# robot-learning-freiburg/CL-SLAM

Measured on AMD Instinct MI355X. Metric: online-adapt frames/sec @192x640 (1 triplet + K replay), higher is better.
Workload: dtype f32; 1 GPU; DepthPosePrediction.adapt(steps=1), 192x640, 1 online + K=4 replay triplets (global batch 5); ResNet-18 depth+pose nets, closed-form random-init weights; a frame = 5 triplets (value = steps/s * B/5); global_batch=5, replay_k=4, height=192, width=640, adapt_steps_per_frame=1, parallelism=single, lcd_encoder_in_frame=False

## Files before the change

cl-slam_amd/clslam_hip/_lib.py:

```python
import ctypes as C
from pathlib import Path

import torch
from typing import Optional

LIB_PATH = Path(__file__).resolve().parents[1] / 'lib' / 'libclslam_hip.so'

OK = 0
ACT_NONE, ACT_RELU, ACT_ELU, ACT_HSWISH, ACT_HSIGMOID = 0, 1, 2, 3, 4
PAD_ZERO, PAD_REFLECT = 0, 1
DEPTH_EVAL_MEDIAN_SCALING, DEPTH_EVAL_FROM_DISP, DEPTH_EVAL_NO_MAX = 1, 2, 4

fptr = C.c_void_p
i32 = C.c_int32


class ConvDesc(C.Structure):
    _fields_ = [('src_a', fptr), ('src_b', fptr), ('weight', fptr), ('scale', fptr), ('shift', fptr),
                ('residual', fptr), ('out', fptr),
                ('batch', i32), ('in_h', i32), ('in_w', i32), ('ch_a', i32), ('ch_b', i32),
                ('out_h', i32), ('out_w', i32), ('ch_out', i32),
                ('ksize', i32), ('stride', i32), ('pad', i32), ('pad_mode', i32), ('upsample_a', i32),
                ('act', i32), ('config', i32), ('actgrad_src', fptr), ('actgrad_kind', i32),
                ('workspace', C.c_void_p), ('workspace_bytes', C.c_size_t), ('weight_wino', fptr), ('cu_limit', i32)]


class TransposeItem(C.Structure):
    _fields_ = [('w', fptr), ('wt', fptr), ('ch_out', i32), ('taps', i32), ('ch_in', i32), ('ch_in_sel', i32)]


class CopyItem(C.Structure):
    _fields_ = [('src', C.c_void_p), ('dst', C.c_void_p), ('bytes', C.c_size_t)]


class LossDesc(C.Structure):
    _fields_ = [('partial', fptr * 4), ('disp', fptr * 4), ('rgb0', fptr * 4), ('means', fptr * 4),
                ('pose', fptr), ('dist0', fptr), ('dist1', fptr), ('sample_w', fptr), ('smooth_w', fptr),
                ('losses', fptr), ('smooth_aux', fptr),
                ('batch', i32), ('nblk', i32), ('H', i32), ('W', i32), ('n_smooth', i32),
                ('smooth_scale', C.c_float), ('vel_scale', C.c_float)]


_SIGNATURES = {
    'clslam_version': [],
    'clslam_is_device_build': [],
    'clslam_conv2d': [C.POINTER(ConvDesc), C.c_void_p],
    'clslam_conv2d_pick_config': [C.POINTER(ConvDesc)],
    'clslam_wino_weight_transform': [fptr, fptr, i32, i32, C.c_void_p],
    'clslam_weight_transpose': [fptr, fptr, i32, i32, i32, i32, C.c_void_p],
    'clslam_weight_transpose_multi': [C.POINTER(TransposeItem), i32, C.c_void_p],
    'clslam_fold_blocks': [i32, i32, i32, i32, i32],
    'clslam_fold_act_grad': [fptr, fptr, fptr, fptr, i32, i32, i32, i32, i32, i32, i32, i32, fptr, fptr, C.c_void_p],
    'clslam_wgrad_splits': [C.POINTER(ConvDesc), i32],
    'clslam_conv_wgrad': [C.POINTER(ConvDesc), fptr, fptr, i32, C.c_void_p],
    'clslam_wgrad_patch_supported': [C.POINTER(ConvDesc)],
    'clslam_wgrad_patch_splits': [C.POINTER(ConvDesc), i32],
    'clslam_conv_wgrad_patch': [C.POINTER(ConvDesc), fptr, fptr, i32, C.c_void_p],
    'clslam_reduce_partials': [fptr, fptr, C.c_size_t, i32, C.c_float, C.c_void_p],
    'clslam_reduce_multi': [fptr, i32, i32, C.c_void_p],
    'clslam_reduce_multi_adam': [fptr, i32, i32, fptr, fptr, fptr, fptr, C.c_double, C.c_double, C.c_double, C.c_double, i32, fptr, C.c_void_p],
    'clslam_colsum_blocks': [i32],
    'clslam_colsum': [fptr, fptr, i32, i32, C.c_void_p],
    'clslam_stem_packed_size': [i32],
    'clslam_stem_pack_weight': [fptr, fptr, i32, C.c_void_p],
    'clslam_stem_conv': [fptr, fptr, fptr, fptr, fptr, fptr, i32, i32, i32, i32, C.c_void_p],
    'clslam_maxpool3x3s2': [fptr, fptr, i32, i32, i32, i32, C.c_void_p],
    'clslam_dispconv_fwd': [fptr, fptr, fptr, fptr, i32, i32, i32, i32, C.c_void_p],
    'clslam_dispconv_bwd_data': [fptr, fptr, fptr, i32, i32, i32, i32, i32, C.c_void_p],
    'clslam_dispconv_wgrad_blocks': [i32],
    'clslam_dispconv_wgrad': [fptr, fptr, fptr, i32, i32, i32, i32, C.c_void_p],
    'clslam_pose_head_fwd': [fptr, fptr, fptr, fptr, fptr, i32, i32, C.c_void_p],
    'clslam_pose_head_bwd': [fptr, fptr, fptr, fptr, fptr, fptr, fptr, i32, i32, C.c_float, C.c_void_p],
    'clslam_pose_to_proj': [fptr, fptr, fptr, fptr, i32, C.c_void_p],
    'clslam_warp_fwd': [fptr, i32, i32, fptr, fptr, fptr, fptr, fptr, fptr, i32, i32, i32, C.c_float, C.c_float, C.c_void_p],
    'clslam_warp_fwd_pyramid': [C.POINTER(fptr), fptr, fptr, fptr, fptr, fptr, fptr, i32, i32, i32, C.c_float, C.c_float, C.c_void_p],
    'clslam_warp_coords_pyramid': [C.POINTER(fptr), fptr, fptr, fptr, i32, i32, i32, C.c_float, C.c_float, C.c_void_p],
    'clslam_warp_cells_pyramid': [C.POINTER(fptr), fptr, fptr, C.c_void_p, i32, i32, i32, C.c_float, C.c_float, C.c_void_p],
    'clslam_warp_bwd_blocks': [i32, i32],
    'clslam_automask_pyramid': [fptr, fptr, fptr, fptr, fptr, i32, i32, i32, i32, C.c_void_p],
    'clslam_disp_mean_pyramid': [C.POINTER(fptr), fptr, i32, i32, i32, C.c_void_p],
    'clslam_photo_automask_pyramid': [fptr, fptr, fptr, fptr, fptr, fptr, fptr, i32, i32, i32, C.c_void_p],
    'clslam_warp_fwd_pyramid_range': [C.POINTER(fptr), fptr, fptr, fptr, fptr, fptr, fptr, i32, i32, i32, C.c_float, C.c_float, i32, i32,
                                      C.c_void_p],
    'clslam_photo_automask_pyramid_range': [fptr, fptr, fptr, fptr, C.c_uint64, C.c_uint64, fptr, fptr, fptr, i32, i32, i32, i32, i32,
                                            C.c_void_p],
    'clslam_loss_bwd2_pyramid_range': [C.POINTER(fptr), fptr, fptr, fptr, fptr, fptr, fptr, fptr, fptr, fptr, fptr, fptr, i32, i32, i32,
                                       C.c_float, C.c_float, i32, i32, C.c_void_p],
    'clslam_disp_grad_pyramid_range': [fptr, C.POINTER(fptr), fptr, i32, C.POINTER(fptr), i32, i32, i32, i32, i32, C.c_void_p],
    'clslam_photo_automask_pyramid_rng': [fptr, fptr, fptr, C.c_uint64, C.c_uint64, fptr, fptr, fptr, i32, i32, i32, C.c_void_p],
    'clslam_tie_break_noise': [fptr, C.c_size_t, C.c_uint64, C.c_uint64, C.c_void_p],
    'clslam_smooth_intended_chunks': [],
    'clslam_smooth_intended_fwd': [C.POINTER(fptr), C.POINTER(fptr), fptr, i32, i32, i32, C.c_void_p],
    'clslam_smooth_intended_finalize': [fptr, fptr, fptr, fptr, fptr, i32, i32, i32, C.c_float, C.c_void_p],
    'clslam_smooth_intended_bwd': [C.POINTER(fptr), C.POINTER(fptr), fptr, fptr, C.POINTER(fptr), i32, i32, i32, C.c_float, C.c_void_p],
    'clslam_loss_bwd2_blocks': [i32, i32],
    'clslam_loss_bwd2_pyramid': [C.POINTER(fptr), fptr, fptr, fptr, fptr, fptr, fptr, fptr, fptr, fptr, fptr, fptr, i32, i32, i32,
                                 C.c_float, C.c_float, C.c_void_p],
    'clslam_loss_bwd_blocks': [i32, i32],
    'clslam_loss_bwd_pyramid': [C.POINTER(fptr), fptr, fptr, fptr, fptr, fptr, fptr, fptr, fptr, fptr, fptr, fptr, i32, i32, i32,
                                C.c_float, C.c_float, C.c_void_p],
    'clslam_disp_grad_pyramid': [fptr, C.POINTER(fptr), fptr, i32, C.POINTER(fptr), i32, i32, i32, C.c_void_p],
    'clslam_warp_bwd': [fptr, fptr, i32, i32, fptr, fptr, fptr, fptr, fptr, fptr, i32, i32, i32, C.c_float, C.c_float,
                        C.c_void_p],
    'clslam_pose_bwd': [fptr, i32, i32, fptr, fptr, fptr, fptr, fptr, C.c_float, fptr, i32, C.c_void_p],
    'clslam_photo_map': [fptr, fptr, fptr, fptr, i32, i32, i32, i32, C.c_void_p],
    'clslam_automask_blocks': [i32, i32],
    'clslam_automask': [fptr, fptr, fptr, fptr, fptr, i32, i32, i32, C.c_void_p],
    'clslam_disp_mean_chunks': [],
    'clslam_disp_mean': [fptr, fptr, i32, i32, C.c_void_p],
    'clslam_loss_finalize': [C.POINTER(LossDesc), C.c_void_p],
    'clslam_photo_grad': [fptr, fptr, fptr, fptr, fptr, fptr, i32, i32, i32, C.c_void_p],
    'clslam_mbv3_stem': [fptr, fptr, fptr, fptr, fptr, i32, i32, i32, C.c_void_p],
    'clslam_dwconv': [fptr, fptr, fptr, fptr, fptr, i32, i32, i32, i32, i32, i32, i32, C.c_void_p],
    'clslam_lanczos_ksize': [i32, i32],
    'clslam_lanczos_plan': [i32, i32, C.c_void_p, C.c_void_p],
    'clslam_resize_pass_u8': [C.c_void_p, C.c_void_p, fptr, C.c_void_p, C.c_void_p, i32, i32, i32, i32, i32, i32, i32, C.c_void_p],
    'clslam_u8_to_planar_f32': [C.c_void_p, fptr, i32, i32, i32, i32, C.c_void_p],
    'clslam_color_jitter_u8': [C.c_void_p, C.c_void_p, C.c_void_p, C.c_void_p, i32, i32, i32, C.POINTER(C.c_int), i32,
                               C.POINTER(C.c_double), C.c_void_p],
    'clslam_color_jitter_f32_blocks': [i32, i32],
    'clslam_color_jitter_f32': [fptr, fptr, C.c_void_p, fptr, i32, i32, i32, C.c_void_p],
    'clslam_avgpool_chunks': [i32],
    'clslam_global_avgpool': [fptr, fptr, fptr, i32, i32, i32, C.c_void_p],
    'clslam_se_gate': [fptr, fptr, fptr, fptr, fptr, fptr, i32, i32, i32, C.c_void_p],
    'clslam_channel_scale': [fptr, fptr, i32, i32, i32, C.c_void_p],
    'clslam_adam_step': [fptr, fptr, fptr, fptr, C.c_size_t, C.c_double, C.c_double, C.c_double, C.c_double, i32, C.c_float,
                         fptr, C.c_void_p],
    'clslam_disp_grad': [fptr, fptr, fptr, i32, fptr, i32, i32, i32, i32, i32, C.c_void_p],
    'clslam_copy_multi': [C.c_void_p, i32, C.c_void_p],
    'clslam_handoff_arm': [C.c_void_p],
    'clslam_handoff_wait': [C.c_void_p, C.c_void_p, C.c_void_p],
    'clslam_conv_profile_begin': [i32],
    'clslam_conv_profile_end': [C.c_void_p, i32, C.c_void_p],
    'clslam_ip_scores': [fptr, fptr, fptr, i32, i32, i32, C.c_void_p],
    'clslam_topk_chunks': [i32],
    'clslam_topk_desc': [fptr, i32, i32, i32, fptr, C.c_void_p, fptr, C.c_void_p, C.c_void_p],
    'clslam_l2_normalize_rows': [fptr, i32, i32, C.c_void_p],
    'clslam_diversity_commit': [fptr, fptr, i32, C.c_void_p, i32, i32, i32, i32, C.c_float, fptr, fptr, C.c_void_p,
                                fptr, C.c_void_p],    'clslam_pgo_edge_eval': [fptr, fptr, fptr, i32, fptr, fptr, fptr, C.c_void_p],
    'clslam_pgo_lin_stride': [],
    'clslam_pgo_build_system': [fptr, fptr, fptr, fptr, fptr, i32, fptr, fptr, fptr, i32, i32, fptr, fptr, fptr, fptr, C.c_void_p],
    'clslam_pgo_solve_workspace': [i32],
    'clslam_pgo_solve': [fptr, fptr, fptr, fptr, fptr, C.c_double, i32, C.c_double, i32, fptr, fptr, fptr, C.c_void_p],
    'clslam_pgo_update_score': [fptr, fptr, fptr, i32, fptr, fptr, fptr, fptr, fptr, i32, i32, fptr, i32, C.c_void_p],
    'clslam_depth_metrics_scratch': [i32, i32, i32],
    'clslam_depth_metrics': [fptr, fptr, fptr, C.c_void_p, fptr, fptr, i32, i32, i32, i32, i32, C.c_float, C.c_float, i32, C.c_void_p],
    'clslam_pcl_backproject_scratch': [i32, i32, i32],
    'clslam_pcl_backproject': [fptr, fptr, fptr, fptr, fptr, C.c_void_p, i32, i32, i32, C.c_float, C.c_void_p],
    'clslam_pcl_transform': [fptr, fptr, fptr, fptr, C.c_longlong, i32, C.c_void_p],
    'clslam_pcl_splat_scratch': [i32, i32],
    'clslam_pcl_splat': [fptr, fptr, fptr, i32, fptr, fptr, i32, i32, C.c_longlong, C.c_longlong, i32, C.c_double, i32, C.c_void_p],
    'clslam_pcl_resolve': [fptr, fptr, C.c_longlong, fptr, fptr, fptr, i32, i32, i32, C.c_void_p],
}
_RESTYPES = {'clslam_last_error': C.c_char_p, 'clslam_last_error_string': C.c_char_p, 'clslam_build_id': C.c_char_p}
ABI_VERSION = 106
_SIZE_FNS = {'clslam_wino_weight_size': [i32, i32]}
_PTR_FNS = {'clslam_handoff_event_create': []}
_VOID_FNS = {'clslam_handoff_event_destroy': [C.c_void_p]}


class ClslamError(RuntimeError):
    pass


class Library:
    def __init__(self, path: Path, require_device: bool = True) -> None:
        if not Path(path).exists():
            raise ClslamError(
                f'{path} not found: build it with `python cl-slam_amd/csrc/build.py` '
                '(hipcc --offload-arch=gfx950). There is no CPU fallback for this path.')
        self.path = Path(path)
        self.cdll = C.CDLL(str(path))
        try:
            got = int(self.cdll.clslam_version())
        except AttributeError:
            raise ClslamError(f'{path} does not export clslam_version: not a clslam kernel library') from None
        if got != ABI_VERSION:
            raise ClslamError(f'{path} implements ABI version {got}, this binding needs {ABI_VERSION}: rebuild it with '
                              '`python cl-slam_amd/csrc/build.py`')
        for name, rt in _RESTYPES.items():
            fn = getattr(self.cdll, name)
            fn.restype, fn.argtypes = rt, []
        for name, argtypes in _SIZE_FNS.items():
            fn = getattr(self.cdll, name)
            fn.restype, fn.argtypes = C.c_size_t, argtypes
        for name, argtypes in _PTR_FNS.items():
            fn = getattr(self.cdll, name)
            fn.restype, fn.argtypes = C.c_void_p, argtypes
        for name, argtypes in _VOID_FNS.items():
            fn = getattr(self.cdll, name)
            fn.restype, fn.argtypes = None, argtypes
        for name, argtypes in _SIGNATURES.items():
            fn = getattr(self.cdll, name)
            fn.argtypes = argtypes
            fn.restype = C.c_int
        self.is_device = bool(self.cdll.clslam_is_device_build())
        if require_device and not self.is_device:
            raise ClslamError(f'{path} is not a gfx950 device build')

    def call(self, name: str, *args) -> None:
        rc = getattr(self.cdll, name)(*args)
        if rc != OK:
            raise ClslamError(f'{name} failed ({rc}): {self.cdll.clslam_last_error().decode()}')

    @property
    def device_type(self) -> str:
        return 'cuda' if self.is_device else 'cpu'


_LIB: Optional[Library] = None


def get_lib() -> Library:
    global _LIB
    if _LIB is None:
        _LIB = Library(LIB_PATH, require_device=True)
    return _LIB


def install_library_for_tests(path) -> Library:
    global _LIB
    _LIB = Library(Path(path), require_device=False)
    return _LIB


def exported_symbols():
    return list(_RESTYPES) + list(_SIZE_FNS) + list(_PTR_FNS) + list(_VOID_FNS) + list(_SIGNATURES)


def build_id() -> str:
    built = get_lib().cdll.clslam_build_id().decode()
    built = built.split(':', 1)[1] if built.startswith('clslam-build-id:') else built
    csrc = Path(__file__).resolve().parents[1] / 'csrc'
    if not (csrc / 'build.py').exists():
        return built
    import importlib.util
    spec = importlib.util.spec_from_file_location('_clslam_build', csrc / 'build.py')
    mod = importlib.util.module_from_spec(spec)
    spec.loader.exec_module(mod)
    src = mod.source_id()
    return built if built == src else f'stale:{built}/{src}'
```

cl-slam_amd/clslam_hip/engine.py:

```python
import contextlib
import math
import os
from types import SimpleNamespace
from typing import Any, Dict, List, Optional, Tuple

import torch

from . import ops
from ._lib import ACT_ELU, ACT_NONE, ACT_RELU, PAD_REFLECT, PAD_ZERO, ClslamError, get_lib

NUM_CH_ENC = (64, 64, 128, 256, 512)
NUM_CH_DEC = (16, 32, 64, 128, 256)
BN_EPS = 1e-5

LOSS_NAMES = ('reprojection_loss', 'smooth_loss', 'reg_loss', 'depth_loss')

WGRAD_TARGET_BLOCKS = 512


def _align4(n: int) -> int:
    return (n + 3) // 4 * 4


class TrainableLayout:
# ... 111 lines not shown
        for st in (self.main_stream, self.side_stream, self.wg_stream, self.capture_stream):
            if st is not None:
                self._conv_workspace(st.cuda_stream)
        self.async_tail = False
        self.data_parallel = False
        self.tail_stream = pool.get('tail')
        self._tail_event = None
        self._tail_open = False
        self.fuse_adam = os.environ.get('CLSLAM_FUSE_ADAM', '0') == '1'
        self._pending_reduce = None
        self.descriptor_memo = os.environ.get('CLSLAM_DESCRIPTOR_MEMO', '1') != '0'
        self._memo = None
        self.memo_hits = 0
        self.grad_buckets = int(os.environ.get('CLSLAM_GRAD_BUCKETS', '3'))
        self.grads_synced = False
        self.time_exchange = False
        self.exchange_events: List[Any] = []
        self.exchange_main_done = None
        self._capturing = False
        self._noise_torch_seed = None
        self.noise_seed = 1
        self.noise_draws = 0
        self.noise_stream = 0
        self._handoff = ops.Handoff() if device.type == 'cuda' else None
        self._cu_enc = self._cu_dec = self._cu_pose = self._cu_depth = 0
        self.device_cus = (torch.cuda.get_device_properties(device).multi_processor_count if device.type == 'cuda' else 256)
        self.reuse_frozen_features = os.environ.get('CLSLAM_REUSE_FROZEN', '1') != '0'
        self.winograd = not os.environ.get('CLSLAM_NO_WINOGRAD')

    def bind(self, models: Dict[str, torch.nn.Module]) -> None:
        self.models = models
        for name, m in models.items():
            m._bind(self, name)

    def _module_version(self) -> int:
        if self._tracked is None:
            self._tracked = [t for m in self.models.values() for t in torch.nn.Module.state_dict(m, keep_vars=True).values()]
        return sum(t._version for t in self._tracked)

    def pack_if_needed(self) -> None:
        ver = self._module_version()
        if ver != self._packed_version:
            if self._modules_stale:
                raise ClslamError('module parameters were modified while newer adapted weights live in the engine; '
                                  'call sync_modules() first')
            self.pack()

    def _on(self, st):
        if st is None:
            return contextlib.nullcontext()
        return torch.cuda.stream(st) if self._capturing else ops.launch_on(st)

    def _use_tail(self) -> bool:
        return (self.async_tail and self.tail_stream is not None and self.device.type == 'cuda' and not self._capturing
                and ops.PROFILE is None)

    def _side_streams(self):
        return (self.side_stream, self.wg_stream) if self.use_side_stream else (None, None)

    def cu_limit(self, B: int, phase: str = 'encoders') -> int:
        if not phase.startswith('enc'):
            return 0
        if not (self.use_side_stream and 2 <= B <= 16):
            return 0
        if phase == 'enc_pose':
            return self.device_cus * 5 // 8
        if phase == 'enc_depth':
            return self.device_cus * 3 // 8
        return self.device_cus // 2

    def wait_training(self, stream=None) -> None:
        if self._tail_event is not None:
            (stream or torch.cuda.current_stream(self.device)).wait_event(self._tail_event)
        if self._train_done is not None:
            (stream or torch.cuda.current_stream(self.device)).wait_event(self._train_done)

    @property
    def w(self) -> torch.Tensor:
        self.wait_training()
        return self._w

    @property
    def g(self) -> torch.Tensor:
        self.wait_training()
        return self._g

    @property
    def m(self) -> torch.Tensor:
        self.wait_training()
        return self._m

    @property
    def v(self) -> torch.Tensor:
        self.wait_training()
        return self._v

    def prealloc_outputs(self, B: int) -> None:
        H, W = self.H, self.W
        E = lambda *s: torch.empty(*s, device=self.device)
        self._prealloc = (B, ([E(B, H >> s, W >> s) for s in range(4)], E(2 * B, 12), E(2, B, 4, 4), E(4, B, H, W),
                              E(4, 2, B, 3, H, W), E(18)))

    def detached_ok(self) -> bool:
        return (self.detached_training and self.main_stream is not None and self.device.type == 'cuda'
                and not self._capturing and ops.PROFILE is None)

    def begin_detached(self):
        cur = torch.cuda.current_stream(self.device)
        em = self.main_stream
        if cur.cuda_stream == em.cuda_stream:
            return cur, None
        em.wait_stream(cur)
        self._caller = cur
        return cur, em

    def end_detached(self, cur, released, failed: bool = False) -> None:
        self._caller = None
        self._prealloc, self._prealloc_armed = None, False
        ev = torch.cuda.Event()
        ev.record(self.main_stream)
        self._train_done = ev
        cur.wait_event(ev if (failed or released is None) else released)

    def training_stream(self):
        return torch.cuda.stream(self.tail_stream) if self._tail_open else contextlib.nullcontext()

    @torch.no_grad()
    def pack(self) -> None:
        dev = self.device
        self.wait_training()
        for which in ('depth_encoder', 'pose_encoder'):
            sd = {k: v.detach().to(dev, torch.float32) for k, v in torch.nn.Module.state_dict(self.models[which]).items()}
            e = SimpleNamespace()

            def bn(prefix):
                scale = sd[prefix + '.weight'] / torch.sqrt(sd[prefix + '.running_var'] + BN_EPS)
                shift = sd[prefix + '.bias'] - sd[prefix + '.running_mean'] * scale
                return scale.contiguous(), shift.contiguous()

            def conv(key):
                wt = sd[key]
                return wt.permute(0, 2, 3, 1).reshape(wt.shape[0], wt.shape[2] * wt.shape[3], wt.shape[1]).contiguous()

            e.stem_w = ops.stem_pack_weight(sd['resnet.conv1.weight'].contiguous())
            e.stem_scale, e.stem_shift = bn('resnet.bn1')
            e.blocks = []
            for li, (cin, cout, stride) in enumerate(((64, 64, 1), (64, 128, 2), (128, 256, 2), (256, 512, 2)), start=1):
                for bi in range(2):
                    p = f'resnet.layer{li}.{bi}'
                    blk = SimpleNamespace(stride=stride if bi == 0 else 1, cin=cin if bi == 0 else cout, cout=cout)
                    blk.w1 = conv(p + '.conv1.weight'); blk.s1, blk.b1 = bn(p + '.bn1')
                    blk.w2 = conv(p + '.conv2.weight'); blk.s2, blk.b2 = bn(p + '.bn2')
                    blk.u1 = ops.wino_weight_transform(blk.w1) if (blk.stride == 1 and self.winograd) else None
                    blk.u2 = ops.wino_weight_transform(blk.w2) if self.winograd else None
                    blk.wd = None
                    if (p + '.downsample.0.weight') in sd:
                        blk.wd = conv(p + '.downsample.0.weight'); blk.sd, blk.bd = bn(p + '.downsample.1')
                    e.blocks.append(blk)
            self.enc[which] = e
        for name, off, shape in self.layout.entries:
            model, key = name.split('/', 1)
            t = torch.nn.Module.state_dict(self.models[model])[key].detach().to(dev, torch.float32)
            flat = TrainableLayout.to_compute(t)
            self._w[off:off + flat.numel()].copy_(flat)
        self._packed_version = self._module_version()
        self._modules_stale = False
        self._desc_cache.clear()
        for ws in self._ws.values():
            if hasattr(ws, 'frozen_valid'):
                ws.frozen_valid = False
        self._memo = None

    @torch.no_grad()
    def sync_modules(self) -> None:
        if not self._modules_stale or self.models is None:
            return
        self.wait_training()
        for name, off, shape in self.layout.entries:
            model, key = name.split('/', 1)
            p = torch.nn.Module.state_dict(self.models[model], keep_vars=True)[key]
            p.data.copy_(TrainableLayout.to_reference(self._w[off:off + math.prod(shape)], shape))
        self._modules_stale = False
        self._packed_version = self._module_version()

    @torch.no_grad()
    def install_weights(self, flat: torch.Tensor, adam_step_count: Optional[int] = None) -> None:
        self.pack_if_needed()
        self.wait_training()
        self._w.copy_(flat.reshape(-1)[:self.layout.size])
        if adam_step_count is not None:
            self.adam_step_count = int(adam_step_count)
        self._modules_stale = True

    def wview(self, name: str) -> torch.Tensor:
        self.wait_training()
        for n, off, shape in self.layout.entries:
            if n == name:
                return self._w[off:off + math.prod(shape)]
        raise KeyError(name)

    def _slot(self, buf: torch.Tensor, name: str, numel: int) -> torch.Tensor:
        off = self.layout.offset[name]
        return buf[off:off + numel]

    def workspace(self, B: int) -> SimpleNamespace:
        ws = self._ws.get(B)
        if ws is not None:
            return ws
        dev, H, W = self.device, self.H, self.W
        E = lambda *s: torch.empty(*s, device=dev)
        ws = SimpleNamespace(B=B)
        ws.denc = self._enc_bufs(B)
        ws.penc = self._enc_bufs(2 * B)
        self._depth_dec_bufs(B, ws)
        self._pose_dec_bufs(2 * B, ws)
        ws.T = E(2, B, 4, 4)
        ws.P = E(2, B, 3, 4)
        ws.depth = E(4, B, H, W)
        ws.warped = E(4, 2, B, 3, H, W)
        ws.idmap = E(2, B, H, W)
        ws.coef = None
        ws.sel = torch.empty(4, B, H, W, dtype=torch.uint8, device=dev)
        ws.nblk = ops.automask_blocks(H, W)
        ws.partial = E(4, B, ws.nblk)
        ws.means = E(4, B, ops.disp_mean_chunks())
        ws.losses = E(18)
        ws.noise = E(4, B, 2, H, W)
        ws.train = None
        self._ws[B] = ws
        return ws

    def _enc_bufs(self, n: int) -> SimpleNamespace:
        dev, H, W = self.device, self.H, self.W
        E = lambda *s: torch.empty(*s, device=dev)
        hs = [H >> k for k in range(6)]
        wsz = [W >> k for k in range(6)]
        e = SimpleNamespace()
        e.f0 = E(n, hs[1], wsz[1], 64)
        e.pool = E(n, hs[2], wsz[2], 64)
        e.t = [E(n, hs[2 + li], wsz[2 + li], c) for li, c in enumerate((64, 128, 256, 512))]
        e.ds = [None] + [E(n, hs[2 + li], wsz[2 + li], c) for li, c in ((1, 128), (2, 256), (3, 512))]
        e.y = [[E(n, hs[2 + li], wsz[2 + li], c) for _ in range(2)] for li, c in enumerate((64, 128, 256, 512))]
        return e

    def _depth_dec_bufs(self, n: int, st: Optional[SimpleNamespace] = None) -> SimpleNamespace:
        st = SimpleNamespace() if st is None else st
        H, W = self.H, self.W
        E = lambda *s: torch.empty(*s, device=self.device)
        st.x = {}
        for i in range(4, -1, -1):
            st.x[i, 0] = E(n, H >> (i + 1), W >> (i + 1), NUM_CH_DEC[i])
            st.x[i, 1] = E(n, H >> i, W >> i, NUM_CH_DEC[i])
        st.disp = [E(n, H >> s, W >> s) for s in range(4)]
        return st

    def _pose_dec_bufs(self, n: int, st: Optional[SimpleNamespace] = None) -> SimpleNamespace:
        st = SimpleNamespace() if st is None else st
        h5, w5 = self.H >> 5, self.W >> 5
        E = lambda *s: torch.empty(*s, device=self.device)
        st.sq, st.p0, st.p1 = E(n, h5, w5, 256), E(n, h5, w5, 256), E(n, h5, w5, 256)
        st.pmean, st.pose = E(n, 256), E(n, 12)
        return st

    def _train_bufs(self, ws: SimpleNamespace) -> SimpleNamespace:
        if ws.train is not None:
            return ws.train
        dev, H, W, B = self.device, self.H, self.W, ws.B
        E = lambda *s: torch.empty(*s, device=dev)
        t = SimpleNamespace()
        ws.coef = E(4, B, 9, H, W)
        t.ddisp_up = E(4, B, H, W)
        t.nb2 = ops.loss_bwd2_blocks(H, W)
        t.dp_partial = torch.empty(4, B, t.nb2, 24, dtype=torch.float64, device=dev)
        t.dz_disp = [torch.empty(B, H >> s, W >> s, device=dev) for s in range(4)]
        t.dpose = E(2 * B, 12)
        t.dz = {k: torch.empty_like(v) for k, v in ws.x.items()}
        pad_elems = max(B * ((H >> i) + 2) * ((W >> i) + 2) * NUM_CH_DEC[i] for i in range(5))
        t.dxp = [E(pad_elems), E(pad_elems)]
        t.wt_ready = None
        t.wt_dec = {}
        t.wt_pose = {}
        t.wt_table = None
        t.dz_p1 = torch.empty_like(ws.p1)
        t.dz_p0 = torch.empty_like(ws.p0)
        t.dz_sq = torch.empty_like(ws.sq)
        t.plan, t.items, t.table, t.disp_part = {}, [], None, {}
        t.side = SimpleNamespace()
        t.bias_part = {k: E(ops.fold_blocks(v.shape[0], v.shape[1], v.shape[2], v.shape[3], False) * v.shape[-1])
                       for k, v in ws.x.items()}
        ws.train = t
        return t

    CONV_WS_BYTES = 32 << 20

    def _conv_workspace(self, handle: Optional[int] = None) -> None:
        if self.device.type != 'cuda' and handle is None:
            handle = 0
        if handle is None:
            handle = torch.cuda.current_stream(self.device).cuda_stream
        if handle not in self._conv_ws:
            self._conv_ws[handle] = torch.zeros(self.CONV_WS_BYTES, dtype=torch.uint8, device=self.device)
            ops.set_conv_workspace(handle, self._conv_ws[handle])

    def _encoder(self, e, bufs, n: int, stem_inputs, waits=None, stream=None, aux=None, cu_limit=None) -> List[torch.Tensor]:
        ops.PERSISTENT_CU_LIMIT = self._cu_enc if cu_limit is None else cu_limit
        ek = (id(self), 'enc', id(e), id(bufs), n)
        for i, (img_a, img_b, off, cnt) in enumerate(stem_inputs):
            if waits is not None:
                (stream or torch.cuda.current_stream(self.device)).wait_event(waits[i])
            ops.stem_conv(img_a, img_b, e.stem_w, e.stem_scale, e.stem_shift, bufs.f0[off:off + cnt])
        ops.maxpool3x3s2(bufs.f0, bufs.pool)
        x = bufs.pool
        feats = [bufs.f0]
        for li in range(4):
            for bi in range(2):
                blk = e.blocks[li * 2 + bi]
                t, y = bufs.t[li], bufs.y[li][bi]
                res, joined = x, None
                if blk.wd is not None:
                    res = bufs.ds[li]
                    if aux is not None and stream is not None:
                        evs = bufs.__dict__.setdefault('ds_events', {})
                        fork, joined = evs.get(li) or evs.setdefault(li, (torch.cuda.Event(), torch.cuda.Event()))
                        fork.record(stream)
                        aux.wait_event(fork)
                        with self._on(aux):
                            ops.conv2d(x, blk.wd, res, scale=blk.sd, shift=blk.bd, ksize=1, stride=blk.stride, pad=0, act=ACT_NONE,
                                       cache=self._desc_cache, key=(ek, li, bi, 'd'))
                        joined.record(aux)
                ops.conv2d(x, blk.w1, t, scale=blk.s1, shift=blk.b1, ksize=3, stride=blk.stride, act=ACT_RELU, weight_wino=blk.u1,
                           cache=self._desc_cache, key=(ek, li, bi, 1))
                if blk.wd is not None and joined is None:
                    ops.conv2d(x, blk.wd, res, scale=blk.sd, shift=blk.bd, ksize=1, stride=blk.stride, pad=0, act=ACT_NONE,
                               cache=self._desc_cache, key=(ek, li, bi, 'd'))
                if joined is not None:
                    stream.wait_event(joined)
                ops.conv2d(t, blk.w2, y, scale=blk.s2, shift=blk.b2, residual=res, ksize=3, act=ACT_RELU, weight_wino=blk.u2,
                           cache=self._desc_cache, key=(ek, li, bi, 2))
                x = y
            feats.append(x)
        return feats

    def _wb(self, prefix: str, cout: int, cin: int, taps: int):
        hit = self._wb_cache.get(prefix)
        if hit is None:
            w = self._slot(self._w, prefix + '.weight', cout * taps * cin).view(cout, taps, cin)
            b = self._slot(self._w, prefix + '.bias', cout)
            hit = self._wb_cache[prefix] = (w, b)
        return hit

    def _depth_decoder(self, ws, feats: List[torch.Tensor]) -> None:
        x = feats[4]
        ops.PERSISTENT_CU_LIMIT = self._cu_dec
        main = self._main
        leaf = self._side_streams()[1] if main is not None else None
        forked = False
        for i in range(4, -1, -1):
            cin0 = NUM_CH_ENC[-1] if i == 4 else NUM_CH_DEC[i + 1]
            w, b = self._wb(f'depth_decoder/upconv_{i}_0.conv.conv', NUM_CH_DEC[i], cin0, 9)
            ops.conv2d(x, w, ws.x[i, 0], shift=b, ksize=3, pad_mode=PAD_REFLECT, act=ACT_ELU, cache=self._desc_cache, key=(id(self), 'dec', id(ws), i, 0))
            skip = feats[i - 1] if i > 0 else None
            cin1 = NUM_CH_DEC[i] + (NUM_CH_ENC[i - 1] if i > 0 else 0)
            w, b = self._wb(f'depth_decoder/upconv_{i}_1.conv.conv', NUM_CH_DEC[i], cin1, 9)
            fork = leaf is not None and 0 < i <= 3
            ho = self._handoff if (fork and not self._capturing and ops.PROFILE is None) else None
            if ho is not None:
                ho.arm()
            ops.conv2d(ws.x[i, 0], w, ws.x[i, 1], src_b=skip, shift=b, ksize=3, pad_mode=PAD_REFLECT, upsample_a=True,
                       act=ACT_ELU, cache=self._desc_cache, key=None if skip is None else (id(self), 'dec', id(ws), i, 1, skip.data_ptr()))
            x = ws.x[i, 1]
            if i <= 3:
                w, b = self._wb(f'depth_decoder/dispconv_{i}.conv', 1, NUM_CH_DEC[i], 9)
                if fork:
                    if ho is not None:
                        ho.release(main, leaf)
                    else:
                        ev = torch.cuda.Event()
                        ev.record(main)
                        leaf.wait_event(ev)
                    with self._on(leaf):
                        ops.dispconv_fwd(x, w.view(9, NUM_CH_DEC[i]), b, ws.disp[i])
                    forked = True
                else:
                    ops.dispconv_fwd(x, w.view(9, NUM_CH_DEC[i]), b, ws.disp[i])
        if forked:
            main.wait_stream(leaf)

    def _pose_decoder(self, ws, f4: torch.Tensor) -> None:
        ops.PERSISTENT_CU_LIMIT = self._cu_dec
        w, b = self._wb('pose_decoder/squeeze', 256, 512, 1)
        ops.conv2d(f4, w, ws.sq, shift=b, ksize=1, pad=0, act=ACT_RELU, cache=self._desc_cache, key=(id(self), 'pdec', id(ws), 0))
        w, b = self._wb('pose_decoder/pose_0', 256, 256, 9)
        ops.conv2d(ws.sq, w, ws.p0, shift=b, ksize=3, act=ACT_RELU, cache=self._desc_cache, key=(id(self), 'pdec', id(ws), 1))
        w, b = self._wb('pose_decoder/pose_1', 256, 256, 9)
        ops.conv2d(ws.p0, w, ws.p1, shift=b, ksize=3, act=ACT_RELU, cache=self._desc_cache, key=(id(self), 'pdec', id(ws), 2))
        w, b = self._wb('pose_decoder/pose_2', 12, 256, 1)
        ops.pose_head_fwd(ws.p1, w.view(12, 256), b, ws.pmean, ws.pose)

    def forward(self, inputs: Dict[Any, torch.Tensor], *, train: bool, sample_w: torch.Tensor,
                smooth_w: Optional[torch.Tensor], noise: Optional[Dict[int, torch.Tensor]] = None,
                draw_noise: bool = True, keep_noise: bool = False,
                reuse_frozen: bool = False, inputs_ready=None) -> Tuple[Dict[Any, torch.Tensor], torch.Tensor]:
        self._main = torch.cuda.current_stream(self.device) if self.device.type == 'cuda' else None
        self._conv_workspace(None if self._main is None else self._main.cuda_stream)
        if self._train_done is not None and self._main.cuda_stream != self.main_stream.cuda_stream:
            self._main.wait_event(self._train_done)
        c = SimpleNamespace(inputs=inputs, inputs_ready=inputs_ready, train=train, noise=noise, draw_noise=draw_noise,
                            keep_noise=keep_noise, have_noise=False, id_ready=None)
        self._convert_inputs(c)
        B = c.B
        self._cu_enc, self._cu_dec = self.cu_limit(B, 'encoders'), self.cu_limit(B, 'decoders')
        self._cu_pose, self._cu_depth = self.cu_limit(B, 'enc_pose'), self.cu_limit(B, 'enc_depth')
        ops.PERSISTENT_CU_LIMIT = self._cu_dec
        ws = self.workspace(B)
        c.reuse = bool(reuse_frozen and self.reuse_frozen_features and getattr(ws, 'frozen_valid', False))
        ws.frozen_valid = False
        c.memo_feats = self._memo_lookup(c.aug[0]) if (B == 1 and not c.reuse) else None
        if train:
            self._train_bufs(ws)
        if self.fresh_outputs:
            self._fresh_output_planes(ws, B)
        self._networks(ws, c)
        self._loss_stage(ws, c, sample_w, smooth_w)
        ws.frozen_valid = True
        return self._outputs(ws, B), ws.losses

    def _convert_inputs(self, c) -> None:
        inputs, H, W = c.inputs, self.H, self.W
        if c.inputs_ready is not None:
            needs_conversion = any(inputs[k, f, 0].dtype != torch.float32 or not inputs[k, f, 0].is_contiguous()
                                   for k in ('rgb_aug', 'rgb') for f in (-1, 0, 1))
            self._main.wait_event(c.inputs_ready[3 if needs_conversion else 0])
        c.aug = {f: self._img(inputs['rgb_aug', f, 0]) for f in (-1, 0, 1)}
        c.rgb = {f: self._img(inputs['rgb', f, 0]) for f in (-1, 0, 1)}
        B = c.B = c.aug[0].shape[0]
        for name, group in (('rgb_aug', c.aug), ('rgb', c.rgb)):
            for f, t in group.items():
                if tuple(t.shape) != (B, 3, H, W):
                    raise ClslamError(f"('{name}', {f}, 0) must be ({B}, 3, {H}, {W}), got {tuple(t.shape)}")
        for s in range(1, 4):
            t = inputs['rgb', 0, s]
            if tuple(t.shape) != (B, 3, H >> s, W >> s):
                raise ClslamError(f"('rgb', 0, {s}) must be ({B}, 3, {H >> s}, {W >> s}), got {tuple(t.shape)}")
        for k in (('camera_matrix', 0), ('inv_camera_matrix', 0)):
            if tuple(inputs[k].shape) != (B, 4, 4):
                raise ClslamError(f'{k} must be ({B}, 4, 4), got {tuple(inputs[k].shape)}')

    def _fresh_output_planes(self, ws, B: int) -> None:
        H, W = self.H, self.W
        pre = self._prealloc if self._prealloc_armed else None
        if pre is not None and pre[0] == B:
            self._prealloc = None
            ws.disp, ws.pose, ws.T, ws.depth, ws.warped, ws.losses = pre[1]
        else:
            E = lambda *s: torch.empty(*s, device=self.device)
            ws.disp = [E(B, H >> s, W >> s) for s in range(4)]
            ws.pose, ws.T = E(2 * B, 12), E(2, B, 4, 4)
            ws.depth, ws.warped, ws.losses = E(4, B, H, W), E(4, 2, B, 3, H, W), E(18)

    def _identity_and_noise(self, ws, c) -> bool:
        if not c.reuse:
            ops.photo_map(c.rgb[-1], c.rgb[0], ws.idmap[0], None, c.B, c.B, self.H, self.W)
            ops.photo_map(c.rgb[1], c.rgb[0], ws.idmap[1], None, c.B, c.B, self.H, self.W)
        if c.noise is not None:
            for s in range(4):
                ws.noise[s].copy_(c.noise[s])
            return True
        if c.keep_noise:
            return True
        if c.draw_noise and self._capturing:
            ws.noise.normal_().mul_(1e-5)
            return True
        return False

    def _enqueue_identity(self, ws, c, wg) -> None:
        if c.inputs_ready is not None:
            wg.wait_event(c.inputs_ready[3])
        with (torch.cuda.stream(wg) if (c.noise is not None or self._capturing) else ops.launch_on(wg)):
            c.have_noise = self._identity_and_noise(ws, c)
        c.id_ready = torch.cuda.Event()
        c.id_ready.record(wg)

    def _pose_encoder(self, ws, c, **kw) -> torch.Tensor:
        aug, B = c.aug, c.B
        return self._encoder(self.enc['pose_encoder'], ws.penc, 2 * B, [(aug[-1], aug[0], 0, B), (aug[0], aug[1], B, B)],
                             waits=None if c.inputs_ready is None else c.inputs_ready[1:3], cu_limit=self._cu_pose, **kw)[4]

    def _pose_branch(self, ws, c, side, ds_aux) -> torch.Tensor:
        with self._on(side):
            pf4 = ws.pf4 if c.reuse else self._pose_encoder(ws, c, stream=side, aux=ds_aux)
            self.wait_training(side)
            self._pose_decoder(ws, pf4)
        return pf4

    def _networks(self, ws, c) -> None:
        B, reuse, main = c.B, c.reuse, self._main
        side, wg = self._side_streams()
        ds_aux = wg if (B == 1 and not self._capturing) else None
        defer_identity = wg is not None and ds_aux is not None and c.inputs_ready is not None and not reuse
        if wg is not None:
            wg.wait_stream(main)
            if not defer_identity:
                self._enqueue_identity(ws, c, wg)
        if side is not None:
            side.wait_stream(main)
            if reuse:
                dfeats = ws.dfeats
                self.wait_training(main)
                self._depth_decoder(ws, dfeats)
                pf4 = self._pose_branch(ws, c, side, ds_aux)
            else:
                dfeats = c.memo_feats if c.memo_feats is not None else self._encoder(
                    self.enc['depth_encoder'], ws.denc, B, [(c.aug[0], None, 0, B)], stream=main, aux=ds_aux, cu_limit=self._cu_depth)
                pf4 = self._pose_branch(ws, c, side, ds_aux)
                self.wait_training(main)
                self._depth_decoder(ws, dfeats)
            main.wait_stream(side)
        else:
            self.wait_training()
            dfeats = (ws.dfeats if reuse else c.memo_feats if c.memo_feats is not None else
                      self._encoder(self.enc['depth_encoder'], ws.denc, B, [(c.aug[0], None, 0, B)], cu_limit=self._cu_depth))
            self._depth_decoder(ws, dfeats)
            pf4 = ws.pf4 if reuse else self._pose_encoder(ws, c)
            self._pose_decoder(ws, pf4)
        ws.dfeats, ws.pf4 = dfeats, pf4
        if defer_identity:
            self._enqueue_identity(ws, c, wg)

    def _loss_stage(self, ws, c, sample_w: torch.Tensor, smooth_w: Optional[torch.Tensor]) -> None:
        inputs, rgb, B, H, W = c.inputs, c.rgb, c.B, self.H, self.W
        if c.inputs_ready is not None:
            self._main.wait_event(c.inputs_ready[3])
        K = self._mat(inputs['camera_matrix', 0])
        Kinv = self._mat(inputs['inv_camera_matrix', 0])
        ops.pose_to_proj(ws.pose, K, ws.T, ws.P)
        ops.warp_fwd_pyramid(ws.disp, rgb[-1], rgb[1], Kinv, ws.P, ws.depth, ws.warped, self.min_depth, self.max_depth)
        if c.id_ready is not None:
            self._main.wait_event(c.id_ready)
        else:
            c.have_noise = self._identity_and_noise(ws, c)
        if c.have_noise or not c.draw_noise:
            ops.photo_automask_pyramid(ws.warped, rgb[0], ws.idmap, ws.noise if c.have_noise else None, ws.sel,
                                       ws.coef if c.train else None, ws.partial, B, H, W)
        else:
            seed, offset = self._next_noise_draw()
            ops.photo_automask_pyramid_rng(ws.warped, rgb[0], ws.idmap, seed, offset, ws.sel,
                                           ws.coef if c.train else None, ws.partial, B, H, W)
        ops.disp_mean_pyramid(ws.disp, ws.means, H, W)
        n_smooth = 0 if (smooth_w is None or self.smooth_intended) else int(smooth_w.numel())
        if n_smooth and not (n_smooth < (W >> 3) - 1):
            raise ClslamError('reference smoothness layout needs batch < width/8 - 1')
        aux = getattr(ws, 'smooth_aux', None)
        if n_smooth and (aux is None or aux.shape[1] != 2 + 2 * n_smooth):
            aux = torch.zeros(4, 2 + 2 * n_smooth, device=self.device)
            ws.smooth_aux = aux
        d0 = inputs['relative_distance', 0].to(torch.float64).reshape(-1).contiguous() if self.vel_scale > 0 else None
        d1 = inputs['relative_distance', 1].to(torch.float64).reshape(-1).contiguous() if self.vel_scale > 0 else None
        rgb0 = [self._img(inputs['rgb', 0, s]) for s in range(4)]
        ops.loss_finalize([ws.partial[s] for s in range(4)], ws.disp, rgb0, [ws.means[s] for s in range(4)], ws.pose, d0, d1,
                          sample_w, smooth_w if n_smooth else None, ws.losses, aux if n_smooth else None, B, ws.nblk, H, W,
                          n_smooth, self.smooth_scale, self.vel_scale)
        if self.smooth_intended:
            if getattr(ws, 'si_partial', None) is None:
                ws.si_partial = torch.empty(4, B, ops.smooth_intended_chunks(), device=self.device)
                ws.si_aux = torch.empty(4, B, 2, device=self.device)
            ops.smooth_intended_fwd(ws.disp, rgb0, ws.si_partial, H, W)
            ops.smooth_intended_finalize(ws.si_partial, ws.means, sample_w, ws.losses, ws.si_aux, B, H, W, self.smooth_scale)
        ws.ctx = SimpleNamespace(rgb=rgb, K=K, Kinv=Kinv, d0=d0, d1=d1, sample_w=sample_w, n_smooth=n_smooth,
                                 aux=aux if n_smooth else None, B=B, rgb0=rgb0)

    def _memo_lookup(self, x: torch.Tensor) -> Optional[List[torch.Tensor]]:
        m = self._memo
        if (m is None or not self.descriptor_memo or self._capturing or m.version != self._packed_version
                or m.x.shape != x.shape or m.x.device != x.device):
            return None
        self._memo = None
        if not bool(torch.equal(m.x, x)):
            return None
        self.memo_hits += 1
        return m.feats

    def _next_noise_draw(self) -> Tuple[int, int]:
        if self.device.type == 'cuda':
            gen = torch.cuda.default_generators[self.device.index if self.device.index is not None else torch.cuda.current_device()]
            ts = int(gen.initial_seed())
            off = int(gen.get_offset())
            gen.set_offset(off + 4)
            self.noise_draws = off // 4 + 1
        else:
            ts = int(torch.default_generator.initial_seed())
            if ts != self._noise_torch_seed:
                self.noise_draws = 0
            self.noise_draws += 1
        if ts != self._noise_torch_seed:
            self._noise_torch_seed = ts
            self.noise_seed = (ts * 0x9E3779B97F4A7C15 + 0x7F4A7C15) & 0xFFFFFFFFFFFFFFFF or 1
        return self.noise_seed, (int(self.noise_stream) << 40) | self.noise_draws

    def _img(self, t: torch.Tensor) -> torch.Tensor:
        if t.dtype != torch.float32 or not t.is_contiguous():
            t = t.to(torch.float32).contiguous()
        return t

    def _mat(self, t: torch.Tensor) -> torch.Tensor:
        return t.to(torch.float32).contiguous()

    def _outputs(self, ws, B: int) -> Dict[Any, torch.Tensor]:
        out: Dict[Any, torch.Tensor] = {}
        for s in (3, 2, 1, 0):
            out['disp', s] = ws.disp[s].unsqueeze(1)
        for fi, f in enumerate((-1, 1)):
            out['axis_angle', 0, f] = ws.pose[fi * B:(fi + 1) * B, 0:3].unsqueeze(1)
            out['translation', 0, f] = ws.pose[fi * B:(fi + 1) * B, 3:6].unsqueeze(1)
            out['cam_T_cam', 0, f] = ws.T[fi]
        for s in range(4):
            out['depth', s] = ws.depth[s].unsqueeze(1)
            for fi, f in enumerate((-1, 1)):
                out['rgb', f, s] = ws.warped[s, fi]
        return out

    def losses_dict(self, losses: torch.Tensor) -> Dict[str, torch.Tensor]:
        d: Dict[str, torch.Tensor] = {}
        for s in range(4):
            for j, name in enumerate(LOSS_NAMES):
                d[f'{name}/scale_{s}'] = losses[s * 4 + j]
        total = losses[17:18]
        d['depth_loss'] = total
        if self.vel_scale > 0:
            d['velocity_loss'] = losses[16]
        d['loss'] = total
        return d

    def _wgrad(self, t, desc_src, out_shape, dz, name_prefix: str, cout: int, cin: int, taps: int, bias_blocks: int = 0,
               bias_partial=None, **geom) -> None:
        desc = ops.conv_desc(desc_src[0], out_shape, src_b=desc_src[1], ksize=3 if taps == 9 else 1, **geom)
        n = cout * taps * cin
        plan = t.plan.get(name_prefix)
        if plan is None:
            use_patch = ops.wgrad_patch_supported(desc)
            splits = (ops.wgrad_patch_splits(desc, WGRAD_TARGET_BLOCKS) if use_patch else
                      ops.wgrad_splits(desc, WGRAD_TARGET_BLOCKS))
            plan = SimpleNamespace(use_patch=use_patch, splits=splits, partial=torch.empty(splits * n, device=self.device),
                                   colsum=None, nb=0)
            t.items.append((plan.partial, self._slot(self._g, name_prefix + '.weight', n), n, splits))
            if bias_blocks:
                t.items.append((bias_partial, self._slot(self._g, name_prefix + '.bias', cout), cout, bias_blocks))
            else:
                rows = out_shape[0] * out_shape[1] * out_shape[2]
                plan.nb = ops.colsum_blocks(rows)
                plan.colsum = torch.empty(plan.nb * cout, device=self.device)
                t.items.append((plan.colsum, self._slot(self._g, name_prefix + '.bias', cout), cout, plan.nb))
            t.plan[name_prefix] = plan
        if plan.use_patch:
            ops.conv_wgrad_patch(desc, dz, plan.partial, plan.splits)
        else:
            ops.conv_wgrad(desc, dz, plan.partial, plan.splits)
        if plan.colsum is not None:
            ops.colsum(dz, plan.colsum, out_shape[0] * out_shape[1] * out_shape[2], cout)

    def bucket_ranges(self):
        off = self.layout.offset
        a_end, c_start = off['depth_decoder/upconv_3_0.conv.conv.weight'], off['pose_decoder/squeeze.weight']
        if self.grad_buckets >= 3:
            return [('pose', c_start, self.layout.size), ('mid', a_end, c_start), ('deep', 0, a_end)]
        if self.grad_buckets == 2:
            return [('early', a_end, self.layout.size), ('deep', 0, a_end)]
        return [('all', 0, self.layout.size)]

    def exchange_report(self) -> Optional[Dict[str, Any]]:
        if not self.exchange_events or self.exchange_main_done is None:
            return None
        buckets = [{'bucket': n, 'mbytes': round(nb / 1e6, 2), 'ms': round(e0.elapsed_time(e1), 4)} for n, e0, e1, nb in self.exchange_events]
        total = sum(b['ms'] for b in buckets)
        exposed = max(0.0, self.exchange_main_done.elapsed_time(self.exchange_events[-1][2]))
        rep = {'buckets': buckets, 'allreduce_ms': round(total, 4), 'exposed_ms': round(exposed, 4),
               'overlap_fraction': round(1.0 - min(exposed, total) / total, 4) if total > 0 else None}
        self.exchange_events, self.exchange_main_done = [], None
        return rep

    def _bucket_sync(self, t, name: str, events, allreduce) -> None:
        tail = self.tail_stream
        for ev in events:
            tail.wait_event(ev)
        table, n, lo, hi = t.bucket_tables[name]
        with torch.cuda.stream(tail):
            ops.reduce_multi(table, n, self._g)
            if self.time_exchange:
                e0, e1 = torch.cuda.Event(enable_timing=True), torch.cuda.Event(enable_timing=True)
                e0.record(tail)
                allreduce(self._g[lo:hi])
                e1.record(tail)
                self.exchange_events.append((name, e0, e1, (hi - lo) * 4))
            else:
                allreduce(self._g[lo:hi])

    def backward(self, B: int, defer_reduce: bool = False, allreduce=None) -> None:
        ops.PERSISTENT_CU_LIMIT = self.cu_limit(B, 'backward')
        ws = self._ws[B]
        t = ws.train
        c = ws.ctx
        H, W = self.H, self.W
        feats = ws.dfeats
        self._main = torch.cuda.current_stream(self.device) if self.device.type == 'cuda' else None
        side, wg = self._side_streams()
        t.wt_ready = None
        if wg is None:
            self._transpose_decoder_weights(t)
        else:
            wg.wait_stream(self._main)
            with self._on(wg):
                self._transpose_decoder_weights(t)
            t.wt_ready = torch.cuda.Event()
            t.wt_ready.record(wg)
        ops.loss_bwd2_pyramid(ws.disp, ws.sel, ws.coef, ws.warped, c.rgb[0], c.rgb[-1], c.rgb[1], c.Kinv, ws.P, c.sample_w,
                              t.ddisp_up, t.dp_partial, self.min_depth, self.max_depth)
        ops.disp_grad_pyramid(t.ddisp_up, ws.disp, c.aux if c.n_smooth else None, c.n_smooth, t.dz_disp, H, W)
        if self.smooth_intended:
            ops.smooth_intended_bwd(ws.disp, c.rgb0, ws.si_aux, c.sample_w, t.dz_disp, H, W, self.smooth_scale)
        ops.pose_bwd(t.dp_partial, 4, t.nb2, ws.pose, c.K, c.d0, c.d1, c.sample_w, self.vel_scale, t.dpose)
        self.inputs_released = None
        if self._caller is not None:
            self.inputs_released = torch.cuda.Event()
            self.inputs_released.record(self._main)
        bucketed = allreduce is not None and self.grad_buckets > 1
        overlap = (bucketed and self._use_tail() and side is not None and wg is not None
                   and getattr(t, 'bucket_tables', None) is not None)
        self.grads_synced = False
        if side is not None:
            main = self._main
            side.wait_stream(main)
            if t.wt_ready is not None:
                side.wait_event(t.wt_ready)
            with self._on(side):
                self._backward_pose_decoder(ws, t, B, t.side)
            if overlap and self.grad_buckets >= 3:
                ev = torch.cuda.Event()
                ev.record(side)
                self._bucket_sync(t, 'pose', [ev], allreduce)
            self._backward_depth_decoder(ws, t, B, mid_done=(lambda evs: self._bucket_sync(
                t, 'mid' if self.grad_buckets >= 3 else 'early', evs, allreduce)) if overlap else None)
            main.wait_stream(side)
        else:
            self._backward_depth_decoder(ws, t, B)
            self._backward_pose_decoder(ws, t, B, t)
        if t.table is None:
            for key, n in (('pose_decoder/pose_2.weight', 12 * 256), ('pose_decoder/pose_2.bias', 12)):
                sl = self._slot(self._g, key, n)
                t.items.append((sl, sl, n, 1))
            t.table = ops.make_reduce_table(t.items, self.device)
            base = self._g.data_ptr()
            t.bucket_tables = {}
            for name, lo, hi in self.bucket_ranges():
                its = [it for it in t.items if lo <= (it[1].data_ptr() - base) // 4 < hi]
                t.bucket_tables[name] = (ops.make_reduce_table(its, self.device), len(its), lo, hi)
            assert sum(v[1] for v in t.bucket_tables.values()) == len(t.items)
        self._pending_reduce = None
        if bucketed:
            ranges = self.bucket_ranges()
            if overlap:
                name, lo, hi = ranges[-1]
                if self.time_exchange:
                    self.exchange_main_done = torch.cuda.Event(enable_timing=True)
                    self.exchange_main_done.record(self._main)
                self.tail_stream.wait_stream(self._main)
                self._bucket_sync(t, name, [], allreduce)
                self._tail_open = True
            else:
                if self._use_tail():
                    self.tail_stream.wait_stream(self._main)
                    with torch.cuda.stream(self.tail_stream):
                        ops.reduce_multi(t.table, len(t.items), self._g)
                        for name, lo, hi in ranges:
                            allreduce(self._g[lo:hi])
                    self._tail_open = True
                else:
                    ops.reduce_multi(t.table, len(t.items), self._g)
                    for name, lo, hi in ranges:
                        allreduce(self._g[lo:hi])
            self.grads_synced = True
        elif defer_reduce and self.fuse_adam and not self.data_parallel and not self._capturing and not self._use_tail():
            self._pending_reduce = (t.table, len(t.items))
        elif self._use_tail():
            self.tail_stream.wait_stream(self._main)
            with torch.cuda.stream(self.tail_stream):
                ops.reduce_multi(t.table, len(t.items), self._g)
            self._tail_open = True
        else:
            ops.reduce_multi(t.table, len(t.items), self._g)

    def _transpose_decoder_weights(self, t) -> None:
        if t.wt_table is None:
            items = []
            for i in range(5):
                ci = NUM_CH_DEC[i]
                cin1 = ci + (NUM_CH_ENC[i - 1] if i > 0 else 0)
                t.wt_dec[i, 1] = torch.empty(ci, 9, ci, device=self.device)
                w1, _ = self._wb(f'depth_decoder/upconv_{i}_1.conv.conv', ci, cin1, 9)
                items.append((w1, t.wt_dec[i, 1], ci))
                if i < 4:
                    cin0 = NUM_CH_DEC[i + 1]
                    t.wt_dec[i, 0] = torch.empty(cin0, 9, ci, device=self.device)
                    w0, _ = self._wb(f'depth_decoder/upconv_{i}_0.conv.conv', ci, cin0, 9)
                    items.append((w0, t.wt_dec[i, 0], None))
            for k in (0, 1):
                t.wt_pose[k] = torch.empty(256, 9, 256, device=self.device)
                wp, _ = self._wb(f'pose_decoder/pose_{k}', 256, 256, 9)
                items.append((wp, t.wt_pose[k], None))
            t.wt_table = ops.transpose_table(items)
        ops.weight_transpose_multi(t.wt_table, self._w)

    def _backward_depth_decoder(self, ws, t, B: int, mid_done=None) -> None:
        H, W = self.H, self.W
        feats = ws.dfeats
        main = self._main
        side, wg = self._side_streams()
        if wg is not None:
            wg.wait_stream(main)

        wg_streams = [wg] if (wg is None or side is None) else [wg, side]
        counter = [0]

        ho = self._handoff if (wg is not None and not self._capturing and ops.PROFILE is None) else None

        def on_wg(fn, dep='record'):
            if wg is None:
                fn()
                return
            st = wg_streams[counter[0] % len(wg_streams)]
            counter[0] += 1
            if dep == 'armed':
# ... 288 lines not shown
```

cl-slam_amd/clslam_hip/ops.py:

```python
import ctypes as C
from typing import Optional

import torch

from . import _lib
from ._lib import ACT_ELU, ACT_HSIGMOID, ACT_HSWISH, ACT_NONE, ACT_RELU, PAD_REFLECT, PAD_ZERO


PROFILE = None


def profile_begin(max_launches: int = 8192) -> None:
    global PROFILE
    _lib.get_lib().call('clslam_conv_profile_begin', max_launches)
    PROFILE = []


def profile_end():
    global PROFILE
    meta, PROFILE = PROFILE, None
    cap = max(1, len(meta))
    ms = (C.c_float * cap)()
    count = C.c_int(0)
    _lib.get_lib().call('clslam_conv_profile_end', C.cast(ms, C.c_void_p), cap, C.cast(C.pointer(count), C.c_void_p))
    if not _lib.get_lib().is_device:
        return [(k, cfg, fl, 0.0, desc, nb) for k, cfg, fl, desc, nb in meta]
    if count.value != len(meta):
        raise _lib.ClslamError(f'profile_end: {count.value} timed launches for {len(meta)} conv2d calls')
    return [(k, cfg, fl, ms[i] * 1e-3, desc, nb) for i, (k, cfg, fl, desc, nb) in enumerate(meta)]


_raw_stream = torch._C._cuda_getCurrentRawStream if hasattr(torch._C, '_cuda_getCurrentRawStream') else None


_FORCED_STREAM: Optional[int] = None


class launch_on:
    __slots__ = ('handle', 'prev')

    def __init__(self, stream):
        self.handle = None if stream is None else stream.cuda_stream

    def __enter__(self):
        global _FORCED_STREAM
        self.prev = _FORCED_STREAM
        if self.handle is not None:
            _FORCED_STREAM = self.handle
        return self

    def __exit__(self, *exc):
        global _FORCED_STREAM
        _FORCED_STREAM = self.prev
        return False


def _stream(t: torch.Tensor) -> int:
    if _FORCED_STREAM is not None:
        return _FORCED_STREAM
    if t.is_cuda:
        if _raw_stream is not None:
            return _raw_stream(t.device.index)
        return torch.cuda.current_stream(t.device).cuda_stream
    return 0


_QUERY_CACHE: dict = {}


def _query(name: str, *args) -> int:
    lib = _lib._LIB or _lib.get_lib()
    key = (id(lib), name, args)
    v = _QUERY_CACHE.get(key)
    if v is None:
        v = _QUERY_CACHE[key] = getattr(lib.cdll, name)(*args)
    return v


def _p(t: Optional[torch.Tensor]):
    if t is None:
        return None
    lib = _lib._LIB or _lib.get_lib()
    if t.is_cuda != lib.is_device or t.dtype is not torch.float32 or not t.is_contiguous():
        if t.device.type != lib.device_type:
            raise _lib.ClslamError(f'tensor on {t.device}, library {lib.path.name} runs on {lib.device_type}')
        raise _lib.ClslamError(f'expected contiguous fp32, got {t.dtype} contiguous={t.is_contiguous()}')
    return t.data_ptr()


def _pa(t: Optional[torch.Tensor], dtype):
    if t is None:
        return None
    lib = _lib.get_lib()
    if t.device.type != lib.device_type or t.dtype != dtype or not t.is_contiguous():
        raise _lib.ClslamError(f'expected contiguous {dtype} on {lib.device_type}, got {t.dtype} on {t.device}')
    return t.data_ptr()


class Handoff:
    POOL = 64

    def __init__(self) -> None:
        self.lib = _lib.get_lib()
        self.events = []
        self.next = 0
        self.armed = None

    def arm(self) -> None:
        if not self.lib.is_device:
            return
        if len(self.events) < self.POOL:
            ev = self.lib.cdll.clslam_handoff_event_create()
            if not ev:
                raise _lib.ClslamError('clslam_handoff_event_create failed: ' + self.lib.cdll.clslam_last_error().decode())
            self.events.append(ev)
            self.armed = ev
        else:
            self.armed = self.events[self.next % self.POOL]
        self.next += 1
        self.lib.call('clslam_handoff_arm', self.armed)

    def release(self, producer, consumer) -> None:
        ev, self.armed = self.armed, None
        if ev is None:
            return
        self.lib.call('clslam_handoff_wait', ev, producer.cuda_stream, consumer.cuda_stream)

    def __del__(self):
        try:
            for ev in self.events:
                self.lib.cdll.clslam_handoff_event_destroy(ev)
        except Exception:
            pass


_CONV_WORKSPACES = {}


def set_conv_workspace(stream_handle: int, workspace: Optional[torch.Tensor]) -> None:
    if workspace is None:
        _CONV_WORKSPACES.pop(stream_handle, None)
    else:
        assert workspace.dtype == torch.uint8 and workspace.is_contiguous()
        _CONV_WORKSPACES[stream_handle] = workspace


PERSISTENT_CU_LIMIT = 0


_CONV_DESC_CACHE: dict = {}


def conv2d(src_a, weight, out, *, src_b=None, scale=None, shift=None, residual=None, ksize=3, stride=1,
           pad=None, pad_mode=PAD_ZERO, upsample_a=False, act=ACT_NONE, config=-1, actgrad_src=None,
           actgrad_kind=ACT_NONE, workspace=None, weight_wino=None, cu_limit=None, key=None, cache=None):
    if cache is None:
        cache = _CONV_DESC_CACHE
    if key is not None and PROFILE is None:
        ent = cache.get(key)
        if ent is not None:
            d, ref, lib = ent
            if d.src_a == src_a.data_ptr() and d.out == out.data_ptr() and d.weight == weight.data_ptr():
                stream = _stream(out)
                ws = workspace if workspace is not None else (_CONV_WORKSPACES.get(stream) if _CONV_WORKSPACES else None)
                if ws is None:
                    d.workspace, d.workspace_bytes = None, 0
                else:
                    d.workspace, d.workspace_bytes = ws.data_ptr(), ws.numel()
                d.cu_limit = PERSISTENT_CU_LIMIT if cu_limit is None else cu_limit
                rc = lib.cdll.clslam_conv2d(ref, stream)
                if rc != _lib.OK:
                    raise _lib.ClslamError(f'clslam_conv2d failed ({rc}): {lib.cdll.clslam_last_error().decode()}')
                return out
    B, Ho, Wo, Cout = out.shape
    Ha, Wa, Ca = src_a.shape[1:]
    Hi, Wi = (Ha * 2, Wa * 2) if upsample_a else (Ha, Wa)
    Cb = 0 if src_b is None else src_b.shape[3]
    if pad is None:
        pad = ksize // 2
    assert weight.shape[0] == Cout and weight.numel() == Cout * ksize * ksize * (Ca + Cb), weight.shape
    stream = _stream(out)
    if workspace is None and _CONV_WORKSPACES:
        workspace = _CONV_WORKSPACES.get(stream)
    d = _lib.ConvDesc(_p(src_a), _p(src_b), _p(weight), _p(scale), _p(shift), _p(residual), _p(out),
                      B, Hi, Wi, Ca, Cb, Ho, Wo, Cout, ksize, stride, pad, pad_mode, int(upsample_a), act, config,
                      _p(actgrad_src), actgrad_kind, None if workspace is None else workspace.data_ptr(),
                      0 if workspace is None else workspace.numel(), _p(weight_wino),
                      PERSISTENT_CU_LIMIT if cu_limit is None else cu_limit)
    if PROFILE is not None:
        cfg = config if config >= 0 else _lib.get_lib().cdll.clslam_conv2d_pick_config(C.byref(d))
        nbytes = 4.0 * (src_a.numel() + (0 if src_b is None else src_b.numel()) + weight.numel() + out.numel() +
                        (0 if residual is None else residual.numel()) + (0 if actgrad_src is None else actgrad_src.numel()))
        PROFILE.append(('conv', cfg, 2.0 * B * Ho * Wo * Cout * ksize * ksize * (Ca + Cb),
                        f'B{B} {Hi}x{Wi} {Ca}+{Cb}->{Cout} k{ksize} s{stride} pad{pad}', nbytes))
    lib = _lib.get_lib()
    lib.call('clslam_conv2d', C.byref(d), stream)
    if key is not None and PROFILE is None:
        cache[key] = (d, C.byref(d), lib)
    return out


def conv_desc(src_a, out_shape, *, src_b=None, ksize=3, stride=1, pad=None, pad_mode=PAD_ZERO, upsample_a=False):
    B, Ho, Wo, Cout = out_shape
    Ha, Wa, Ca = src_a.shape[1:]
    Hi, Wi = (Ha * 2, Wa * 2) if upsample_a else (Ha, Wa)
    Cb = 0 if src_b is None else src_b.shape[3]
    if pad is None:
        pad = ksize // 2
    return _lib.ConvDesc(_p(src_a), _p(src_b), None, None, None, None, None, B, Hi, Wi, Ca, Cb, Ho, Wo, Cout,
                         ksize, stride, pad, pad_mode, int(upsample_a), ACT_NONE, -1, None, ACT_NONE, None, 0, None, 0)


def wino_weight_transform(w, out=None):
    Cout, taps, Cin = w.shape
    assert taps == 9
    n = _lib.get_lib().cdll.clslam_wino_weight_size(Cout, Cin)
    if out is None:
        out = torch.empty(n, device=w.device, dtype=torch.float32)
    assert out.numel() >= n
    _lib.get_lib().call('clslam_wino_weight_transform', _p(w), _p(out), Cout, Cin, _stream(w))
    return out


def weight_transpose(w, wt, ch_in_sel=None):
    Cout, taps, Cin = w.shape
    sel = Cin if ch_in_sel is None else ch_in_sel
    assert wt.numel() >= sel * taps * Cout
    _lib.get_lib().call('clslam_weight_transpose', _p(w), _p(wt), Cout, taps, Cin, sel, _stream(w))
    return wt


def transpose_table(items):
    tab = (_lib.TransposeItem * len(items))()
    for rec, (w, wt, sel) in zip(tab, items):
        Cout, taps, Cin = w.shape
        sel = Cin if sel is None else sel
        assert wt.numel() >= sel * taps * Cout
        rec.w, rec.wt, rec.ch_out, rec.taps, rec.ch_in, rec.ch_in_sel = _p(w), _p(wt), Cout, taps, Cin, sel
    return tab


def weight_transpose_multi(table, stream_ref):
    _lib.get_lib().call('clslam_weight_transpose_multi', table, len(table), _stream(stream_ref))


def fold_blocks(batch, h, w, ch, pool) -> int:
    return _query('clslam_fold_blocks', batch, h, w, ch, int(pool))


def fold_act_grad(dxp, yout, dz, *, h, w, ch, border, pool, act, bias_partial=None, disp_dz=None, disp_w=None):
    B = dz.shape[0]
    _lib.get_lib().call('clslam_fold_act_grad', _p(dxp), _p(yout), _p(dz), _p(bias_partial), B, h, w, ch,
                        ch if dxp is None else dxp.shape[3], border, int(pool), act, _p(disp_dz), _p(disp_w), _stream(dz))
    return dz


def wgrad_splits(desc, target_blocks=1024) -> int:
    return _lib.get_lib().cdll.clslam_wgrad_splits(C.byref(desc), target_blocks)


def conv_wgrad(desc, dz, partial, splits):
    _lib.get_lib().call('clslam_conv_wgrad', C.byref(desc), _p(dz), _p(partial), splits, _stream(dz))
    return partial


def wgrad_patch_supported(desc) -> bool:
    return bool(_lib.get_lib().cdll.clslam_wgrad_patch_supported(C.byref(desc)))


def wgrad_patch_splits(desc, target_blocks=1024) -> int:
    return _lib.get_lib().cdll.clslam_wgrad_patch_splits(C.byref(desc), target_blocks)


def conv_wgrad_patch(desc, dz, partial, splits):
    _lib.get_lib().call('clslam_conv_wgrad_patch', C.byref(desc), _p(dz), _p(partial), splits, _stream(dz))
    return partial


def reduce_partials(partial, out, n, splits, scale=1.0):
    _lib.get_lib().call('clslam_reduce_partials', _p(partial), _p(out), n, splits, scale, _stream(out))
    return out


def make_reduce_table(items, device):
    import numpy as np
    rec = np.zeros(len(items), dtype=np.dtype([('partial', '<u8'), ('out', '<u8'), ('n', '<u8'), ('splits', '<i4'), ('scale', '<f4')]))
    for i, (part, out, n, splits) in enumerate(items):
        rec[i] = (_p(part), _p(out), n, splits, 1.0)
    return torch.from_numpy(rec.view(np.uint8).copy()).to(device)


def reduce_multi(table, nitems, stream_ref, blocks_per_item=384):
    _lib.get_lib().call('clslam_reduce_multi', table.data_ptr(), nitems, blocks_per_item, _stream(stream_ref))


def reduce_multi_adam(table, nitems, grad, param, exp_avg, exp_avg_sq, lr, step, beta1=0.9, beta2=0.999, eps=1e-8, guard=None,
                      blocks_per_item=384):
    _lib.get_lib().call('clslam_reduce_multi_adam', table.data_ptr(), nitems, blocks_per_item, _p(grad), _p(param), _p(exp_avg),
                        _p(exp_avg_sq), lr, beta1, beta2, eps, step, _p(guard), _stream(grad))


def copy_multi(pairs, stream_ref=None):
    pairs = [(s, d) for s, d in pairs if d.numel()]
    if not pairs:
        return
    items = (_lib.CopyItem * len(pairs))()
    for it, (src, dst) in zip(items, pairs):
        if (src.dtype != dst.dtype or src.numel() != dst.numel() or src.device != dst.device
                or not src.is_contiguous() or not dst.is_contiguous()):
            raise _lib.ClslamError(f'copy_multi: {tuple(src.shape)} {src.dtype} {src.device} -> '
                                   f'{tuple(dst.shape)} {dst.dtype} {dst.device} is not a plain copy')
        it.src, it.dst, it.bytes = src.data_ptr(), dst.data_ptr(), src.numel() * src.element_size()
    _lib.get_lib().call('clslam_copy_multi', C.cast(items, C.c_void_p), len(pairs), _stream(stream_ref if stream_ref is not None else pairs[0][1]))


def colsum_blocks(rows: int) -> int:
    return _query('clslam_colsum_blocks', rows)


def colsum(x, partial, rows, ch):
    _lib.get_lib().call('clslam_colsum', _p(x), _p(partial), rows, ch, _stream(x))
    return partial


def stem_pack_weight(weight):
    n_img = weight.shape[1] // 3
    packed = torch.empty(_lib.get_lib().cdll.clslam_stem_packed_size(n_img), device=weight.device)
    _lib.get_lib().call('clslam_stem_pack_weight', _p(weight), _p(packed), n_img, _stream(weight))
    return packed


def stem_conv(img_a, img_b, weight, scale, shift, out):
    B, _, H, W = img_a.shape
    n_img = 1 if img_b is None else 2
    _lib.get_lib().call('clslam_stem_conv', _p(img_a), _p(img_b), _p(weight), _p(scale), _p(shift), _p(out),
                        B, H, W, n_img, _stream(out))
    return out


def maxpool3x3s2(x, out):
    B, H, W, Cc = x.shape
    _lib.get_lib().call('clslam_maxpool3x3s2', _p(x), _p(out), B, H, W, Cc, _stream(out))
    return out


def dispconv_fwd(x, w, bias, disp):
    B, H, W, Cc = x.shape
    _lib.get_lib().call('clslam_dispconv_fwd', _p(x), _p(w), _p(bias), _p(disp), B, H, W, Cc, _stream(disp))
    return disp


def dispconv_bwd_data(dz, w, dxp, ch, accumulate):
    B, H, W = dz.shape[0], dz.shape[-2], dz.shape[-1]
    _lib.get_lib().call('clslam_dispconv_bwd_data', _p(dz), _p(w), _p(dxp), B, H, W, ch, int(accumulate), _stream(dxp))
    return dxp


def dispconv_wgrad_blocks(pixels: int) -> int:
    return _query('clslam_dispconv_wgrad_blocks', pixels)


def dispconv_wgrad(dz, x, partial):
    B, H, W, Cc = x.shape
    _lib.get_lib().call('clslam_dispconv_wgrad', _p(dz), _p(x), _p(partial), B, H, W, Cc, _stream(x))
    return partial


def pose_head_fwd(x, w2, b2, mean, pose):
    N, H, W, _ = x.shape
    _lib.get_lib().call('clslam_pose_head_fwd', _p(x), _p(w2), _p(b2), _p(mean), _p(pose), N, H * W, _stream(x))
    return pose


def pose_head_bwd(dpose, x, w2, mean, dz1, dw2, db2, grad_scale=1.0):
    N, H, W, _ = x.shape
    _lib.get_lib().call('clslam_pose_head_bwd', _p(dpose), _p(x), _p(w2), _p(mean), _p(dz1), _p(dw2), _p(db2),
                        N, H * W, grad_scale, _stream(x))


def _nd(v):
    return -1.0 if v is None else float(v)


def pose_to_proj(pose, kmat, cam_t_cam, proj):
    B = kmat.shape[0]
    _lib.get_lib().call('clslam_pose_to_proj', _p(pose), _p(kmat), _p(cam_t_cam), _p(proj), B, _stream(pose))


def warp_fwd(disp_s, src_m1, src_p1, inv_k, proj, depth, warped, min_depth, max_depth):
    B, H, W = depth.shape[0], depth.shape[-2], depth.shape[-1]
    h, w = disp_s.shape[-2:]
    _lib.get_lib().call('clslam_warp_fwd', _p(disp_s), h, w, _p(src_m1), _p(src_p1), _p(inv_k), _p(proj), _p(depth),
                        _p(warped), B, H, W, _nd(min_depth), _nd(max_depth), _stream(depth))


def warp_bwd_blocks(H, W) -> int:
    return _query('clslam_warp_bwd_blocks', H, W)


def warp_bwd(dpred, disp_s, src_m1, src_p1, inv_k, proj, ddisp_up, dp_partial, min_depth, max_depth):
    B, H, W = ddisp_up.shape[0], ddisp_up.shape[-2], ddisp_up.shape[-1]
    h, w = disp_s.shape[-2:]
    _lib.get_lib().call('clslam_warp_bwd', _p(dpred), _p(disp_s), h, w, _p(src_m1), _p(src_p1), _p(inv_k), _p(proj),
                        _p(ddisp_up), _pa(dp_partial, torch.float64), B, H, W, _nd(min_depth), _nd(max_depth), _stream(dpred))


def pose_bwd(dp_partial, nscale, nblk, pose, kmat, dist0, dist1, sample_w, vel_scale, dpose):
    B = kmat.shape[0]
    _lib.get_lib().call('clslam_pose_bwd', _pa(dp_partial, torch.float64), nscale, nblk, _p(pose), _p(kmat), _pa(dist0, torch.float64),
                        _pa(dist1, torch.float64), _p(sample_w), float(vel_scale or 0.0), _p(dpose), B, _stream(pose))


def photo_map(pred, target, out_map, coef, npred, batch, H, W):
    _lib.get_lib().call('clslam_photo_map', _p(pred), _p(target), _p(out_map), _p(coef), npred, batch, H, W,
                        _stream(out_map))


def automask_blocks(H, W) -> int:
    return _query('clslam_automask_blocks', H, W)


def automask(idmap, noise, rpmap, sel, partial, batch, H, W):
    _lib.get_lib().call('clslam_automask', _p(idmap), _p(noise), _p(rpmap), _pa(sel, torch.uint8), _p(partial), batch,
                        H, W, _stream(idmap))


def disp_mean_chunks() -> int:
    return _query('clslam_disp_mean_chunks')


def disp_mean(disp, means):
    B = disp.shape[0]
    _lib.get_lib().call('clslam_disp_mean', _p(disp), _p(means), B, disp.numel() // B, _stream(disp))


def loss_finalize(partials, disps, rgb0s, means, pose, dist0, dist1, sample_w, smooth_w, losses, smooth_aux, batch,
                  nblk, H, W, n_smooth, smooth_scale, vel_scale):
    d = _lib.LossDesc()
    for s in range(4):
        d.partial[s] = _p(partials[s]); d.disp[s] = _p(disps[s]); d.rgb0[s] = _p(rgb0s[s]); d.means[s] = _p(means[s])
    d.pose = _p(pose)
    d.dist0 = _pa(dist0, torch.float64); d.dist1 = _pa(dist1, torch.float64)
    d.sample_w = _p(sample_w); d.smooth_w = _p(smooth_w); d.losses = _p(losses); d.smooth_aux = _p(smooth_aux)
    d.batch, d.nblk, d.H, d.W, d.n_smooth = batch, nblk, H, W, n_smooth
    d.smooth_scale, d.vel_scale = float(smooth_scale), float(vel_scale or 0.0)
    _lib.get_lib().call('clslam_loss_finalize', C.byref(d), _stream(losses))


def photo_grad(sel, coef, pred, target, sample_w, dpred, batch, H, W):
    _lib.get_lib().call('clslam_photo_grad', _pa(sel, torch.uint8), _p(coef), _p(pred), _p(target), _p(sample_w),
                        _p(dpred), batch, H, W, _stream(dpred))


def disp_grad(ddisp_up, disp, smooth_aux, n_smooth, dz, H, W):
    B, h, w = disp.shape[0], disp.shape[-2], disp.shape[-1]
    _lib.get_lib().call('clslam_disp_grad', _p(ddisp_up), _p(disp), _p(smooth_aux), n_smooth, _p(dz), B, h, w, H, W,
                        _stream(dz))


def adam_step(param, grad, exp_avg, exp_avg_sq, lr, step, beta1=0.9, beta2=0.999, eps=1e-8, grad_scale=1.0, guard=None):
    _lib.get_lib().call('clslam_adam_step', _p(param), _p(grad), _p(exp_avg), _p(exp_avg_sq), param.numel(), lr, beta1,
                        beta2, eps, step, grad_scale, _p(guard), _stream(param))


def mbv3_stem(img, weight, scale, shift, out):
    B, _, H, W = img.shape
    _lib.get_lib().call('clslam_mbv3_stem', _p(img), _p(weight), _p(scale), _p(shift), _p(out), B, H, W, _stream(out))
    return out


def dwconv(x, weight, scale, shift, out, ksize, stride, act):
    B, H, W, Cc = x.shape
    _lib.get_lib().call('clslam_dwconv', _p(x), _p(weight), _p(scale), _p(shift), _p(out), B, H, W, Cc, ksize, stride, act,
                        _stream(out))
    return out


def avgpool_chunks(hw: int) -> int:
    return _query('clslam_avgpool_chunks', hw)


def global_avgpool(x, out, partial=None):
    B, Cc = x.shape[0], x.shape[-1]
    hw = 1
    for n in x.shape[1:-1]:
        hw *= n
    _lib.get_lib().call('clslam_global_avgpool', _p(x), _p(out), _p(partial), B, hw, Cc, _stream(out))
    return out


def se_gate(pool, w1, b1, w2, b2, gate):
    B, Cc = pool.shape
    _lib.get_lib().call('clslam_se_gate', _p(pool), _p(w1), _p(b1), _p(w2), _p(b2), _p(gate), B, Cc, w1.shape[0],
                        _stream(gate))
    return gate


def channel_scale(x, gate):
    B, Cc = x.shape[0], x.shape[-1]
    _lib.get_lib().call('clslam_channel_scale', _p(x), _p(gate), B, x.numel() // (B * Cc), Cc, _stream(x))
    return x


def _ptr4(tensors):
# ... 301 lines not shown
```

cl-slam_amd/csrc/capi.hip:

```cpp
#include "common.h"

#include <cstdarg>
#include <cstdio>
#include <utility>
#include <vector>

namespace clslam {

static thread_local char g_err[512] = "";

void set_error(const char* fmt, ...) {
    va_list ap;
    va_start(ap, fmt);
    vsnprintf(g_err, sizeof(g_err), fmt, ap);
    va_end(ap);
}

int check_launch(const char* what) {
    hipError_t e = hipGetLastError();
    if (e != hipSuccess) {
        set_error("%s: launch failed: %s", what, hipGetErrorString(e));
        return CLSLAM_ERR_LAUNCH;
    }
    return CLSLAM_OK;
}

static thread_local std::vector<std::pair<hipEvent_t, hipEvent_t>> g_prof;
static thread_local int g_prof_cap = 0;

static thread_local hipEvent_t g_handoff = nullptr;

hipEvent_t take_handoff_event() {
    hipEvent_t e = g_handoff;
    g_handoff = nullptr;
    return e;
}

bool profile_next_events(hipEvent_t* start, hipEvent_t* stop) {
#if CLSLAM_DEVICE_BUILD
    if (g_prof_cap <= 0 || (int)g_prof.size() >= g_prof_cap) {
        hipEvent_t h = take_handoff_event();
        if (h == nullptr) return false;
        *start = nullptr; *stop = h;
        return true;
    }
    hipEvent_t a = nullptr, b = nullptr;
    if (hipEventCreate(&a) != hipSuccess || hipEventCreate(&b) != hipSuccess) return false;
    g_prof.emplace_back(a, b);
    *start = a; *stop = b;
    return true;
#else
    (void)start; (void)stop;
    return false;
#endif
}

}

extern "C" int clslam_conv_profile_begin(int max_launches) {
    CLSLAM_REQUIRE(max_launches > 0, "conv_profile_begin: max_launches must be positive");
    CLSLAM_REQUIRE(clslam::g_prof_cap == 0, "conv_profile_begin: already armed on this thread");
    clslam::g_prof.clear();
    clslam::g_prof_cap = max_launches;
    return CLSLAM_OK;
}

extern "C" int clslam_conv_profile_end(float* ms, int capacity, int* count) {
    CLSLAM_REQUIRE(count && (ms || capacity == 0), "conv_profile_end: null");
    clslam::g_prof_cap = 0;
    int n = 0, rc = CLSLAM_OK;
#if CLSLAM_DEVICE_BUILD
    for (auto& ev : clslam::g_prof) {
        float t = 0.f;
        if (hipEventSynchronize(ev.second) != hipSuccess || hipEventElapsedTime(&t, ev.first, ev.second) != hipSuccess) {
            clslam::set_error("conv_profile_end: %s", hipGetErrorString(hipGetLastError()));
            rc = CLSLAM_ERR_LAUNCH;
        }
        if (n < capacity) ms[n] = t;
        ++n;
        hipEventDestroy(ev.first); hipEventDestroy(ev.second);
    }
#endif
    clslam::g_prof.clear();
    *count = n;
    return rc;
}

extern "C" void* clslam_handoff_event_create(void) {
#if CLSLAM_DEVICE_BUILD
    hipEvent_t e = nullptr;
    if (hipEventCreateWithFlags(&e, hipEventDisableTiming) != hipSuccess) {
        clslam::set_error("handoff_event_create: %s", hipGetErrorString(hipGetLastError()));
        return nullptr;
    }
    return (void*)e;
#else
    return nullptr;
#endif
}

extern "C" void clslam_handoff_event_destroy(void* event) {
#if CLSLAM_DEVICE_BUILD
    if (event) (void)hipEventDestroy((hipEvent_t)event);
#else
    (void)event;
#endif
}

extern "C" int clslam_handoff_arm(void* event) {
    CLSLAM_REQUIRE(event, "handoff_arm: null event");
    clslam::g_handoff = (hipEvent_t)event;
    return CLSLAM_OK;
}

extern "C" int clslam_handoff_wait(void* event, void* producer_stream, void* consumer_stream) {
    CLSLAM_REQUIRE(event, "handoff_wait: null event");
#if CLSLAM_DEVICE_BUILD
    hipEvent_t e = (hipEvent_t)event;
    if (clslam::g_handoff == e) {
        clslam::g_handoff = nullptr;
        if (hipEventRecord(e, (hipStream_t)producer_stream) != hipSuccess) {
            clslam::set_error("handoff_wait: hipEventRecord: %s", hipGetErrorString(hipGetLastError()));
            return CLSLAM_ERR_LAUNCH;
        }
    }
    if (hipStreamWaitEvent((hipStream_t)consumer_stream, e, 0) != hipSuccess) {
        clslam::set_error("handoff_wait: hipStreamWaitEvent: %s", hipGetErrorString(hipGetLastError()));
        return CLSLAM_ERR_LAUNCH;
    }
#else
    (void)producer_stream; (void)consumer_stream;
    if (clslam::g_handoff == (hipEvent_t)event) clslam::g_handoff = nullptr;
#endif
    return CLSLAM_OK;
}

extern "C" int clslam_version(void) { return 106; }
#ifndef CLSLAM_BUILD_ID
#define CLSLAM_BUILD_ID "unstamped"
#endif
extern "C" const char* clslam_build_id(void) { return CLSLAM_BUILD_ID; }
extern "C" const char* clslam_last_error(void) { return clslam::g_err; }
extern "C" const char* clslam_last_error_string(void) { return clslam::g_err; }
extern "C" int clslam_is_device_build(void) { return CLSLAM_DEVICE_BUILD; }
```

cl-slam_amd/csrc/common.h:

```cpp
#pragma once
#include <hip/hip_runtime.h>
#if CLSLAM_DEVICE_BUILD
#include <hip/hip_ext.h>
#endif
#include <clslam/intrin.h>

#include <algorithm>

#include "../../include/clslam_hip.h"

namespace clslam {

void set_error(const char* fmt, ...);
int check_launch(const char* what);

#define CLSLAM_REQUIRE(cond, ...)                     \
    do {                                              \
        if (!(cond)) {                                \
            ::clslam::set_error(__VA_ARGS__);         \
            return CLSLAM_ERR_INVALID;                \
        }                                             \
    } while (0)

__device__ __forceinline__ int reflect_idx(int i, int n) {
    i = i < 0 ? -i : i;
    return i >= n ? 2 * n - 2 - i : i;
}

__device__ __forceinline__ float apply_act(float v, int act) {
    if (act == CLSLAM_ACT_RELU) return v > 0.f ? v : 0.f;
    if (act == CLSLAM_ACT_ELU) return v > 0.f ? v : expm1f(v);
    if (act == CLSLAM_ACT_HSWISH) return v * fminf(fmaxf(v + 3.f, 0.f), 6.f) / 6.f;
    if (act == CLSLAM_ACT_HSIGMOID) return fminf(fmaxf(v + 3.f, 0.f), 6.f) / 6.f;
    return v;
}

__device__ __forceinline__ float act_grad_from_output(float y, int act) {
    if (act == CLSLAM_ACT_RELU) return y > 0.f ? 1.f : 0.f;
    if (act == CLSLAM_ACT_ELU) return y > 0.f ? 1.f : y + 1.f;
    return 1.f;
}

__device__ __forceinline__ int xcd_remap(int bid, int nblk) {
    const int q = nblk >> 3, r = nblk & 7;
    const int xcd = bid & 7, idx = bid >> 3;
    return (xcd < r ? xcd * (q + 1) : r * (q + 1) + (xcd - r) * q) + idx;
}

inline int cdiv(int a, int b) { return (a + b - 1) / b; }

bool profile_next_events(hipEvent_t* start, hipEvent_t* stop);
hipEvent_t take_handoff_event();

template <typename F, typename Arg>
inline void conv_launch(F kernel, int nblk, hipStream_t stream, const Arg& k) {
#if CLSLAM_DEVICE_BUILD
    hipEvent_t e0, e1;
    if (profile_next_events(&e0, &e1)) {
        hipExtLaunchKernelGGL(kernel, dim3(nblk), dim3(256), 0, stream, e0, e1, 0, k);
        return;
    }
#endif
    hipLaunchKernelGGL(kernel, dim3(nblk), dim3(256), 0, stream, k);
}

}
```

cl-slam_amd/csrc/conv_fwd.hip:

```cpp
#include "common.h"

#include <type_traits>

namespace clslam {

struct ConvK {
    const float* __restrict__ src_a;
    const float* __restrict__ src_b;
    const float* __restrict__ wgt;
    const float* __restrict__ scale;
    const float* __restrict__ shift;
    const float* __restrict__ residual;
    const float* __restrict__ actgrad_src;
    float* __restrict__ out;
    int actgrad_kind;
    int B, Hi, Wi, Ca, Cb, Ho, Wo, Cout;
    int ksize, stride, pad, pad_mode, ups, act;
    int M, tilesM, tilesN, nblk;
};

template <int BM, int BN, int BK, int MF, int WGM>
__global__ __launch_bounds__(256) void conv_igemm_kernel(ConvK p) {
    constexpr int LDA = BK + 4;
    constexpr int WGN = 4 / WGM;
    constexpr int WM = BM / WGM, WN = BN / WGN;
    constexpr int TM = WM / MF, TN = WN / MF;
    constexpr int KG = 64 / MF;
    constexpr int KSTEP = KG * 4;
    constexpr int F4_ROW = BK / 4;
    constexpr int A_IT = (BM * F4_ROW + 255) / 256;
    constexpr int B_IT = (BN * F4_ROW + 255) / 256;
    constexpr int NACC = MF == 32 ? 16 : 4;
    static_assert(WM % MF == 0 && WN % MF == 0 && BK % KSTEP == 0, "tile shape");

    __shared__ __attribute__((aligned(16))) float As[2][BM * LDA];
    __shared__ __attribute__((aligned(16))) float Bs[2][BN * LDA];

    const int tid = threadIdx.x;
    const int lane = tid & 63, wave = tid >> 6;
    const int wm0 = (wave / WGN) * WM, wn0 = (wave % WGN) * WN;

    const int logical = xcd_remap((int)blockIdx.x, p.nblk);
    const int tn = logical / p.tilesM, tm = logical - tn * p.tilesM;
    const int m0 = tm * BM, n0 = tn * BN;

    const int Cin = p.Ca + p.Cb;
    const int taps = p.ksize * p.ksize;
    const int HA = p.ups ? (p.Hi >> 1) : p.Hi, WA = p.ups ? (p.Wi >> 1) : p.Wi;

    int a_b[A_IT], a_iy0[A_IT], a_ix0[A_IT];
    bool a_ok[A_IT];
#pragma unroll
    for (int it = 0; it < A_IT; ++it) {
        const int f = tid + it * 256;
        const int row = f / F4_ROW;
        const int m = m0 + row;
        a_ok[it] = (f < BM * F4_ROW) && (m < p.M);
        const int mm = a_ok[it] ? m : 0;
        const int b = mm / (p.Ho * p.Wo);
        const int r = mm - b * (p.Ho * p.Wo);
        const int oy = r / p.Wo, ox = r - oy * p.Wo;
        a_b[it] = b;
        a_iy0[it] = oy * p.stride - p.pad;
        a_ix0[it] = ox * p.stride - p.pad;
    }

    float4 ra[A_IT], rb[B_IT];
    bool ra_ok[A_IT];
    const int chunks_per_tap = Cin / BK;
    const int niter = taps * chunks_per_tap;

    auto load_global = [&](int iter) {
        const int tap = iter / chunks_per_tap;
        const int c0 = (iter - tap * chunks_per_tap) * BK;
        const int ky = tap / p.ksize, kx = tap - ky * p.ksize;
#pragma unroll
        for (int it = 0; it < A_IT; ++it) {
            const int f = tid + it * 256;
            const int c = c0 + (f % F4_ROW) * 4;
            int iy = a_iy0[it] + ky, ix = a_ix0[it] + kx;
            bool ok = a_ok[it];
            if (p.pad_mode == CLSLAM_PAD_REFLECT) {
                iy = reflect_idx(iy, p.Hi);
                ix = reflect_idx(ix, p.Wi);
            } else {
                ok = ok && iy >= 0 && iy < p.Hi && ix >= 0 && ix < p.Wi;
            }
            const int sy = p.ups ? (iy >> 1) : iy, sx = p.ups ? (ix >> 1) : ix;
            const size_t oa = ok ? ((size_t)(a_b[it] * HA + sy) * WA + sx) * p.Ca : 0;
            const size_t ob = ok ? ((size_t)(a_b[it] * p.Hi + iy) * p.Wi + ix) * p.Cb : 0;
            const float* ptr = (c < p.Ca) ? p.src_a + oa + c : p.src_b + ob + (c - p.Ca);
            ra[it] = *reinterpret_cast<const float4*>(ptr);
            ra_ok[it] = ok;
        }
#pragma unroll
        for (int it = 0; it < B_IT; ++it) {
            const int f = tid + it * 256;
            const int row = f / F4_ROW;
            const int n = n0 + row;
            const bool okb = (f < BN * F4_ROW) && (n < p.Cout);
            rb[it] = *reinterpret_cast<const float4*>(p.wgt + ((size_t)(okb ? n : 0) * taps + tap) * Cin + c0 + (f % F4_ROW) * 4);
        }
    };
    auto store_lds = [&](int buf) {
#pragma unroll
        for (int it = 0; it < A_IT; ++it) {
            const int f = tid + it * 256;
            float4 v = ra[it];
            if (!ra_ok[it]) v = make_float4(0.f, 0.f, 0.f, 0.f);
            if (f < BM * F4_ROW)
                *reinterpret_cast<float4*>(&As[buf][(f / F4_ROW) * LDA + (f % F4_ROW) * 4]) = v;
        }
#pragma unroll
        for (int it = 0; it < B_IT; ++it) {
            const int f = tid + it * 256;
            float4 v = rb[it];
            if (n0 + f / F4_ROW >= p.Cout) v = make_float4(0.f, 0.f, 0.f, 0.f);
            if (f < BN * F4_ROW)
                *reinterpret_cast<float4*>(&Bs[buf][(f / F4_ROW) * LDA + (f % F4_ROW) * 4]) = v;
        }
    };

    typedef float accv __attribute__((ext_vector_type(NACC)));
    accv acc[TM][TN];
#pragma unroll
    for (int i = 0; i < TM; ++i)
#pragma unroll
        for (int j = 0; j < TN; ++j)
#pragma unroll
            for (int r = 0; r < NACC; ++r) acc[i][j][r] = 0.f;

    const int frow = lane % MF;
    const int kg = lane / MF;

    load_global(0);
    store_lds(0);
    __syncthreads();

    for (int iter = 0; iter < niter; ++iter) {
        const int buf = iter & 1;
        if (iter + 1 < niter) load_global(iter + 1);
#pragma unroll
        for (int kk = 0; kk < BK / KSTEP; ++kk) {
            float4 fa[TM], fb[TN];
#pragma unroll
            for (int i = 0; i < TM; ++i)
                fa[i] = *reinterpret_cast<const float4*>(&As[buf][(wm0 + i * MF + frow) * LDA + kk * KSTEP + kg * 4]);
#pragma unroll
            for (int j = 0; j < TN; ++j)
                fb[j] = *reinterpret_cast<const float4*>(&Bs[buf][(wn0 + j * MF + frow) * LDA + kk * KSTEP + kg * 4]);
#pragma unroll
            for (int t = 0; t < 4; ++t) {
#pragma unroll
                for (int i = 0; i < TM; ++i) {
                    const float av = t == 0 ? fa[i].x : t == 1 ? fa[i].y : t == 2 ? fa[i].z : fa[i].w;
#pragma unroll
                    for (int j = 0; j < TN; ++j) {
                        const float bv = t == 0 ? fb[j].x : t == 1 ? fb[j].y : t == 2 ? fb[j].z : fb[j].w;
                        if constexpr (MF == 32) acc[i][j] = mfma_32x32x2(av, bv, acc[i][j]);
                        else acc[i][j] = mfma_16x16x4(av, bv, acc[i][j]);
                    }
                }
            }
        }
        if (iter + 1 < niter) store_lds(buf ^ 1);
        __syncthreads();
    }

    auto element = [&](int i, int j, int r, bool& ok) -> size_t {
        int row;
        if constexpr (MF == 32) row = (r & 3) + 8 * (r >> 2) + 4 * (lane >> 5);
        else row = 4 * (lane >> 4) + r;
        const int m = m0 + wm0 + i * MF + row;
        const int n = n0 + wn0 + j * MF + (lane % MF);
        ok = m < p.M && n < p.Cout;
        return (size_t)min(m, p.M - 1) * p.Cout + min(n, p.Cout - 1);
    };
    float sc[TN], sh[TN];
#pragma unroll
    for (int j = 0; j < TN; ++j) {
        const int n = min(n0 + wn0 + j * MF + (lane % MF), p.Cout - 1);
        sc[j] = p.scale ? p.scale[n] : 1.f;
        sh[j] = p.shift ? p.shift[n] : 0.f;
    }
    float resq[TM][TN][NACC], agq[TM][TN][NACC];
    const bool has_res = p.residual != nullptr, has_ag = p.actgrad_src != nullptr;
#pragma unroll
    for (int i = 0; i < TM; ++i)
#pragma unroll
        for (int j = 0; j < TN; ++j)
#pragma unroll
            for (int r = 0; r < NACC; ++r) { resq[i][j][r] = 0.f; agq[i][j][r] = 1.f; }
    if (has_res) {
#pragma unroll
        for (int i = 0; i < TM; ++i)
#pragma unroll
            for (int j = 0; j < TN; ++j)
#pragma unroll
                for (int r = 0; r < NACC; ++r) { bool ok; resq[i][j][r] = p.residual[element(i, j, r, ok)]; }
    }
    if (has_ag) {
#pragma unroll
        for (int i = 0; i < TM; ++i)
#pragma unroll
            for (int j = 0; j < TN; ++j)
#pragma unroll
                for (int r = 0; r < NACC; ++r) { bool ok; agq[i][j][r] = p.actgrad_src[element(i, j, r, ok)]; }
    }
    auto values = [&](auto act_tag) {
        constexpr int ACT = decltype(act_tag)::value;
#pragma unroll
        for (int i = 0; i < TM; ++i)
#pragma unroll
            for (int j = 0; j < TN; ++j)
#pragma unroll
                for (int r = 0; r < NACC; ++r) {
                    const float v = acc[i][j][r] * sc[j] + sh[j] + resq[i][j][r];
                    acc[i][j][r] = ACT < 0 ? apply_act(v, p.act) : apply_act(v, ACT);
                }
    };
    if (p.act == CLSLAM_ACT_RELU) values(std::integral_constant<int, CLSLAM_ACT_RELU>{});
    else if (p.act == CLSLAM_ACT_NONE) values(std::integral_constant<int, CLSLAM_ACT_NONE>{});
    else if (p.act == CLSLAM_ACT_ELU) values(std::integral_constant<int, CLSLAM_ACT_ELU>{});
    else values(std::integral_constant<int, -1>{});
    if (has_ag) {
#pragma unroll
        for (int i = 0; i < TM; ++i)
#pragma unroll
            for (int j = 0; j < TN; ++j)
#pragma unroll
                for (int r = 0; r < NACC; ++r) acc[i][j][r] *= act_grad_from_output(agq[i][j][r], p.actgrad_kind);
    }
#pragma unroll
    for (int i = 0; i < TM; ++i)
#pragma unroll
        for (int j = 0; j < TN; ++j)
#pragma unroll
            for (int r = 0; r < NACC; ++r) {
                bool ok;
                const size_t o = element(i, j, r, ok);
                if (ok) p.out[o] = acc[i][j][r];
            }
}

template <int BM, int BN, int BK, int MF, int WGM>
static int launch_conv(ConvK k, hipStream_t stream) {
    k.tilesM = cdiv(k.M, BM);
    k.tilesN = cdiv(k.Cout, BN);
    k.nblk = k.tilesM * k.tilesN;
    conv_launch(conv_igemm_kernel<BM, BN, BK, MF, WGM>, k.nblk, stream, k);
    return check_launch("conv_igemm");
}

}

namespace clslam { int conv3x3_patch_dispatch(const clslam_conv_desc* d, int cfg, hipStream_t stream);
                   int conv3x3_sk_dispatch(const clslam_conv_desc* d, int cfg, hipStream_t stream);
                   int conv3x3_wino_dispatch(const clslam_conv_desc* d, hipStream_t stream);
                   int conv3x3_wino_supported(const clslam_conv_desc* d);
                   int conv3x3_wino_units_per_group(const clslam_conv_desc* d); }

using namespace clslam;

extern "C" int clslam_conv2d_pick_config(const clslam_conv_desc* d) {
    const int Cin = d->ch_a + d->ch_b;
    const int M = d->batch * d->out_h * d->out_w;
    const bool bk32 = (Cin % 32 == 0) && (d->ch_b == 0 || d->ch_a % 32 == 0);
    if (d->config != -2 && d->workspace != nullptr && conv3x3_wino_supported(d) && Cin >= 64 && d->ch_out >= 64 && !getenv("CLSLAM_NO_WINOGRAD")) {
        static const int min_units = getenv("CLSLAM_WINO_MIN_UNITS") ? atoi(getenv("CLSLAM_WINO_MIN_UNITS")) : 8;
        const int upg = conv3x3_wino_units_per_group(d);
        if (upg >= min_units || (d->out_w <= 24 && upg >= 5)) return 40;
    }
    const bool sk_ok = d->workspace != nullptr && d->ksize == 3 && d->ch_out >= 64 && !getenv("CLSLAM_NO_STREAMK") &&
                       d->config != -2;
    static const int sk_all = getenv("CLSLAM_SK_ALL") ? atoi(getenv("CLSLAM_SK_ALL")) : 0;
    if (sk_ok && sk_all && Cin >= sk_all) return d->stride == 2 ? (d->out_w <= 44 ? 31 : 30) : (d->out_w <= 44 ? 32 : 30);
    static const int sk_fill_min = getenv("CLSLAM_SK_FILL") ? atoi(getenv("CLSLAM_SK_FILL")) : 0;
    const bool sk_fill = (long long)d->batch * cdiv(d->out_h * d->out_w, 128) * cdiv(d->ch_out, 64) >= sk_fill_min;
    const int px = d->out_h * d->out_w;
    auto full_enough = [&](int cfg) {
        const int covered = cfg == 32 ? cdiv(px, 128) * 128 : cfg == 33 ? cdiv(px, 64) * 64
                                      : cdiv(d->out_h, cfg == 30 ? 8 : 4) * (cfg == 30 ? 8 : 4) * cdiv(d->out_w, 16) * 16;
        return px * 10 >= covered * 4;
    };
    int sk = 0;
    if (sk_ok && sk_fill && d->stride == 1 && d->out_h == d->in_h + 2 * d->pad - 2 && d->out_w == d->in_w + 2 * d->pad - 2) {
        const long long units128 = (long long)d->batch * cdiv(px, 128) * cdiv(d->ch_out, 64) * (Cin / 16);
        const bool tie_case = Cin < 512 && d->ch_out >= 256 && d->out_w > 24 && units128 >= 1280 && M < 4000;
        if (d->out_w <= 44 && Cin >= 256 && !tie_case) sk = units128 >= 1280 ? 32 : 33;
        else if (d->out_w <= 84 && d->out_w > 44 && Cin >= 256 && M >= 4000) sk = 30;
    }
    if (sk_ok && sk_fill && d->stride == 2 && d->out_w <= 24 && Cin >= 256) {
        const int spanned = std::min(d->out_h, (127 + d->out_w - 1) / d->out_w + 1);
        const bool band_fits = ((spanned - 1) * 2 + 3) * ((d->out_w - 1) * 2 + 3) <= 544;
        const long long units = (long long)d->batch * cdiv(px, 128) * cdiv(d->ch_out, 64) * (Cin / 16);
        if (units >= 512) sk = (band_fits && !getenv("CLSLAM_NO_SK_RUN_S2")) ? 32 : 30;
        else sk = 31;
    }
    if (sk_ok && sk_fill && d->stride == 2 && d->out_w > 24 && d->out_w <= 84 && M >= 16000) sk = 30;
    if (sk && full_enough(sk)) return sk;
    if (d->ksize == 3 && d->stride == 1 && d->out_h == d->in_h + 2 * d->pad - 2 && d->out_w == d->in_w + 2 * d->pad - 2) {
        if (d->out_w <= 24) return 22;
        static const bool pick_v2 = !getenv("CLSLAM_PICK_V1");
        if (pick_v2 && d->ch_out >= 32) {
            const double cov20 = (double)px / ((double)cdiv(d->out_h, 8) * 8 * cdiv(d->out_w, 16) * 16);
            const double cov21 = (double)px / ((double)cdiv(d->out_h, 4) * 4 * cdiv(d->out_w, 16) * 16);
            const long long nblk20 = (long long)d->batch * cdiv(d->out_h, 8) * cdiv(d->out_w, 16) * cdiv(d->ch_out, 16);
            if (cov21 > 1.04 * cov20) return 21;
            if (M >= 4000) return nblk20 < 1000 ? 21 : 20;
            return nblk20 >= 400 ? 20 : 21;
        }
        return M >= 16000 ? 20 : 21;
    }
    if (d->ksize == 3 && d->stride == 2 && d->out_h == (d->in_h + 2 * d->pad - 3) / 2 + 1 && d->out_w == (d->in_w + 2 * d->pad - 3) / 2 + 1)
        return 23;
    if (d->ch_out % 32 != 0) return bk32 ? 6 : 4;
    if (!bk32) return 5;
    if (d->ch_out == 32) return 3;
    if (d->ch_out == 64 && M >= 30000) return 3;
    return 2;
}

extern "C" int clslam_conv2d(const clslam_conv_desc* d, void* stream_) {
    hipStream_t stream = (hipStream_t)stream_;
    CLSLAM_REQUIRE(d, "conv2d: null descriptor");
    if (d->batch == 0 || d->out_h * d->out_w == 0) return CLSLAM_OK;
    CLSLAM_REQUIRE(d->src_a && d->weight && d->out, "conv2d: null pointer");
    const int Cin = d->ch_a + d->ch_b;
    CLSLAM_REQUIRE(d->ksize == 1 || d->ksize == 3, "conv2d: ksize %d unsupported", d->ksize);
    CLSLAM_REQUIRE(Cin % 16 == 0 && d->ch_a % 16 == 0 && d->ch_out % 16 == 0,
                   "conv2d: channels must be multiples of 16 (Ca=%d Cb=%d Cout=%d)", d->ch_a, d->ch_b, d->ch_out);
    CLSLAM_REQUIRE(!d->upsample_a || (d->in_h % 2 == 0 && d->in_w % 2 == 0), "conv2d: upsample needs even dims");
    CLSLAM_REQUIRE(d->pad_mode == CLSLAM_PAD_ZERO || (d->pad < d->in_h && d->pad < d->in_w), "conv2d: reflect pad too large");
    CLSLAM_REQUIRE(d->ch_b == 0 || d->src_b, "conv2d: src_b missing");
    CLSLAM_REQUIRE(d->stride >= 1 && d->out_h == (d->in_h + 2 * d->pad - d->ksize) / d->stride + 1 &&
                       d->out_w == (d->in_w + 2 * d->pad - d->ksize) / d->stride + 1,
                   "conv2d: output size %dx%d does not match input %dx%d, ksize %d, stride %d, pad %d", d->out_h, d->out_w, d->in_h,
                   d->in_w, d->ksize, d->stride, d->pad);
    ConvK k;
    k.src_a = d->src_a; k.src_b = d->src_b; k.wgt = d->weight; k.scale = d->scale; k.shift = d->shift;
    k.residual = d->residual; k.out = d->out; k.actgrad_src = d->actgrad_src; k.actgrad_kind = d->actgrad_kind;
    k.B = d->batch; k.Hi = d->in_h; k.Wi = d->in_w; k.Ca = d->ch_a; k.Cb = d->ch_b;
    k.Ho = d->out_h; k.Wo = d->out_w; k.Cout = d->ch_out;
    k.ksize = d->ksize; k.stride = d->stride; k.pad = d->pad; k.pad_mode = d->pad_mode;
    k.ups = d->upsample_a; k.act = d->act;
    k.M = d->batch * d->out_h * d->out_w;
    k.tilesM = k.tilesN = k.nblk = 0;
    if (k.M == 0) return CLSLAM_OK;
    int cfg = d->config;
    const bool bk32 = (Cin % 32 == 0) && (d->ch_b == 0 || d->ch_a % 32 == 0);
    if (cfg < 0) cfg = clslam_conv2d_pick_config(d);
    if (cfg == 40) {
        const int rc = conv3x3_wino_dispatch(d, stream);
        if (rc == CLSLAM_OK || d->config >= 0) return rc;
        clslam_conv_desc tiled = *d;
        tiled.config = -2;
        cfg = clslam_conv2d_pick_config(&tiled);
    }
    if (cfg >= 30) {
        const int rc = conv3x3_sk_dispatch(d, cfg, stream);
        if (rc == CLSLAM_OK || d->config >= 0) return rc;
        clslam_conv_desc tiled = *d;
        tiled.config = -2;
        cfg = clslam_conv2d_pick_config(&tiled);
    }
    if (cfg >= 10) return conv3x3_patch_dispatch(d, cfg, stream);
    const bool need32 = (cfg <= 3 || cfg == 6);
    if (need32 && !bk32) { set_error("conv2d: config %d needs channel multiples of 32", cfg); return CLSLAM_ERR_INVALID; }
    if ((cfg == 0 || cfg == 1) && d->ch_out % 32 != 0) { set_error("conv2d: config %d needs Cout %% 32 == 0", cfg); return CLSLAM_ERR_INVALID; }
    switch (cfg) {
        case 0: return launch_conv<128, 64, 32, 32, 2>(k, stream);
        case 1: return launch_conv<64, 64, 32, 32, 2>(k, stream);
        case 2: return launch_conv<32, 32, 32, 16, 2>(k, stream);
        case 3: return launch_conv<64, 32, 32, 16, 2>(k, stream);
        case 4: return launch_conv<128, 16, 16, 16, 4>(k, stream);
        case 5: return launch_conv<64, 32, 16, 16, 2>(k, stream);
        case 6: return launch_conv<128, 16, 32, 16, 4>(k, stream);
        default: set_error("conv2d: unknown config %d", cfg); return CLSLAM_ERR_INVALID;
    }
}
```

cl-slam_amd/csrc/conv_patch.hip:

```cpp
#include "common.h"

#include <type_traits>

namespace clslam {

constexpr int kSplitKMaxTiles = 16384;

struct PatchK {
    const float* __restrict__ src_a;
    const float* __restrict__ src_b;
    const float* __restrict__ wgt;
    const float* __restrict__ scale;
    const float* __restrict__ shift;
    const float* __restrict__ residual;
    const float* __restrict__ actgrad_src;
    float* __restrict__ out;
    int actgrad_kind;
    int B, Hi, Wi, Ca, Cb, Ho, Wo, Cout;
    int pad, pad_mode, ups, act;
    int tilesX, tilesY, tilesN, nblk;
    int n_fastest;
    int ksplit;
    float* ws;
    unsigned* counters;
    size_t ws_bytes;
};

constexpr int run_pp(int bm) { return bm <= 64 ? 224 : 320; }

template <int TH, int TW, int BN, int BK, int MF, int WGM, bool RUN, int LDPAD, int S, bool SK>
__global__ __launch_bounds__(256) void conv3x3_patch_kernel(PatchK p) {
    constexpr int BM = TH * TW;
    constexpr int PH = (TH - 1) * S + 3, PW = (TW - 1) * S + 3, PP = RUN ? run_pp(BM) : PH * PW;
    static_assert(!RUN || S == 1, "run tiles are stride-1 only");
    constexpr int LD = BK + LDPAD;
    constexpr int WGN = 4 / WGM;
    constexpr int WM = BM / WGM, WN = BN / WGN;
    constexpr int TM = WM / MF, TN = WN / MF;
    constexpr int KG = 64 / MF, KSTEP = KG * 4;
    constexpr int F4 = BK / 4;
    constexpr int P_SLOTS = PP * F4, W_SLOTS = 9 * BN * F4;
    constexpr int P_IT = (P_SLOTS + 255) / 256, W_IT = (W_SLOTS + 255) / 256;
    constexpr int NACC = MF == 32 ? 16 : 4;
    static_assert(WM % MF == 0 && WN % MF == 0 && BK % KSTEP == 0 && TW % 8 == 0, "tile shape");

    __shared__ __attribute__((aligned(16))) float Ps[PP * LD];
    __shared__ __attribute__((aligned(16))) float Wsm[9 * BN * LD];

    const int tid = threadIdx.x, lane = tid & 63, wave = tid >> 6;
    const int wm0 = (wave / WGN) * WM, wn0 = (wave % WGN) * WN;

    int logical = xcd_remap((int)blockIdx.x, p.nblk);
    const int tiles_total = SK ? p.nblk / p.ksplit : p.nblk;
    const int split = SK ? logical / tiles_total : 0;
    if (SK) logical -= split * tiles_total;
    const int tile_id = logical;
    int tn;
    if (p.n_fastest) { tn = logical % p.tilesN; logical /= p.tilesN; }
    const int tx = logical % p.tilesX; logical /= p.tilesX;
    const int ty = logical % p.tilesY; logical /= p.tilesY;
    const int b = logical % p.B;
    if (!p.n_fastest) tn = logical / p.B;
    const int n0 = tn * BN;
    const int m0 = tx * BM;
    const int oy0 = RUN ? m0 / p.Wo : ty * TH, ox0 = RUN ? 0 : tx * TW;
    const int pw = RUN ? p.Wo + 2 : PW;
    const int ph = RUN ? (min(p.Ho * p.Wo, m0 + BM) - 1) / p.Wo - oy0 + 3 : PH;
    const int npatch = ph * pw;
    const int Cin = p.Ca + p.Cb;
    const int HA = p.ups ? (p.Hi >> 1) : p.Hi, WA = p.ups ? (p.Wi >> 1) : p.Wi;

    int offA[P_IT], offB[P_IT];
#pragma unroll
    for (int it = 0; it < P_IT; ++it) {
        const int f = tid + it * 256;
        const int pp = f / F4;
        offA[it] = -1; offB[it] = -1;
        if (f < P_SLOTS && pp < npatch) {
            const int pr = pp / pw, pc = pp - pr * pw;
            int iy = oy0 * S - p.pad + pr, ix = ox0 * S - p.pad + pc;
            bool ok = true;
            if (p.pad_mode == CLSLAM_PAD_REFLECT) {
                iy = reflect_idx(iy, p.Hi); ix = reflect_idx(ix, p.Wi);
                iy = min(max(iy, 0), p.Hi - 1); ix = min(max(ix, 0), p.Wi - 1);
            } else {
                ok = iy >= 0 && iy < p.Hi && ix >= 0 && ix < p.Wi;
            }
            if (ok) {
                const int sy = p.ups ? (iy >> 1) : iy, sx = p.ups ? (ix >> 1) : ix;
                offA[it] = ((b * HA + sy) * WA + sx) * p.Ca;
                offB[it] = ((b * p.Hi + iy) * p.Wi + ix) * p.Cb;
            }
        }
    }

    bool okP[P_IT], okW[W_IT];
    const float* wptr[W_IT];
#pragma unroll
    for (int it = 0; it < P_IT; ++it) {
        okP[it] = offA[it] >= 0;
        if (!okP[it]) { offA[it] = 0; offB[it] = 0; }
    }
#pragma unroll
    for (int it = 0; it < W_IT; ++it) {
        const int f = tid + it * 256;
        const int c4 = f % F4;
        const int n = (f / F4) % BN;
        const int tap = f / (F4 * BN);
        okW[it] = (f < W_SLOTS) && (n0 + n < p.Cout);
        wptr[it] = p.wgt + ((size_t)(okW[it] ? n0 + n : 0) * 9 + (okW[it] ? tap : 0)) * Cin + c4 * 4;
    }
    float4 rp[P_IT], rw[W_IT];
    auto load_global = [&](int c0) {
#pragma unroll
        for (int it = 0; it < P_IT; ++it) {
            const int f = tid + it * 256;
            const int c = c0 + (f % F4) * 4;
            const float* ptr = c < p.Ca ? p.src_a + offA[it] + c : p.src_b + offB[it] + (c - p.Ca);
            rp[it] = *reinterpret_cast<const float4*>(ptr);
        }
#pragma unroll
        for (int it = 0; it < W_IT; ++it) rw[it] = *reinterpret_cast<const float4*>(wptr[it] + c0);
    };
    auto store_lds = [&]() {
#pragma unroll
        for (int it = 0; it < P_IT; ++it) {
            const int f = tid + it * 256;
            float4 v = rp[it];
            if (!okP[it]) v = make_float4(0.f, 0.f, 0.f, 0.f);
            if (f < P_SLOTS) *reinterpret_cast<float4*>(&Ps[(f / F4) * LD + (f % F4) * 4]) = v;
        }
#pragma unroll
        for (int it = 0; it < W_IT; ++it) {
            const int f = tid + it * 256;
            float4 v = rw[it];
            if (!okW[it]) v = make_float4(0.f, 0.f, 0.f, 0.f);
            if (f < W_SLOTS) *reinterpret_cast<float4*>(&Wsm[(f / F4) * LD + (f % F4) * 4]) = v;
        }
    };

    typedef float accv __attribute__((ext_vector_type(NACC)));
    constexpr int NCH = (TM * TN == 1) ? 2 : 1;
    accv acc[TM][TN][NCH];
#pragma unroll
    for (int i = 0; i < TM; ++i)
#pragma unroll
        for (int j = 0; j < TN; ++j)
#pragma unroll
            for (int h = 0; h < NCH; ++h)
#pragma unroll
                for (int r = 0; r < NACC; ++r) acc[i][j][h][r] = 0.f;

    const int frow = lane % MF, kg = lane / MF;
    int prow[TM];
#pragma unroll
    for (int i = 0; i < TM; ++i) {
        const int m = wm0 + i * MF + frow;
        if constexpr (RUN) {
            const int mm = min(m0 + m, p.Ho * p.Wo - 1);
            prow[i] = (mm / p.Wo - oy0) * pw + (mm % p.Wo);
        } else {
            prow[i] = (m / TW) * S * PW + (m % TW) * S;
        }
    }

    const int cps = SK ? (Cin / BK + p.ksplit - 1) / p.ksplit : Cin / BK;
    const int c_begin = SK ? split * cps * BK : 0, c_end = SK ? min(Cin, c_begin + cps * BK) : Cin;
    if (c_begin < c_end) load_global(c_begin);
    float scv[TN], shv[TN];
#pragma unroll
    for (int j = 0; j < TN; ++j) {
        const int n = min(n0 + wn0 + j * MF + (lane % MF), p.Cout - 1);
        scv[j] = p.scale ? p.scale[n] : 1.f;
        shv[j] = p.shift ? p.shift[n] : 0.f;
    }
    constexpr bool PRE_RES = (TM * TN * NACC <= 4) && !SK && RUN;
    float resv[PRE_RES ? TM * TN * NACC : 1];
    if constexpr (PRE_RES) {
#pragma unroll
        for (int r = 0; r < NACC; ++r) {
            const int m = wm0 + 4 * (lane >> 4) + r;
            int oy, ox;
            bool ok = true;
            if constexpr (RUN) {
                const int mm = min(m0 + m, p.Ho * p.Wo - 1);
                oy = mm / p.Wo; ox = mm % p.Wo;
            } else {
                oy = min(oy0 + m / TW, p.Ho - 1); ox = min(ox0 + m % TW, p.Wo - 1);
            }
            const int n = min(n0 + wn0 + (lane % MF), p.Cout - 1);
            resv[r] = p.residual ? p.residual[(((size_t)b * p.Ho + oy) * p.Wo + ox) * p.Cout + n] : 0.f;
        }
    }
    for (int c0 = c_begin; c0 < c_end; c0 += BK) {
        __syncthreads();
        store_lds();
        __syncthreads();
        if (c0 + BK < c_end) load_global(c0 + BK);
#pragma unroll
        for (int tap = 0; tap < 9; ++tap) {
            const int ky = tap / 3, kx = tap - ky * 3;
#pragma unroll
            for (int kk = 0; kk < BK / KSTEP; ++kk) {
                float4 fa[TM], fb[TN];
#pragma unroll
                for (int i = 0; i < TM; ++i)
                    fa[i] = *reinterpret_cast<const float4*>(&Ps[(prow[i] + ky * pw + kx) * LD + kk * KSTEP + kg * 4]);
#pragma unroll
                for (int j = 0; j < TN; ++j)
                    fb[j] = *reinterpret_cast<const float4*>(&Wsm[((tap * BN) + wn0 + j * MF + frow) * LD + kk * KSTEP + kg * 4]);
#pragma unroll
                for (int t = 0; t < 4; ++t) {
#pragma unroll
                    for (int i = 0; i < TM; ++i) {
                        const float av = t == 0 ? fa[i].x : t == 1 ? fa[i].y : t == 2 ? fa[i].z : fa[i].w;
#pragma unroll
                        for (int j = 0; j < TN; ++j) {
                            const float bv = t == 0 ? fb[j].x : t == 1 ? fb[j].y : t == 2 ? fb[j].z : fb[j].w;
                            accv& a = acc[i][j][t % NCH];
                            if constexpr (MF == 32) a = mfma_32x32x2(av, bv, a);
                            else a = mfma_16x16x4(av, bv, a);
                        }
                    }
                }
            }
        }
    }

    if constexpr (SK) {
        __shared__ int s_last;
        float* slab = p.ws + ((size_t)split * tiles_total + tile_id) * (BM * BN);
#pragma unroll
        for (int i = 0; i < TM; ++i)
#pragma unroll
            for (int j = 0; j < TN; ++j)
#pragma unroll
                for (int r = 0; r < NACC; ++r) {
                    int row;
                    if constexpr (MF == 32) row = (r & 3) + 8 * (r >> 2) + 4 * (lane >> 5);
                    else row = 4 * (lane >> 4) + r;
                    coherent_store(&slab[(wm0 + i * MF + row) * BN + wn0 + j * MF + (lane % MF)],
                                   NCH == 2 ? acc[i][j][0][r] + acc[i][j][NCH - 1][r] : acc[i][j][0][r]);
                }
        stores_complete();
        __syncthreads();
        if (tid == 0) s_last = (coherent_inc(&p.counters[tile_id]) == (unsigned)(p.ksplit - 1));
        __syncthreads();
        if (!s_last) return;
        if (tid == 0) coherent_store_u32(&p.counters[tile_id], 0u);
        const float* gather = p.ws + (size_t)tile_id * (BM * BN);
#pragma unroll
        for (int i = 0; i < TM; ++i)
#pragma unroll
            for (int j = 0; j < TN; ++j)
#pragma unroll
                for (int r = 0; r < NACC; ++r) {
                    int row;
                    if constexpr (MF == 32) row = (r & 3) + 8 * (r >> 2) + 4 * (lane >> 5);
                    else row = 4 * (lane >> 4) + r;
                    const int e = (wm0 + i * MF + row) * BN + wn0 + j * MF + (lane % MF);
                    float sum = 0.f;
                    for (int sp = 0; sp < p.ksplit; ++sp) sum += coherent_load(&gather[(size_t)sp * tiles_total * (BM * BN) + e]);
                    acc[i][j][0][r] = sum;
                    if (NCH == 2) acc[i][j][NCH - 1][r] = 0.f;
                }
    }

    constexpr int NE = TM * TN * NACC;
    auto element = [&](int i, int j, int r, bool& ok) -> size_t {
        int row;
        if constexpr (MF == 32) row = (r & 3) + 8 * (r >> 2) + 4 * (lane >> 5);
        else row = 4 * (lane >> 4) + r;
        const int m = wm0 + i * MF + row;
        const int n = n0 + wn0 + j * MF + (lane % MF);
        int oy, ox;
        if constexpr (RUN) {
            ok = (m0 + m < p.Ho * p.Wo) && n < p.Cout;
            const int mm = min(m0 + m, p.Ho * p.Wo - 1);
            oy = mm / p.Wo; ox = mm % p.Wo;
        } else {
            oy = oy0 + m / TW; ox = ox0 + m % TW;
            ok = oy < p.Ho && ox < p.Wo && n < p.Cout;
            oy = min(oy, p.Ho - 1); ox = min(ox, p.Wo - 1);
        }
        return (((size_t)b * p.Ho + oy) * p.Wo + ox) * p.Cout + min(n, p.Cout - 1);
    };
    float vals[TM][TN][NACC], resq[TM][TN][NACC], agq[TM][TN][NACC];
    const bool has_res = !PRE_RES && p.residual != nullptr, has_ag = p.actgrad_src != nullptr;
#pragma unroll
    for (int i = 0; i < TM; ++i)
#pragma unroll
        for (int j = 0; j < TN; ++j)
#pragma unroll
            for (int r = 0; r < NACC; ++r) {
                if constexpr (PRE_RES) resq[i][j][r] = resv[r];
                else resq[i][j][r] = 0.f;
                agq[i][j][r] = 1.f;
            }
    if (has_res) {
#pragma unroll
        for (int i = 0; i < TM; ++i)
#pragma unroll
            for (int j = 0; j < TN; ++j)
#pragma unroll
                for (int r = 0; r < NACC; ++r) { bool ok; resq[i][j][r] = p.residual[element(i, j, r, ok)]; }
    }
    if (has_ag) {
#pragma unroll
        for (int i = 0; i < TM; ++i)
#pragma unroll
            for (int j = 0; j < TN; ++j)
#pragma unroll
                for (int r = 0; r < NACC; ++r) { bool ok; agq[i][j][r] = p.actgrad_src[element(i, j, r, ok)]; }
    }
    auto values = [&](auto act_tag) {
        constexpr int ACT = decltype(act_tag)::value;
#pragma unroll
        for (int i = 0; i < TM; ++i)
#pragma unroll
            for (int j = 0; j < TN; ++j)
#pragma unroll
                for (int r = 0; r < NACC; ++r) {
                    float v = (NCH == 2 ? acc[i][j][0][r] + acc[i][j][NCH - 1][r] : acc[i][j][0][r]) * scv[j] + shv[j];
                    v += resq[i][j][r];
                    vals[i][j][r] = ACT < 0 ? apply_act(v, p.act) : apply_act(v, ACT);
                }
    };
    if (p.act == CLSLAM_ACT_ELU) values(std::integral_constant<int, CLSLAM_ACT_ELU>{});
    else if (p.act == CLSLAM_ACT_RELU) values(std::integral_constant<int, CLSLAM_ACT_RELU>{});
    else if (p.act == CLSLAM_ACT_NONE) values(std::integral_constant<int, CLSLAM_ACT_NONE>{});
    else values(std::integral_constant<int, -1>{});
    if (has_ag) {
#pragma unroll
        for (int i = 0; i < TM; ++i)
#pragma unroll
            for (int j = 0; j < TN; ++j)
#pragma unroll
                for (int r = 0; r < NACC; ++r) vals[i][j][r] *= act_grad_from_output(agq[i][j][r], p.actgrad_kind);
    }
#pragma unroll
    for (int i = 0; i < TM; ++i)
#pragma unroll
        for (int j = 0; j < TN; ++j)
#pragma unroll
            for (int r = 0; r < NACC; ++r) {
                bool ok;
                const size_t o = element(i, j, r, ok);
                if (ok) p.out[o] = vals[i][j][r];
            }
    (void)NE;
}

template <int TH, int TW, int BN, int BK, int MF, int WGM, bool RUN = false, int LDPAD = 4, int S = 1, bool SKOK = false>
static int launch_patch(PatchK k, hipStream_t stream) {
    if (RUN) {
        const int spanned = (TH * TW - 1 + k.Wo - 1) / k.Wo + 1;
        if ((spanned + 2) * (k.Wo + 2) > run_pp(TH * TW)) { set_error("conv2d: image too wide for run tiles (Wo=%d)", k.Wo); return CLSLAM_ERR_INVALID; }
    }
    k.tilesX = RUN ? cdiv(k.Ho * k.Wo, TH * TW) : cdiv(k.Wo, TW);
    k.tilesY = RUN ? 1 : cdiv(k.Ho, TH);
    k.tilesN = cdiv(k.Cout, BN);
    const int tiles = k.tilesX * k.tilesY * k.tilesN * k.B;
    const int chunks = (k.Ca + k.Cb) / BK;
    int ksplit = 1;
    if (const char* e = getenv("CLSLAM_SPLITK")) { if (k.ws) ksplit = std::max(1, std::min(atoi(e), chunks)); }
    if (!SKOK || (size_t)ksplit * tiles * (TH * TW * BN) * sizeof(float) > k.ws_bytes || tiles > kSplitKMaxTiles) ksplit = 1;
    k.ksplit = ksplit;
    k.nblk = tiles * ksplit;
    k.n_fastest = ((size_t)k.Cout * 9 * (k.Ca + k.Cb) * 4 <= (size_t)(2 << 20)) ? 1 : 0;
    if (const char* e = getenv("CLSLAM_N_FASTEST")) k.n_fastest = atoi(e);
    if constexpr (SKOK) {
        if (ksplit > 1) {
            conv_launch(conv3x3_patch_kernel<TH, TW, BN, BK, MF, WGM, RUN, LDPAD, S, true>, k.nblk, stream, k);
            return check_launch("conv3x3_patch(split-K)");
        }
    }
    conv_launch(conv3x3_patch_kernel<TH, TW, BN, BK, MF, WGM, RUN, LDPAD, S, false>, k.nblk, stream, k);
    return check_launch("conv3x3_patch");
}

int conv3x3_patch_dispatch(const clslam_conv_desc* d, int cfg, hipStream_t stream) {
    const int st = d->stride;
    if (d->ksize != 3 || (st != 1 && st != 2) || (st == 2) != (cfg == 23) || ((cfg == 24 || cfg == 25) && (d->ch_a + d->ch_b) % 32 != 0) ||
        (cfg == 26 && d->ch_out % 32 != 0)) {
        set_error("conv2d: patch configs need a 3x3 conv with stride 1 (configs 10-22) or 2 (config 23)");
        return CLSLAM_ERR_INVALID;
    }
    if (d->out_h != (d->in_h + 2 * d->pad - 3) / st + 1 || d->out_w != (d->in_w + 2 * d->pad - 3) / st + 1) {
        set_error("conv2d: inconsistent output size for the patch kernel");
        return CLSLAM_ERR_INVALID;
    }
    PatchK k;
    k.src_a = d->src_a; k.src_b = d->src_b; k.wgt = d->weight; k.scale = d->scale; k.shift = d->shift;
    k.residual = d->residual; k.actgrad_src = d->actgrad_src; k.out = d->out; k.actgrad_kind = d->actgrad_kind;
    k.B = d->batch; k.Hi = d->in_h; k.Wi = d->in_w; k.Ca = d->ch_a; k.Cb = d->ch_b; k.Ho = d->out_h; k.Wo = d->out_w;
    k.Cout = d->ch_out; k.pad = d->pad; k.pad_mode = d->pad_mode; k.ups = d->upsample_a; k.act = d->act;
    k.tilesX = k.tilesY = k.tilesN = k.nblk = 0; k.n_fastest = 0;
    k.ksplit = 1; k.ws = nullptr; k.counters = nullptr; k.ws_bytes = 0;
    if (d->workspace && d->workspace_bytes > (size_t)kSplitKMaxTiles * sizeof(unsigned)) {
        k.counters = (unsigned*)d->workspace;
        k.ws = (float*)((char*)d->workspace + (size_t)kSplitKMaxTiles * sizeof(unsigned));
        k.ws_bytes = d->workspace_bytes - (size_t)kSplitKMaxTiles * sizeof(unsigned);
    }
    switch (cfg) {
        case 10: return launch_patch<8, 16, 64, 16, 32, 2>(k, stream);
        case 11: return launch_patch<8, 16, 32, 16, 32, 4>(k, stream);
        case 12: return launch_patch<8, 16, 16, 16, 16, 4>(k, stream);
        case 13: return launch_patch<4, 16, 64, 16, 32, 2>(k, stream);
        case 14: return launch_patch<8, 16, 16, 32, 16, 4>(k, stream);
        case 15: return launch_patch<16, 16, 16, 16, 16, 4>(k, stream);
        case 16: return launch_patch<8, 16, 32, 16, 16, 4>(k, stream);
        case 17: return launch_patch<4, 16, 16, 16, 16, 4>(k, stream);
        case 18: return launch_patch<4, 16, 16, 16, 16, 4, true>(k, stream);
        case 19: return launch_patch<8, 16, 16, 16, 16, 4, true>(k, stream);
        case 20: return launch_patch<8, 16, 16, 16, 16, 4, false, 8, 1, true>(k, stream);
        case 21: return launch_patch<4, 16, 16, 16, 16, 4, false, 8, 1, true>(k, stream);
        case 22: return launch_patch<4, 16, 16, 16, 16, 4, true, 8, 1, true>(k, stream);
        case 23: return launch_patch<4, 16, 16, 16, 16, 4, false, 8, 2, true>(k, stream);
        case 24: return launch_patch<4, 16, 16, 32, 16, 4, true, 8>(k, stream);
        case 25: return launch_patch<4, 16, 16, 32, 16, 4, false, 8>(k, stream);
        case 26: return launch_patch<4, 8, 32, 16, 16, 2, false, 8>(k, stream);
        default: set_error("conv2d: unknown patch config %d", cfg); return CLSLAM_ERR_INVALID;
    }
}

}
```

cl-slam_amd/csrc/conv_sk.hip:

```cpp
#include "common.h"

#include <mutex>
#include <unordered_map>

namespace clslam {

__device__ float g_zero_page[64];

constexpr int kSkFlagOffset = 8192;
constexpr int kSkMaxGroups = 4096;
constexpr int kSkSlabOffsetBytes = 64 << 10;
constexpr unsigned kSkSpinLimit = 1u << 22;

struct SkK {
    const float* __restrict__ src_a;
    const float* __restrict__ src_b;
    const float* __restrict__ wgt;
    const float* __restrict__ scale;
    const float* __restrict__ shift;
    const float* __restrict__ residual;
    const float* __restrict__ actgrad_src;
    float* __restrict__ out;
    int actgrad_kind;
    int B, Hi, Wi, Ca, Cb, Ho, Wo, Cout;
    int pad, pad_mode, ups, act;
    int tilesX, tilesY, tilesN, tiles, NC, G;
    long long units;
    float* slabs;
    unsigned* flags;
    int b_fastest;
    unsigned epoch;
    int dbg;
};

constexpr int sk_run_pp(int bm, int s = 1) { return s == 2 ? 544 : (bm <= 64 ? 336 : 416); }

template <int TH, int TW, bool RUN, int S, int BN, int NWM, int NWN>
__global__ __launch_bounds__(NWM * NWN * 64) void conv3x3_sk_kernel(SkK p) {
    constexpr int NW = NWM * NWN, NT = NW * 64;
    constexpr int BM = TH * TW;
    constexpr int TM = BM / (16 * NWM), TN = BN / (16 * NWN);
    constexpr int PH = (TH - 1) * S + 3, PW = (TW - 1) * S + 3;
    constexpr int PP = RUN ? sk_run_pp(BM, S) : (PH * PW + 15) / 16 * 16;
    constexpr int NPP = PP / 16, NWP = 9 * BN / 16;
    constexpr int STAGE = (PP + 9 * BN) * 16;
    static_assert(BM % (16 * NWM) == 0 && BN % (16 * NWN) == 0 && TW % 16 == 0, "tile shape");

    __shared__ __attribute__((aligned(1024))) float lds[2 * STAGE];
    __shared__ int s_flag_ok;

    const int tid = threadIdx.x, lane = tid & 63, wave = tid >> 6;
    const int wm = wave / NWN, wn = wave % NWN;
    const int frow = lane & 15, kg = lane >> 4;
    const int Cin = p.Ca + p.Cb;
    const int HA = p.ups ? (p.Hi >> 1) : p.Hi, WA = p.ups ? (p.Wi >> 1) : p.Wi;

#if CLSLAM_DEVICE_BUILD
    const int grp = xcd_remap((int)blockIdx.x, p.G);
#else
    const int grp = (int)blockIdx.x;
#endif
    const long long u0 = (long long)grp * p.units / p.G, u1 = (long long)(grp + 1) * p.units / p.G;
    if (u0 >= u1) return;
    if (tid == 0) s_flag_ok = 1;

    const int drow = lane >> 2;
    const int dslot = (lane & 3) ^ (((drow >> 2) & 1) << 1);
    const int wlane_off = drow * 9 * Cin + dslot * 4;

    auto decode_tile = [&](int t, int& tn, int& tx, int& ty, int& b) {
        if (p.b_fastest) {
            b = t % p.B; t /= p.B;
            tn = t % p.tilesN; t /= p.tilesN;
            tx = t % p.tilesX; ty = t / p.tilesX;
        } else {
            tn = t % p.tilesN; t /= p.tilesN;
            tx = t % p.tilesX; t /= p.tilesX;
            ty = t % p.tilesY; b = t / p.tilesY;
        }
    };

    constexpr int MYP = (NPP + NW - 1) / NW, MYW = (NWP + NW - 1) / NW;
    int offA[MYP], offB[MYP];
    int dma_n0 = 0;
    auto dma_setup_tile = [&](int t) {
        int tn, tx, ty, b;
        decode_tile(t, tn, tx, ty, b);
        dma_n0 = tn * BN;
        const int m0 = tx * BM;
        const int oy0 = RUN ? m0 / p.Wo : ty * TH, ox0 = RUN ? 0 : tx * TW;
        const int pw = RUN ? (p.Wo - 1) * S + 3 : PW;
        const int ph = RUN ? ((min(p.Ho * p.Wo, m0 + BM) - 1) / p.Wo - oy0) * S + 3 : PH;
#pragma unroll
        for (int k = 0; k < MYP; ++k) {
            const int piece = wave + k * NW;
            const int row = piece * 16 + drow;
            offA[k] = -1; offB[k] = -1;
            if (piece < NPP && row < ph * pw) {
                const int pr = row / pw, pc = row - pr * pw;
                int iy = oy0 * S - p.pad + pr, ix = ox0 * S - p.pad + pc;
                bool ok = true;
                if (p.pad_mode == CLSLAM_PAD_REFLECT) {
                    iy = reflect_idx(iy, p.Hi); ix = reflect_idx(ix, p.Wi);
                    iy = min(max(iy, 0), p.Hi - 1); ix = min(max(ix, 0), p.Wi - 1);
                } else {
                    ok = iy >= 0 && iy < p.Hi && ix >= 0 && ix < p.Wi;
                }
                if (ok) {
                    const int sy = p.ups ? (iy >> 1) : iy, sx = p.ups ? (ix >> 1) : ix;
                    offA[k] = ((b * HA + sy) * WA + sx) * p.Ca;
                    offB[k] = ((b * p.Hi + iy) * p.Wi + ix) * p.Cb;
                }
            }
        }
    };
    auto dma_issue = [&](int c, float* stage) {
        if (p.dbg & 8) return;
        const int c0 = c * 16;
        const bool from_a = c0 < p.Ca;
#pragma unroll
        for (int k = 0; k < MYP; ++k) {
            const int piece = wave + k * NW;
            if (piece < NPP) {
                const int off = from_a ? offA[k] : offB[k];
                const float* src = off < 0 ? g_zero_page + dslot * 4
                                           : (from_a ? p.src_a + off + c0 : p.src_b + off + (c0 - p.Ca)) + dslot * 4;
                lds_dma16(src, stage + piece * 256);
            }
        }
#pragma unroll
        for (int k = 0; k < MYW; ++k) {
            const int piece = wave + k * NW;
            if (piece < NWP) {
                const int tap = piece / (BN / 16), nb = (piece % (BN / 16)) * 16;
                const bool ok = dma_n0 + nb + drow < p.Cout;
                const float* src = ok ? p.wgt + (size_t)((dma_n0 + nb) * 9 + tap) * Cin + c0 + wlane_off : g_zero_page + dslot * 4;
                lds_dma16(src, stage + PP * 16 + piece * 256);
            }
        }
    };

    const int bslot = (kg ^ (((frow >> 2) & 1) << 1)) * 4;
    int brow[TN];
#pragma unroll
    for (int j = 0; j < TN; ++j) brow[j] = ((wn * TN + j) * 16 + frow) * 16 + bslot;

    f32x4 acc[TM][TN];
    auto zero_acc = [&]() {
#pragma unroll
        for (int i = 0; i < TM; ++i)
#pragma unroll
            for (int j = 0; j < TN; ++j)
#pragma unroll
                for (int r = 0; r < 4; ++r) acc[i][j][r] = 0.f;
    };
    zero_acc();

    int prow[TM];
    int c_pw = PW;
    auto cmp_setup_tile = [&](int t) {
        if constexpr (RUN) {
            int tn, tx, ty, b;
            decode_tile(t, tn, tx, ty, b);
            const int m0 = tx * BM;
            const int oy0 = m0 / p.Wo;
            c_pw = (p.Wo - 1) * S + 3;
#pragma unroll
            for (int i = 0; i < TM; ++i) {
                const int mm = min(m0 + (wm * TM + i) * 16 + frow, p.Ho * p.Wo - 1);
                prow[i] = (mm / p.Wo - oy0) * S * c_pw + (mm % p.Wo) * S;
            }
        } else {
#pragma unroll
            for (int i = 0; i < TM; ++i) {
                const int m = (wm * TM + i) * 16 + frow;
                prow[i] = (m / TW) * S * PW + (m % TW) * S;
            }
        }
    };

    auto load_frags = [&](const float* Ps, const float* Ws, int tap, float4 (&fa)[TM], float4 (&fb)[TN]) {
        const int ky = tap / 3, kx = tap - ky * 3;
#pragma unroll
        for (int i = 0; i < TM; ++i) {
            const int r = prow[i] + ky * c_pw + kx;
            fa[i] = *reinterpret_cast<const float4*>(&Ps[r * 16 + ((kg ^ (((r >> 2) & 1) << 1)) << 2)]);
        }
#pragma unroll
        for (int j = 0; j < TN; ++j) fb[j] = *reinterpret_cast<const float4*>(&Ws[tap * BN * 16 + brow[j]]);
    };
    auto compute = [&](const float* stage, auto&& between) {
        const float* Ps = stage;
        const float* Ws = stage + PP * 16;
        float4 fa[2][TM], fb[2][TN];
        if (!(p.dbg & 4)) load_frags(Ps, Ws, 0, fa[0], fb[0]);
        between();
        if (p.dbg & 4) return;
#pragma unroll
        for (int tap = 0; tap < 9; ++tap) {
            if (tap < 8) load_frags(Ps, Ws, tap + 1, fa[(tap + 1) & 1], fb[(tap + 1) & 1]);
            sched_fence();
            const float4(&ca)[TM] = fa[tap & 1];
            const float4(&cb)[TN] = fb[tap & 1];
#pragma unroll
            for (int t = 0; t < 4; ++t)
#pragma unroll
                for (int i = 0; i < TM; ++i) {
                    const float xv = t == 0 ? ca[i].x : t == 1 ? ca[i].y : t == 2 ? ca[i].z : ca[i].w;
#pragma unroll
                    for (int j = 0; j < TN; ++j) {
                        const float wv = t == 0 ? cb[j].x : t == 1 ? cb[j].y : t == 2 ? cb[j].z : cb[j].w;
                        acc[i][j] = mfma_16x16x4(wv, xv, acc[i][j]);
                    }
                }
            sched_fence();
        }
    };

    bool publish_pending = false;
    auto finish = [&](int t, int c_lo, int c_hi) {
        const bool owner = c_hi == p.NC;
        if ((p.dbg & 2) && (!owner || c_lo > 0)) return;
        if (!owner) {
            float* slab = p.slabs + (size_t)grp * (BM * BN) + (size_t)wave * (TM * TN * 256) + lane * 4;
            mfma_results_settle();
#pragma unroll
            for (int i = 0; i < TM; ++i)
#pragma unroll
                for (int j = 0; j < TN; ++j) coherent_store4(slab + (i * TN + j) * 256, acc[i][j]);
            vmem_drain_visible();
            publish_pending = true;
            return;
        }
        if (c_lo > 0) {
            const long long tile_first = (long long)t * p.NC;
            int ncon = 0;
            for (int g2 = grp - 1; g2 >= 0 && (long long)(g2 + 1) * p.units / p.G > tile_first; --g2) ++ncon;
            for (int q = tid; q < ncon; q += NT) {
                unsigned spins = 0;
                while (coherent_load_u32(&p.flags[grp - 1 - q]) != p.epoch && ++spins < kSkSpinLimit) spin_pause();
                if (spins >= kSkSpinLimit) s_flag_ok = 0;
                uncounted_flag_store(&p.flags[grp - 1 - q], 0u);
            }
            __syncthreads();
            const float poison = s_flag_ok ? 0.f : __builtin_nanf("");
            const float* slab0 = p.slabs + (size_t)wave * (TM * TN * 256) + lane * 4;
            for (int base = 0; base < ncon; base += 4) {
                const float* sp[4];
#pragma unroll
                for (int q = 0; q < 4; ++q) sp[q] = slab0 + (size_t)(grp - 1 - min(base + q, ncon - 1)) * (BM * BN);
                f32x4 part[4][TM * TN];
                if constexpr (TM * TN == 4) coherent_load4x4_x4(sp[0], sp[1], sp[2], sp[3], part[0], part[1], part[2], part[3]);
                else if constexpr (TM * TN == 2) coherent_load4x2_x4(sp[0], sp[1], sp[2], sp[3], part[0], part[1], part[2], part[3]);
                else {
#pragma unroll
                    for (int q = 0; q < 4; ++q)
#pragma unroll
                        for (int r = 0; r < TM * TN; r += 2) coherent_load4x2(sp[q] + r * 256, part[q][r], part[q][r + 1]);
                }
#pragma unroll
                for (int q = 0; q < 4; ++q)
                    if (base + q < ncon) {
#pragma unroll
                        for (int i = 0; i < TM; ++i)
#pragma unroll
                            for (int j = 0; j < TN; ++j)
#pragma unroll
                                for (int r = 0; r < 4; ++r) acc[i][j][r] += part[q][i * TN + j][r] + poison;
                    }
            }
        }
        if (p.dbg & 1) { if (acc[0][0][0] == 12345.678f) uncounted_flag_store((unsigned*)p.out, 1u); return; }
        int tn, tx, ty, b;
        decode_tile(t, tn, tx, ty, b);
        const int n0 = tn * BN, m0 = tx * BM;
        const int oy0 = RUN ? 0 : ty * TH, ox0 = RUN ? 0 : tx * TW;
        size_t opix[TM];
        bool pix_ok[TM];
#pragma unroll
        for (int i = 0; i < TM; ++i) {
            const int m = (wm * TM + i) * 16 + frow;
            int oy, ox;
            if constexpr (RUN) {
                pix_ok[i] = m0 + m < p.Ho * p.Wo;
                oy = (m0 + m) / p.Wo; ox = (m0 + m) % p.Wo;
            } else {
                oy = oy0 + m / TW; ox = ox0 + m % TW;
                pix_ok[i] = oy < p.Ho && ox < p.Wo;
            }
            opix[i] = (((size_t)b * p.Ho + oy) * p.Wo + ox) * p.Cout;
        }
        const float* extra = p.residual ? p.residual : p.actgrad_src;
        const bool has_res = p.residual != nullptr, has_ag = !has_res && p.actgrad_src != nullptr;
        float4 sc[TN], sh[TN], ex[TM][TN];
        bool ch_ok[TN];
#pragma unroll
        for (int j = 0; j < TN; ++j) {
            const int n = n0 + (wn * TN + j) * 16 + 4 * kg;
            ch_ok[j] = n < p.Cout;
            const int nc = ch_ok[j] ? n : 0;
            sc[j] = p.scale ? *reinterpret_cast<const float4*>(p.scale + nc) : make_float4(1.f, 1.f, 1.f, 1.f);
            sh[j] = p.shift ? *reinterpret_cast<const float4*>(p.shift + nc) : make_float4(0.f, 0.f, 0.f, 0.f);
#pragma unroll
            for (int i = 0; i < TM; ++i)
                ex[i][j] = (extra && ch_ok[j] && pix_ok[i]) ? *reinterpret_cast<const float4*>(extra + opix[i] + n)
                                                            : make_float4(0.f, 0.f, 0.f, 0.f);
        }
        float4 res[TM][TN];
#pragma unroll
        for (int j = 0; j < TN; ++j)
#pragma unroll
            for (int i = 0; i < TM; ++i) {
                float4 v = make_float4(acc[i][j][0] * sc[j].x + sh[j].x, acc[i][j][1] * sc[j].y + sh[j].y,
                                       acc[i][j][2] * sc[j].z + sh[j].z, acc[i][j][3] * sc[j].w + sh[j].w);
                const float4 e = ex[i][j];
                v.x += has_res ? e.x : 0.f; v.y += has_res ? e.y : 0.f; v.z += has_res ? e.z : 0.f; v.w += has_res ? e.w : 0.f;
                v.x = apply_act(v.x, p.act); v.y = apply_act(v.y, p.act); v.z = apply_act(v.z, p.act); v.w = apply_act(v.w, p.act);
                v.x *= has_ag ? act_grad_from_output(e.x, p.actgrad_kind) : 1.f; v.y *= has_ag ? act_grad_from_output(e.y, p.actgrad_kind) : 1.f;
                v.z *= has_ag ? act_grad_from_output(e.z, p.actgrad_kind) : 1.f; v.w *= has_ag ? act_grad_from_output(e.w, p.actgrad_kind) : 1.f;
                res[i][j] = v;
            }
        vmem_drain_visible();
#pragma unroll
        for (int j = 0; j < TN; ++j) {
            const int n = n0 + (wn * TN + j) * 16 + 4 * kg;
#pragma unroll
            for (int i = 0; i < TM; ++i)
                if (ch_ok[j] && pix_ok[i]) uncounted_store4(p.out + opix[i] + n, res[i][j]);
        }
    };

    const int t_hi = (int)((u1 - 1) / p.NC), t_lo = (int)(u0 / p.NC);
    auto seg_lo = [&](int t) { return (int)(max(u0, (long long)t * p.NC) - (long long)t * p.NC); };
    auto seg_hi = [&](int t) { return (int)(min(u1, (long long)(t + 1) * p.NC) - (long long)t * p.NC); };

    int dt = t_hi, dc = seg_lo(t_hi);
    int ct = t_hi, cc = dc, c_lo = dc, c_hi = seg_hi(t_hi);
    dma_setup_tile(dt);
    cmp_setup_tile(ct);
    dma_issue(dc, lds);
    const int nunits = (int)(u1 - u0);
    for (int k = 0; k < nunits; ++k) {
        dma_wait_all();
        wg_barrier_keep_dma();
        if (publish_pending) {
            if (tid == 0) uncounted_flag_store(&p.flags[grp], p.epoch);
            publish_pending = false;
        }
        compute(lds + (k & 1) * STAGE, [&]() {
            if (k + 1 < nunits) {
                if (++dc >= seg_hi(dt)) { --dt; dc = seg_lo(dt); dma_setup_tile(dt); }
                dma_issue(dc, lds + ((k + 1) & 1) * STAGE);
            }
        });
        if (++cc >= c_hi) {
            finish(ct, c_lo, c_hi);
            if (k + 1 < nunits) {
                --ct; c_lo = seg_lo(ct); c_hi = seg_hi(ct); cc = c_lo;
                cmp_setup_tile(ct);
                zero_acc();
            }
        }
    }
    if (publish_pending) {
        stores_complete();
        __syncthreads();
        if (tid == 0) uncounted_flag_store(&p.flags[grp], p.epoch);
    }
}

int sk_device_cus() {
#if CLSLAM_DEVICE_BUILD
    static thread_local int cached_dev = -1, cached_cus = 0;
    int dev = 0;
    if (hipGetDevice(&dev) != hipSuccess) return 256;
    if (dev != cached_dev) {
        int n = 0;
        if (hipDeviceGetAttribute(&n, hipDeviceAttributeMultiprocessorCount, dev) != hipSuccess || n <= 0) n = 256;
        cached_dev = dev; cached_cus = n;
    }
    return cached_cus;
#else
    return 256;
#endif
}

unsigned sk_next_epoch(const void* workspace) {
    static std::mutex mu;
    static std::unordered_map<const void*, unsigned> epochs;
    std::lock_guard<std::mutex> lock(mu);
    unsigned& e = epochs[workspace];
    e = e == 0xFFFFFFFFu ? 1u : e + 1u;
    return e;
}

template <int TH, int TW, bool RUN, int S, int BN, int NWM, int NWN>
static int launch_sk(SkK k, const clslam_conv_desc* d, hipStream_t stream) {
    constexpr int BM = TH * TW;
    if (RUN) {
        const int spanned = std::min(k.Ho, (BM - 1 + k.Wo - 1) / k.Wo + 1);
        if (((spanned - 1) * S + 3) * ((k.Wo - 1) * S + 3) > sk_run_pp(BM, S)) { set_error("conv2d: image too wide for stream-K run tiles (Wo=%d, stride %d)", k.Wo, S); return CLSLAM_ERR_INVALID; }
    }
    k.tilesX = RUN ? cdiv(k.Ho * k.Wo, BM) : cdiv(k.Wo, TW);
    k.tilesY = RUN ? 1 : cdiv(k.Ho, TH);
    k.tilesN = cdiv(k.Cout, BN);
    k.tiles = k.tilesX * k.tilesY * k.tilesN * k.B;
    k.NC = (k.Ca + k.Cb) / 16;
    k.units = (long long)k.tiles * k.NC;
    k.b_fastest = ((size_t)k.Cout * 9 * (k.Ca + k.Cb) > (size_t)k.B * k.Hi * k.Wi * (k.Ca + k.Cb)) ? 1 : 0;
    if (const char* e = getenv("CLSLAM_SK_B_FASTEST")) k.b_fastest = atoi(e);
    constexpr int PHs = (TH - 1) * S + 3, PWs = (TW - 1) * S + 3;
    constexpr int PPs = RUN ? sk_run_pp(BM, S) : (PHs * PWs + 15) / 16 * 16;
    constexpr size_t lds_bytes = (size_t)2 * (PPs + 9 * BN) * 64 + 16;
    constexpr int per_cu = (int)std::max<size_t>(1, std::min<size_t>((size_t)(163840 / lds_bytes), (size_t)(2048 / (NWM * NWN * 64))));
    int G = (d->cu_limit > 0 ? std::min(d->cu_limit, sk_device_cus()) : sk_device_cus()) * per_cu;
    if (const char* e = getenv("CLSLAM_SK_GROUPS")) G = std::max(1, atoi(e));
    G = (int)std::min<long long>(std::min(G, kSkMaxGroups), k.units);
    k.G = G;
    const size_t need = (size_t)kSkSlabOffsetBytes + (size_t)G * BM * BN * sizeof(float);
    if (!d->workspace || d->workspace_bytes < need) {
        set_error("conv2d: the stream-K kernel needs a zero-filled workspace of %zu bytes on the launching stream", need);
        return CLSLAM_ERR_INVALID;
    }
    k.flags = (unsigned*)d->workspace + kSkFlagOffset;
    k.epoch = sk_next_epoch(d->workspace);
    k.slabs = (float*)((char*)d->workspace + kSkSlabOffsetBytes);
    auto kern = conv3x3_sk_kernel<TH, TW, RUN, S, BN, NWM, NWN>;
#if CLSLAM_DEVICE_BUILD
    hipEvent_t e0, e1;
    if (profile_next_events(&e0, &e1)) {
        hipExtLaunchKernelGGL(kern, dim3(G), dim3(NWM * NWN * 64), 0, stream, e0, e1, 0, k);
        return check_launch("conv3x3_sk");
    }
#endif
    hipLaunchKernelGGL(kern, dim3(G), dim3(NWM * NWN * 64), 0, stream, k);
    return check_launch("conv3x3_sk");
}

int conv3x3_sk_dispatch(const clslam_conv_desc* d, int cfg, hipStream_t stream) {
    const int st = d->stride;
    if (d->ksize != 3 || (st != 1 && st != 2)) { set_error("conv2d: stream-K configs need a 3x3 conv with stride 1 or 2"); return CLSLAM_ERR_INVALID; }
    SkK k;
    k.src_a = d->src_a; k.src_b = d->src_b; k.wgt = d->weight; k.scale = d->scale; k.shift = d->shift;
    k.residual = d->residual; k.actgrad_src = d->actgrad_src; k.out = d->out; k.actgrad_kind = d->actgrad_kind;
    k.B = d->batch; k.Hi = d->in_h; k.Wi = d->in_w; k.Ca = d->ch_a; k.Cb = d->ch_b; k.Ho = d->out_h; k.Wo = d->out_w;
    k.Cout = d->ch_out; k.pad = d->pad; k.pad_mode = d->pad_mode; k.ups = d->upsample_a; k.act = d->act;
    k.tilesX = k.tilesY = k.tilesN = k.tiles = k.NC = k.G = 0; k.units = 0; k.slabs = nullptr; k.flags = nullptr;
    k.epoch = 1u; k.b_fastest = 0;
    k.dbg = 0;
    if (const char* e = getenv("CLSLAM_SK_DBG")) k.dbg = atoi(e);
    const bool s2 = st == 2;
    switch (cfg) {
        case 30: return s2 ? launch_sk<8, 16, false, 2, 64, 4, 2>(k, d, stream) : launch_sk<8, 16, false, 1, 64, 4, 2>(k, d, stream);
        case 31: return s2 ? launch_sk<4, 16, false, 2, 64, 4, 2>(k, d, stream) : launch_sk<4, 16, false, 1, 64, 4, 2>(k, d, stream);
        case 32: return s2 ? launch_sk<8, 16, true, 2, 64, 4, 2>(k, d, stream) : launch_sk<8, 16, true, 1, 64, 4, 2>(k, d, stream);
        case 33: if (s2) break; return launch_sk<4, 16, true, 1, 64, 4, 2>(k, d, stream);
        case 34: return s2 ? launch_sk<8, 16, false, 2, 32, 4, 1>(k, d, stream) : launch_sk<8, 16, false, 1, 32, 4, 1>(k, d, stream);
        case 35: return s2 ? launch_sk<4, 16, false, 2, 32, 2, 2>(k, d, stream) : launch_sk<4, 16, false, 1, 32, 2, 2>(k, d, stream);
        case 36: if (s2) break; return launch_sk<4, 16, true, 1, 32, 2, 2>(k, d, stream);
        case 37: if (s2) break; return launch_sk<8, 16, true, 1, 32, 4, 1>(k, d, stream);
        default: break;
    }
    set_error("conv2d: unknown stream-K config %d (stride %d)", cfg, st);
    return CLSLAM_ERR_INVALID;
}

}
```

include/clslam_hip.h:

```cpp
#ifndef CLSLAM_HIP_H
#define CLSLAM_HIP_H

#include <stddef.h>
#include <stdint.h>

#ifdef __cplusplus
extern "C" {
#endif

#define CLSLAM_OK 0
#define CLSLAM_ERR_INVALID (-1)
#define CLSLAM_ERR_LAUNCH (-2)

#define CLSLAM_ACT_NONE 0
#define CLSLAM_ACT_RELU 1
#define CLSLAM_ACT_ELU 2
#define CLSLAM_ACT_HSWISH 3
#define CLSLAM_ACT_HSIGMOID 4

#define CLSLAM_PAD_ZERO 0
#define CLSLAM_PAD_REFLECT 1

#define CLSLAM_ABI_VERSION 106
int clslam_version(void);
const char* clslam_last_error(void);
const char* clslam_last_error_string(void);
const char* clslam_build_id(void);
int clslam_is_device_build(void);

typedef struct clslam_conv_desc {
    const float* src_a;
    const float* src_b;
    const float* weight;
    const float* scale;
    const float* shift;
    const float* residual;
    float* out;
    int32_t batch, in_h, in_w, ch_a, ch_b, out_h, out_w, ch_out;
    int32_t ksize, stride, pad, pad_mode, upsample_a, act;
    int32_t config;
    const float* actgrad_src;
    int32_t actgrad_kind;
    void* workspace;
    size_t workspace_bytes;
    const float* weight_wino;
    int32_t cu_limit;
} clslam_conv_desc;
int clslam_conv2d(const clslam_conv_desc* desc, void* stream);
int clslam_conv2d_pick_config(const clslam_conv_desc* desc);
size_t clslam_wino_weight_size(int ch_out, int ch_in);
int clslam_wino_weight_transform(const float* w, float* u, int ch_out, int ch_in, void* stream);


int clslam_weight_transpose(const float* w, float* wt, int ch_out, int taps, int ch_in, int ch_in_sel,
                            void* stream);
typedef struct clslam_transpose_item {
    const float* w;
    float* wt;
    int ch_out, taps, ch_in, ch_in_sel;
} clslam_transpose_item;
int clslam_weight_transpose_multi(const clslam_transpose_item* items, int nitems, void* stream);
int clslam_fold_blocks(int batch, int h, int w, int ch, int pool);
int clslam_fold_act_grad(const float* dxp, const float* yout, float* dz, float* bias_partial, int batch, int h, int w,
                         int ch, int ch_stride, int border, int pool, int act, const float* disp_dz, const float* disp_w,
                         void* stream);
int clslam_wgrad_splits(const clslam_conv_desc* desc, int target_blocks);
int clslam_conv_wgrad(const clslam_conv_desc* desc, const float* dz, float* partial, int splits, void* stream);
int clslam_wgrad_patch_supported(const clslam_conv_desc* desc);
int clslam_wgrad_patch_splits(const clslam_conv_desc* desc, int target_blocks);
int clslam_conv_wgrad_patch(const clslam_conv_desc* desc, const float* dz, float* partial, int splits, void* stream);
int clslam_reduce_partials(const float* partial, float* out, size_t n, int splits, float scale, void* stream);
int clslam_reduce_multi(const void* items_dev, int nitems, int blocks_per_item, void* stream);
int clslam_reduce_multi_adam(const void* items_dev, int nitems, int blocks_per_item, const float* grad_base, float* param,
                             float* exp_avg, float* exp_avg_sq, double lr, double beta1, double beta2, double eps, int step,
                             const float* guard, void* stream);
int clslam_colsum_blocks(int rows);
int clslam_colsum(const float* x, float* partial, int rows, int ch, void* stream);

int clslam_stem_packed_size(int num_images);
int clslam_stem_pack_weight(const float* weight, float* packed, int num_images, void* stream);
int clslam_stem_conv(const float* img_a, const float* img_b, const float* weight, const float* scale,
                     const float* shift, float* out, int batch, int h, int w, int num_images, void* stream);
int clslam_maxpool3x3s2(const float* in, float* out, int batch, int h, int w, int ch, void* stream);

int clslam_dispconv_fwd(const float* x, const float* w, const float* bias, float* disp, int batch, int h, int wd,
                        int ch, void* stream);
int clslam_dispconv_bwd_data(const float* dz, const float* w, float* dxp, int batch, int h, int wd, int ch,
                             int accumulate, void* stream);
int clslam_dispconv_wgrad_blocks(int pixels);
int clslam_dispconv_wgrad(const float* dz, const float* x, float* partial, int batch, int h, int wd, int ch,
                          void* stream);

int clslam_pose_head_fwd(const float* x, const float* w2, const float* b2, float* mean, float* pose, int n, int hw,
                         void* stream);
int clslam_pose_head_bwd(const float* dpose, const float* x, const float* w2, const float* mean, float* dz1,
                         float* dw2, float* db2, int n, int hw, float grad_scale, void* stream);

int clslam_pose_to_proj(const float* pose, const float* kmat, float* cam_t_cam, float* proj, int batch, void* stream);
int clslam_warp_fwd(const float* disp_s, int h, int w, const float* src_m1, const float* src_p1, const float* inv_k,
                    const float* proj, float* depth, float* warped, int batch, int H, int W, float min_depth,
                    float max_depth, void* stream);
int clslam_warp_fwd_pyramid(const float* const* disp, const float* src_m1, const float* src_p1, const float* inv_k,
                            const float* proj, float* depth, float* warped, int batch, int H, int W, float min_depth,
                            float max_depth, void* stream);
int clslam_warp_fwd_pyramid_range(const float* const* disp, const float* src_m1, const float* src_p1, const float* inv_k,
                                  const float* proj, float* depth, float* warped, int batch, int H, int W, float min_depth,
                                  float max_depth, int scale_lo, int scale_count, void* stream);
int clslam_warp_cells_pyramid(const float* const* disp, const float* inv_k, const float* proj, int* cells, int batch, int H,
                              int W, float min_depth, float max_depth, void* stream);
int clslam_warp_coords_pyramid(const float* const* disp, const float* inv_k, const float* proj, float* coords, int batch, int H,
                               int W, float min_depth, float max_depth, void* stream);
int clslam_warp_bwd_blocks(int H, int W);
int clslam_warp_bwd(const float* dpred, const float* disp_s, int h, int w, const float* src_m1, const float* src_p1,
                    const float* inv_k, const float* proj, float* ddisp_up, double* dp_partial, int batch, int H, int W,
                    float min_depth, float max_depth, void* stream);
int clslam_pose_bwd(const double* dp_partial, int nscale, int nblk, const float* pose, const float* kmat,
                    const double* dist0, const double* dist1, const float* sample_w, float vel_scale, float* dpose,
                    int batch, void* stream);

int clslam_photo_map(const float* pred, const float* target, float* map, float* coef, int npred, int batch, int H,
                     int W, void* stream);
int clslam_automask_blocks(int H, int W);
int clslam_automask(const float* idmap, const float* noise, const float* rpmap, unsigned char* sel, float* partial,
                    int batch, int H, int W, void* stream);
int clslam_automask_pyramid(const float* idmap, const float* noise, const float* rpmap, unsigned char* sel, float* partial,
                            int nscale, int batch, int H, int W, void* stream);
int clslam_disp_mean_pyramid(const float* const* disp, float* psum, int batch, int H, int W, void* stream);
int clslam_photo_automask_pyramid(const float* warped, const float* target, const float* idmap, const float* noise,
                                  unsigned char* sel, float* coef_sel, float* partial, int batch, int H, int W,
                                  void* stream);
int clslam_photo_automask_pyramid_rng(const float* warped, const float* target, const float* idmap, unsigned long long seed,
                                      unsigned long long offset, unsigned char* sel, float* coef_sel, float* partial, int batch,
                                      int H, int W, void* stream);
int clslam_photo_automask_pyramid_range(const float* warped, const float* target, const float* idmap, const float* noise,
                                        unsigned long long seed, unsigned long long offset, unsigned char* sel, float* coef_sel,
                                        float* partial, int batch, int H, int W, int scale_lo, int scale_count, void* stream);
int clslam_tie_break_noise(float* out, size_t npix, unsigned long long seed, unsigned long long offset, void* stream);
int clslam_smooth_intended_chunks(void);
int clslam_smooth_intended_fwd(const float* const* disp, const float* const* rgb0, float* partial, int batch, int H, int W,
                               void* stream);
int clslam_smooth_intended_finalize(const float* partial, const float* means, const float* sample_w, float* losses, float* aux,
                                    int batch, int H, int W, float smooth_scale, void* stream);
int clslam_smooth_intended_bwd(const float* const* disp, const float* const* rgb0, const float* aux, const float* sample_w,
                               float* const* dz, int batch, int H, int W, float smooth_scale, void* stream);
int clslam_loss_bwd2_blocks(int H, int W);
int clslam_loss_bwd2_pyramid(const float* const* disp, const unsigned char* sel, const float* coef_sel, const float* warped,
                             const float* target, const float* src_m1, const float* src_p1, const float* inv_k,
                             const float* proj, const float* sample_w, float* ddisp_up, double* dp_partial, int batch,
                             int H, int W, float min_depth, float max_depth, void* stream);
int clslam_loss_bwd2_pyramid_range(const float* const* disp, const unsigned char* sel, const float* coef_sel, const float* warped,
                                   const float* target, const float* src_m1, const float* src_p1, const float* inv_k,
                                   const float* proj, const float* sample_w, float* ddisp_up, double* dp_partial, int batch,
                                   int H, int W, float min_depth, float max_depth, int scale_lo, int scale_count, void* stream);
int clslam_loss_bwd_blocks(int H, int W);
int clslam_loss_bwd_pyramid(const float* const* disp, const unsigned char* sel, const float* coef, const float* warped,
                            const float* target, const float* src_m1, const float* src_p1, const float* inv_k,
                            const float* proj, const float* sample_w, float* ddisp_up, double* dp_partial, int batch, int H,
                            int W, float min_depth, float max_depth, void* stream);
int clslam_disp_grad_pyramid(const float* ddisp_up, const float* const* disp, const float* smooth_aux, int n_smooth,
                             float* const* dz, int batch, int H, int W, void* stream);
int clslam_disp_grad_pyramid_range(const float* ddisp_up, const float* const* disp, const float* smooth_aux, int n_smooth,
                                   float* const* dz, int batch, int H, int W, int scale_lo, int scale_count, void* stream);
int clslam_disp_mean_chunks(void);
int clslam_disp_mean(const float* disp, float* psum, int batch, int hw, void* stream);
typedef struct clslam_loss_desc {
    const float* partial[4];
    const float* disp[4];
    const float* rgb0[4];
    const float* means[4];
    const float* pose;
    const double* dist0;
    const double* dist1;
    const float* sample_w;
    const float* smooth_w;
    float* losses;
    float* smooth_aux;
    int32_t batch, nblk, H, W, n_smooth;
    float smooth_scale, vel_scale;
} clslam_loss_desc;
int clslam_loss_finalize(const clslam_loss_desc* desc, void* stream);
int clslam_photo_grad(const unsigned char* sel, const float* coef, const float* pred, const float* target,
                      const float* sample_w, float* dpred, int batch, int H, int W, void* stream);
int clslam_disp_grad(const float* ddisp_up, const float* disp, const float* smooth_aux, int n_smooth, float* dz,
                     int batch, int h, int w, int H, int W, void* stream);

int clslam_adam_step(float* param, const float* grad, float* exp_avg, float* exp_avg_sq, size_t n, double lr,
                     double beta1, double beta2, double eps, int step, float grad_scale, const float* guard, void* stream);

int clslam_conv_profile_begin(int max_launches);
int clslam_conv_profile_end(float* ms, int capacity, int* count);

void* clslam_handoff_event_create(void);
void clslam_handoff_event_destroy(void* event);
int clslam_handoff_arm(void* event);
int clslam_handoff_wait(void* event, void* producer_stream, void* consumer_stream);

typedef struct clslam_copy_item {
    const void* src;
    void* dst;
    size_t bytes;
} clslam_copy_item;
int clslam_copy_multi(const clslam_copy_item* items, int nitems, void* stream);

int clslam_ip_scores(const float* db, const float* queries, float* scores, int n, int d, int nq, void* stream);
int clslam_topk_chunks(int n);
int clslam_topk_desc(const float* scores, int n, int nq, int k, float* cand_val, int* cand_idx, float* out_val,
                     int* out_idx, void* stream);
int clslam_l2_normalize_rows(float* x, int n, int d, void* stream);
int clslam_diversity_commit(float* db, float* sim, int ld, unsigned char* occupied, int nslots, int max_slots, int d,
                            int capacity, float threshold, const float* query, const float* scores, int* result,
                            float* similarity, void* stream);

int clslam_lanczos_ksize(int in_size, int out_size);
int clslam_lanczos_plan(int in_size, int out_size, int* bounds, int* coeffs);
int clslam_resize_pass_u8(const unsigned char* src, unsigned char* dst, float* planar, const int* bounds, const int* coeffs,
                          int ksize, int batch, int in_h, int in_w, int ch, int out_size, int axis, void* stream);
int clslam_u8_to_planar_f32(const unsigned char* src, float* planar, int batch, int h, int w, int ch, void* stream);
int clslam_color_jitter_u8(const unsigned char* src, unsigned char* dst, unsigned char* scratch, unsigned long long* lsum,
                           int batch, int h, int w, const int* order, int n_ops, const double* factors, void* stream);

int clslam_color_jitter_f32_blocks(int h, int w);
int clslam_color_jitter_f32(const float* src, float* dst, const void* params, float* partial, int n_images, int h, int w,
                            void* stream);

int clslam_mbv3_stem(const float* img, const float* weight, const float* scale, const float* shift, float* out,
                     int batch, int h, int w, void* stream);
int clslam_dwconv(const float* x, const float* weight, const float* scale, const float* shift, float* out, int batch,
                  int h, int w, int ch, int ksize, int stride, int act, void* stream);
int clslam_avgpool_chunks(int hw);
int clslam_global_avgpool(const float* x, float* out, float* partial, int batch, int hw, int ch, void* stream);
int clslam_se_gate(const float* pool, const float* w1, const float* b1, const float* w2, const float* b2, float* gate,
                   int batch, int ch, int squeeze, void* stream);
int clslam_channel_scale(float* x, const float* gate, int batch, int hw, int ch, void* stream);

int clslam_pgo_edge_eval(const double* est, const int* edge_v, const double* meas, int ne, double* err, double* jac_i,
                         double* jac_j, void* stream);
int clslam_pgo_lin_stride(void);
int clslam_pgo_build_system(const double* est, const int* edge_v, const double* meas, const double* info, const double* huber_delta,
                            int ne, const int* cptr, const int* contrib, const int* diag, int nnzb, int na, double* lin, double* H,
                            double* b, double* scal, void* stream);
int clslam_pgo_solve_workspace(int na);
int clslam_pgo_solve(const double* H, const int* rptr, const int* col, const int* tri, const double* b, double lambda, int na,
                     double tol, int max_iter, double* delta, double* work, double* scal, void* stream);
int clslam_pgo_update_score(const double* est, double* trial, const int* act, int nv, const double* delta, const int* edge_v,
                            const double* meas, const double* info, const double* huber_delta, int ne, int robust, double* scal,
                            int out_index, void* stream);

#define CLSLAM_DEPTH_EVAL_MEDIAN_SCALING 1
#define CLSLAM_DEPTH_EVAL_FROM_DISP 2
#define CLSLAM_DEPTH_EVAL_NO_MAX 4
int clslam_depth_metrics_scratch(int n_images, int hg, int wg);
int clslam_depth_metrics(const float* pred, const float* gt, float* out, void* scratch, float* resampled, float* medians,
                         int n_images, int h, int w, int hg, int wg, float min_depth, float max_depth, int flags, void* stream);

int clslam_pcl_backproject_scratch(int n_images, int h, int w);
int clslam_pcl_backproject(const float* depth, const float* inv_k, const float* image, float* points, long long* offsets,
                           void* scratch, int n_images, int h, int w, float dist_threshold, void* stream);
int clslam_pcl_transform(const float* points, const long long* offsets, const double* poses, float* out, long long m,
                         int n_segments, void* stream);
int clslam_pcl_splat_scratch(int rows, int cols);
int clslam_pcl_splat(const float* points, const long long* offsets, const double* poses, int n_segments, const double* K,
                     unsigned long long* zbuf, int rows, int cols, long long point_base, long long count, int has_min_z,
                     double min_z, int clear, void* stream);
int clslam_pcl_resolve(const float* points, const unsigned long long* zbuf, long long point_base, float* image, float* dist,
                       long long* index, int rows, int cols, int merge, void* stream);

#ifdef __cplusplus
}
#endif
#endif
```

Measured before the change: 352.0 frames/s.

## Fuse downsample 1x1 conv into stride-2 3x3 stage-entry conv kernel

Adds a fused stage-entry kernel path in which the ResNet block's stride-2 3x3 conv also computes the 1x1 stride-2 downsample projection from the same loaded input patch, writing two outputs with separate BN scale/shift. It replaces the previous approach of running the downsample conv on an auxiliary stream with event fork and join. The intent is to drop a separate launch and the repeated read of the input, and to remove the cross-stream synchronisation. The cost is more LDS, registers and stream-K slab workspace per workgroup, and the encoder loses its overlap with the auxiliary stream.

```diff
diff --git a/cl-slam_amd/clslam_hip/_lib.py b/cl-slam_amd/clslam_hip/_lib.py
--- a/cl-slam_amd/clslam_hip/_lib.py
+++ b/cl-slam_amd/clslam_hip/_lib.py
@@ -45,6 +45,7 @@
     'clslam_version': [],
     'clslam_is_device_build': [],
     'clslam_conv2d': [C.POINTER(ConvDesc), C.c_void_p],
+    'clslam_conv2d_stage_entry': [C.POINTER(ConvDesc), fptr, fptr, fptr, fptr, C.c_void_p],
     'clslam_conv2d_pick_config': [C.POINTER(ConvDesc)],
     'clslam_wino_weight_transform': [fptr, fptr, i32, i32, C.c_void_p],
     'clslam_weight_transpose': [fptr, fptr, i32, i32, i32, i32, C.c_void_p],
@@ -153,7 +154,7 @@
     'clslam_pcl_resolve': [fptr, fptr, C.c_longlong, fptr, fptr, fptr, i32, i32, i32, C.c_void_p],
 }
 _RESTYPES = {'clslam_last_error': C.c_char_p, 'clslam_last_error_string': C.c_char_p, 'clslam_build_id': C.c_char_p}
-ABI_VERSION = 106
+ABI_VERSION = 107
 _SIZE_FNS = {'clslam_wino_weight_size': [i32, i32]}
 _PTR_FNS = {'clslam_handoff_event_create': []}
 _VOID_FNS = {'clslam_handoff_event_destroy': [C.c_void_p]}
diff --git a/cl-slam_amd/clslam_hip/engine.py b/cl-slam_amd/clslam_hip/engine.py
--- a/cl-slam_amd/clslam_hip/engine.py
+++ b/cl-slam_amd/clslam_hip/engine.py
@@ -437,7 +437,7 @@
             self._conv_ws[handle] = torch.zeros(self.CONV_WS_BYTES, dtype=torch.uint8, device=self.device)
             ops.set_conv_workspace(handle, self._conv_ws[handle])
 
-    def _encoder(self, e, bufs, n: int, stem_inputs, waits=None, stream=None, aux=None, cu_limit=None) -> List[torch.Tensor]:
+    def _encoder(self, e, bufs, n: int, stem_inputs, waits=None, stream=None, cu_limit=None) -> List[torch.Tensor]:
         ops.PERSISTENT_CU_LIMIT = self._cu_enc if cu_limit is None else cu_limit
         ek = (id(self), 'enc', id(e), id(bufs), n)
         for i, (img_a, img_b, off, cnt) in enumerate(stem_inputs):
@@ -451,25 +451,14 @@
             for bi in range(2):
                 blk = e.blocks[li * 2 + bi]
                 t, y = bufs.t[li], bufs.y[li][bi]
-                res, joined = x, None
+                res = x
                 if blk.wd is not None:
                     res = bufs.ds[li]
-                    if aux is not None and stream is not None:
-                        evs = bufs.__dict__.setdefault('ds_events', {})
-                        fork, joined = evs.get(li) or evs.setdefault(li, (torch.cuda.Event(), torch.cuda.Event()))
-                        fork.record(stream)
-                        aux.wait_event(fork)
-                        with self._on(aux):
-                            ops.conv2d(x, blk.wd, res, scale=blk.sd, shift=blk.bd, ksize=1, stride=blk.stride, pad=0, act=ACT_NONE,
-                                       cache=self._desc_cache, key=(ek, li, bi, 'd'))
-                        joined.record(aux)
-                ops.conv2d(x, blk.w1, t, scale=blk.s1, shift=blk.b1, ksize=3, stride=blk.stride, act=ACT_RELU, weight_wino=blk.u1,
-                           cache=self._desc_cache, key=(ek, li, bi, 1))
-                if blk.wd is not None and joined is None:
-                    ops.conv2d(x, blk.wd, res, scale=blk.sd, shift=blk.bd, ksize=1, stride=blk.stride, pad=0, act=ACT_NONE,
-                               cache=self._desc_cache, key=(ek, li, bi, 'd'))
-                if joined is not None:
-                    stream.wait_event(joined)
+                    ops.conv2d_stage_entry(x, blk.w1, t, blk.wd, res, scale=blk.s1, shift=blk.b1, ds_scale=blk.sd, ds_shift=blk.bd,
+                                           act=ACT_RELU, cache=self._desc_cache, key=(ek, li, bi, 'entry'))
+                else:
+                    ops.conv2d(x, blk.w1, t, scale=blk.s1, shift=blk.b1, ksize=3, stride=blk.stride, act=ACT_RELU, weight_wino=blk.u1,
+                               cache=self._desc_cache, key=(ek, li, bi, 1))
                 ops.conv2d(t, blk.w2, y, scale=blk.s2, shift=blk.b2, residual=res, ksize=3, act=ACT_RELU, weight_wino=blk.u2,
                            cache=self._desc_cache, key=(ek, li, bi, 2))
                 x = y
@@ -621,9 +610,9 @@
         return self._encoder(self.enc['pose_encoder'], ws.penc, 2 * B, [(aug[-1], aug[0], 0, B), (aug[0], aug[1], B, B)],
                              waits=None if c.inputs_ready is None else c.inputs_ready[1:3], cu_limit=self._cu_pose, **kw)[4]
 
-    def _pose_branch(self, ws, c, side, ds_aux) -> torch.Tensor:
+    def _pose_branch(self, ws, c, side) -> torch.Tensor:
         with self._on(side):
-            pf4 = ws.pf4 if c.reuse else self._pose_encoder(ws, c, stream=side, aux=ds_aux)
+            pf4 = ws.pf4 if c.reuse else self._pose_encoder(ws, c, stream=side)
             self.wait_training(side)
             self._pose_decoder(ws, pf4)
         return pf4
@@ -631,23 +620,20 @@
     def _networks(self, ws, c) -> None:
         B, reuse, main = c.B, c.reuse, self._main
         side, wg = self._side_streams()
-        ds_aux = wg if (B == 1 and not self._capturing) else None
-        defer_identity = wg is not None and ds_aux is not None and c.inputs_ready is not None and not reuse
         if wg is not None:
             wg.wait_stream(main)
-            if not defer_identity:
-                self._enqueue_identity(ws, c, wg)
+            self._enqueue_identity(ws, c, wg)
         if side is not None:
             side.wait_stream(main)
             if reuse:
                 dfeats = ws.dfeats
                 self.wait_training(main)
                 self._depth_decoder(ws, dfeats)
-                pf4 = self._pose_branch(ws, c, side, ds_aux)
+                pf4 = self._pose_branch(ws, c, side)
             else:
                 dfeats = c.memo_feats if c.memo_feats is not None else self._encoder(
-                    self.enc['depth_encoder'], ws.denc, B, [(c.aug[0], None, 0, B)], stream=main, aux=ds_aux, cu_limit=self._cu_depth)
-                pf4 = self._pose_branch(ws, c, side, ds_aux)
+                    self.enc['depth_encoder'], ws.denc, B, [(c.aug[0], None, 0, B)], stream=main, cu_limit=self._cu_depth)
+                pf4 = self._pose_branch(ws, c, side)
                 self.wait_training(main)
                 self._depth_decoder(ws, dfeats)
             main.wait_stream(side)
@@ -659,8 +645,6 @@
             pf4 = ws.pf4 if reuse else self._pose_encoder(ws, c)
             self._pose_decoder(ws, pf4)
         ws.dfeats, ws.pf4 = dfeats, pf4
-        if defer_identity:
-            self._enqueue_identity(ws, c, wg)
 
     def _loss_stage(self, ws, c, sample_w: torch.Tensor, smooth_w: Optional[torch.Tensor]) -> None:
         inputs, rgb, B, H, W = c.inputs, c.rgb, c.B, self.H, self.W
diff --git a/cl-slam_amd/clslam_hip/ops.py b/cl-slam_amd/clslam_hip/ops.py
--- a/cl-slam_amd/clslam_hip/ops.py
+++ b/cl-slam_amd/clslam_hip/ops.py
@@ -19,15 +19,24 @@
 def profile_end():
     global PROFILE
     meta, PROFILE = PROFILE, None
-    cap = max(1, len(meta))
+    launches = sum(len(m) == 5 for m in meta)
+    cap = max(1, launches)
     ms = (C.c_float * cap)()
     count = C.c_int(0)
     _lib.get_lib().call('clslam_conv_profile_end', C.cast(ms, C.c_void_p), cap, C.cast(C.pointer(count), C.c_void_p))
     if not _lib.get_lib().is_device:
-        return [(k, cfg, fl, 0.0, desc, nb) for k, cfg, fl, desc, nb in meta]
-    if count.value != len(meta):
-        raise _lib.ClslamError(f'profile_end: {count.value} timed launches for {len(meta)} conv2d calls')
-    return [(k, cfg, fl, ms[i] * 1e-3, desc, nb) for i, (k, cfg, fl, desc, nb) in enumerate(meta)]
+        return [(m[0], m[1], m[2], 0.0, m[3], m[4]) for m in meta]
+    if count.value != launches:
+        raise _lib.ClslamError(f'profile_end: {count.value} timed launches for {launches} conv launches')
+    rows, i = [], -1
+    for m in meta:
+        if len(m) == 5:
+            i += 1
+            rows.append([m[0], m[1], m[2], ms[i] * 1e-3, m[3], m[4]])
+        else:
+            rows.append([m[0], m[1], m[2], ms[i] * 1e-3 * m[5], m[3], m[4]])
+            rows[-2][3] -= rows[-1][3]
+    return [tuple(r) for r in rows]
 
 
 _raw_stream = torch._C._cuda_getCurrentRawStream if hasattr(torch._C, '_cuda_getCurrentRawStream') else None
@@ -200,6 +209,57 @@
     return out
 
 
+def conv2d_stage_entry(src, weight, out, ds_weight, ds_out, *, scale=None, shift=None, ds_scale=None, ds_shift=None,
+                       act=ACT_RELU, config=-1, workspace=None, cu_limit=None, key=None, cache=None):
+    if cache is None:
+        cache = _CONV_DESC_CACHE
+    if key is not None and PROFILE is None:
+        ent = cache.get(key)
+        if ent is not None:
+            d, ref, lib, ds_args = ent
+            if (d.src_a == src.data_ptr() and d.out == out.data_ptr() and d.weight == weight.data_ptr() and
+                    ds_args[0] == ds_weight.data_ptr() and ds_args[3] == ds_out.data_ptr()):
+                stream = _stream(out)
+                ws = workspace if workspace is not None else (_CONV_WORKSPACES.get(stream) if _CONV_WORKSPACES else None)
+                if ws is None:
+                    d.workspace, d.workspace_bytes = None, 0
+                else:
+                    d.workspace, d.workspace_bytes = ws.data_ptr(), ws.numel()
+                d.cu_limit = PERSISTENT_CU_LIMIT if cu_limit is None else cu_limit
+                rc = lib.cdll.clslam_conv2d_stage_entry(ref, *ds_args, stream)
+                if rc != _lib.OK:
+                    raise _lib.ClslamError(f'clslam_conv2d_stage_entry failed ({rc}): {lib.cdll.clslam_last_error().decode()}')
+                return out, ds_out
+    B, Ho, Wo, Cout = out.shape
+    Hi, Wi, Cin = src.shape[1:]
+    assert weight.shape[0] == Cout and weight.numel() == Cout * 9 * Cin, weight.shape
+    assert ds_weight.shape[0] == Cout and ds_weight.numel() == Cout * Cin, ds_weight.shape
+    assert ds_out.shape == out.shape, (ds_out.shape, out.shape)
+    stream = _stream(out)
+    if workspace is None and _CONV_WORKSPACES:
+        workspace = _CONV_WORKSPACES.get(stream)
+    d = _lib.ConvDesc(_p(src), None, _p(weight), _p(scale), _p(shift), None, _p(out),
+                      B, Hi, Wi, Cin, 0, Ho, Wo, Cout, 3, 2, 1, PAD_ZERO, 0, act, config,
+                      None, ACT_NONE, None if workspace is None else workspace.data_ptr(),
+                      0 if workspace is None else workspace.numel(), None,
+                      PERSISTENT_CU_LIMIT if cu_limit is None else cu_limit)
+    ds_args = (_p(ds_weight), _p(ds_scale), _p(ds_shift), _p(ds_out))
+    if PROFILE is not None:
+        cfg = config if config >= 0 else _lib.get_lib().cdll.clslam_conv2d_pick_config(C.byref(d))
+        PROFILE.append(('conv', cfg, 2.0 * B * Ho * Wo * Cout * 9 * Cin, f'B{B} {Hi}x{Wi} {Cin}+0->{Cout} k3 s2 pad1',
+                        4.0 * (src.numel() + weight.numel() + out.numel())))
+        dd = _lib.ConvDesc(_p(src), None, _p(ds_weight), _p(ds_scale), _p(ds_shift), None, _p(ds_out),
+                           B, Hi, Wi, Cin, 0, Ho, Wo, Cout, 1, 2, 0, PAD_ZERO, 0, ACT_NONE, -1, None, ACT_NONE, d.workspace,
+                           d.workspace_bytes, None, d.cu_limit)
+        PROFILE.append(('conv', _lib.get_lib().cdll.clslam_conv2d_pick_config(C.byref(dd)), 2.0 * B * Ho * Wo * Cout * Cin,
+                        f'B{B} {Hi}x{Wi} {Cin}+0->{Cout} k1 s2 pad0', 4.0 * (src.numel() + ds_weight.numel() + ds_out.numel()), 0.1))
+    lib = _lib.get_lib()
+    lib.call('clslam_conv2d_stage_entry', C.byref(d), *ds_args, stream)
+    if key is not None and PROFILE is None:
+        cache[key] = (d, C.byref(d), lib, ds_args)
+    return out, ds_out
+
+
 def conv_desc(src_a, out_shape, *, src_b=None, ksize=3, stride=1, pad=None, pad_mode=PAD_ZERO, upsample_a=False):
     B, Ho, Wo, Cout = out_shape
     Ha, Wa, Ca = src_a.shape[1:]
diff --git a/cl-slam_amd/csrc/capi.hip b/cl-slam_amd/csrc/capi.hip
--- a/cl-slam_amd/csrc/capi.hip
+++ b/cl-slam_amd/csrc/capi.hip
@@ -135,7 +135,7 @@
     return CLSLAM_OK;
 }
 
-extern "C" int clslam_version(void) { return 106; }
+extern "C" int clslam_version(void) { return 107; }
 #ifndef CLSLAM_BUILD_ID
 #define CLSLAM_BUILD_ID "unstamped"
 #endif
diff --git a/cl-slam_amd/csrc/common.h b/cl-slam_amd/csrc/common.h
--- a/cl-slam_amd/csrc/common.h
+++ b/cl-slam_amd/csrc/common.h
@@ -49,6 +49,13 @@
 
 inline int cdiv(int a, int b) { return (a + b - 1) / b; }
 
+struct StageEntryDs {
+    const float* weight;
+    const float* scale;
+    const float* shift;
+    float* out;
+};
+
 bool profile_next_events(hipEvent_t* start, hipEvent_t* stop);
 hipEvent_t take_handoff_event();
 
diff --git a/cl-slam_amd/csrc/conv_fwd.hip b/cl-slam_amd/csrc/conv_fwd.hip
--- a/cl-slam_amd/csrc/conv_fwd.hip
+++ b/cl-slam_amd/csrc/conv_fwd.hip
@@ -254,8 +254,8 @@
 
 }
 
-namespace clslam { int conv3x3_patch_dispatch(const clslam_conv_desc* d, int cfg, hipStream_t stream);
-                   int conv3x3_sk_dispatch(const clslam_conv_desc* d, int cfg, hipStream_t stream);
+namespace clslam { int conv3x3_patch_dispatch(const clslam_conv_desc* d, int cfg, hipStream_t stream, const StageEntryDs* ds = nullptr);
+                   int conv3x3_sk_dispatch(const clslam_conv_desc* d, int cfg, hipStream_t stream, const StageEntryDs* ds = nullptr);
                    int conv3x3_wino_dispatch(const clslam_conv_desc* d, hipStream_t stream);
                    int conv3x3_wino_supported(const clslam_conv_desc* d);
                    int conv3x3_wino_units_per_group(const clslam_conv_desc* d); }
@@ -379,3 +379,28 @@
         default: set_error("conv2d: unknown config %d", cfg); return CLSLAM_ERR_INVALID;
     }
 }
+
+extern "C" int clslam_conv2d_stage_entry(const clslam_conv_desc* d, const float* ds_weight, const float* ds_scale, const float* ds_shift,
+                                         float* ds_out, void* stream_) {
+    hipStream_t stream = (hipStream_t)stream_;
+    CLSLAM_REQUIRE(d, "conv2d_stage_entry: null descriptor");
+    if (d->batch == 0 || d->out_h * d->out_w == 0) return CLSLAM_OK;
+    CLSLAM_REQUIRE(d->src_a && d->weight && d->out && ds_weight && ds_out, "conv2d_stage_entry: null pointer");
+    CLSLAM_REQUIRE(d->ksize == 3 && d->stride == 2 && d->pad == 1 && d->pad_mode == CLSLAM_PAD_ZERO && !d->upsample_a && d->ch_b == 0 &&
+                       !d->residual && !d->actgrad_src,
+                   "conv2d_stage_entry: needs a 3x3 stride-2 pad-1 zero-padded convolution of one source without residual "
+                   "(ksize %d, stride %d, pad %d)", d->ksize, d->stride, d->pad);
+    CLSLAM_REQUIRE(d->ch_a % 16 == 0 && d->ch_out % 16 == 0, "conv2d_stage_entry: channels must be multiples of 16 (Cin=%d Cout=%d)",
+                   d->ch_a, d->ch_out);
+    CLSLAM_REQUIRE(d->out_h == (d->in_h - 1) / 2 + 1 && d->out_w == (d->in_w - 1) / 2 + 1,
+                   "conv2d_stage_entry: output size %dx%d does not match input %dx%d", d->out_h, d->out_w, d->in_h, d->in_w);
+    CLSLAM_REQUIRE(ds_out != d->out, "conv2d_stage_entry: the two outputs must not alias");
+    const StageEntryDs ds = {ds_weight, ds_scale, ds_shift, ds_out};
+    const int cfg = d->config < 0 ? clslam_conv2d_pick_config(d) : d->config;
+    CLSLAM_REQUIRE(cfg == 23 || (cfg >= 30 && cfg <= 32), "conv2d_stage_entry: config %d has no fused instantiation", cfg);
+    if (cfg >= 30) {
+        const int rc = conv3x3_sk_dispatch(d, cfg, stream, &ds);
+        if (rc == CLSLAM_OK || d->config >= 0) return rc;
+    }
+    return conv3x3_patch_dispatch(d, 23, stream, &ds);
+}
diff --git a/cl-slam_amd/csrc/conv_patch.hip b/cl-slam_amd/csrc/conv_patch.hip
--- a/cl-slam_amd/csrc/conv_patch.hip
+++ b/cl-slam_amd/csrc/conv_patch.hip
@@ -24,15 +24,20 @@
     float* ws;
     unsigned* counters;
     size_t ws_bytes;
+    const float* __restrict__ ds_wgt;
+    const float* __restrict__ ds_scale;
+    const float* __restrict__ ds_shift;
+    float* __restrict__ ds_out;
 };
 
 constexpr int run_pp(int bm) { return bm <= 64 ? 224 : 320; }
 
-template <int TH, int TW, int BN, int BK, int MF, int WGM, bool RUN, int LDPAD, int S, bool SK>
+template <int TH, int TW, int BN, int BK, int MF, int WGM, bool RUN, int LDPAD, int S, bool SK, bool DS = false>
 __global__ __launch_bounds__(256) void conv3x3_patch_kernel(PatchK p) {
     constexpr int BM = TH * TW;
     constexpr int PH = (TH - 1) * S + 3, PW = (TW - 1) * S + 3, PP = RUN ? run_pp(BM) : PH * PW;
     static_assert(!RUN || S == 1, "run tiles are stride-1 only");
+    static_assert(!DS || (S == 2 && !RUN && !SK && BN * (BK / 4) <= 256), "fused stage entry: stride-2 rectangle tiles, unsplit");
     constexpr int LD = BK + LDPAD;
     constexpr int WGN = 4 / WGM;
     constexpr int WM = BM / WGM, WN = BN / WGN;
@@ -46,6 +51,7 @@
 
     __shared__ __attribute__((aligned(16))) float Ps[PP * LD];
     __shared__ __attribute__((aligned(16))) float Wsm[9 * BN * LD];
+    __shared__ __attribute__((aligned(16))) float Dsm[DS ? BN * LD : 4];
 
     const int tid = threadIdx.x, lane = tid & 63, wave = tid >> 6;
     const int wm0 = (wave / WGN) * WM, wn0 = (wave % WGN) * WN;
@@ -111,6 +117,10 @@
         wptr[it] = p.wgt + ((size_t)(okW[it] ? n0 + n : 0) * 9 + (okW[it] ? tap : 0)) * Cin + c4 * 4;
     }
     float4 rp[P_IT], rw[W_IT];
+    const bool hasD = DS && tid < BN * F4;
+    const bool okD = hasD && (n0 + tid / F4 < p.Cout);
+    const float* dptr = DS ? p.ds_wgt + (size_t)(okD ? n0 + tid / F4 : 0) * Cin + (tid % F4) * 4 : nullptr;
+    float4 rd = make_float4(0.f, 0.f, 0.f, 0.f);
     auto load_global = [&](int c0) {
 #pragma unroll
         for (int it = 0; it < P_IT; ++it) {
@@ -121,6 +131,7 @@
         }
 #pragma unroll
         for (int it = 0; it < W_IT; ++it) rw[it] = *reinterpret_cast<const float4*>(wptr[it] + c0);
+        if constexpr (DS) { if (hasD) rd = *reinterpret_cast<const float4*>(dptr + c0); }
     };
     auto store_lds = [&]() {
 #pragma unroll
@@ -137,6 +148,9 @@
             if (!okW[it]) v = make_float4(0.f, 0.f, 0.f, 0.f);
             if (f < W_SLOTS) *reinterpret_cast<float4*>(&Wsm[(f / F4) * LD + (f % F4) * 4]) = v;
         }
+        if constexpr (DS) {
+            if (hasD) *reinterpret_cast<float4*>(&Dsm[(tid / F4) * LD + (tid % F4) * 4]) = okD ? rd : make_float4(0.f, 0.f, 0.f, 0.f);
+        }
     };
 
     typedef float accv __attribute__((ext_vector_type(NACC)));
@@ -150,6 +164,15 @@
             for (int h = 0; h < NCH; ++h)
 #pragma unroll
                 for (int r = 0; r < NACC; ++r) acc[i][j][h][r] = 0.f;
+    accv accd[DS ? TM : 1][DS ? TN : 1];
+    if constexpr (DS) {
+#pragma unroll
+        for (int i = 0; i < TM; ++i)
+#pragma unroll
+            for (int j = 0; j < TN; ++j)
+#pragma unroll
+                for (int r = 0; r < NACC; ++r) accd[i][j][r] = 0.f;
+    }
 
     const int frow = lane % MF, kg = lane / MF;
     int prow[TM];
@@ -173,6 +196,15 @@
         const int n = min(n0 + wn0 + j * MF + (lane % MF), p.Cout - 1);
         scv[j] = p.scale ? p.scale[n] : 1.f;
         shv[j] = p.shift ? p.shift[n] : 0.f;
+    }
+    float scd[DS ? TN : 1], shd[DS ? TN : 1];
+    if constexpr (DS) {
+#pragma unroll
+        for (int j = 0; j < TN; ++j) {
+            const int n = min(n0 + wn0 + j * MF + (lane % MF), p.Cout - 1);
+            scd[j] = p.ds_scale ? p.ds_scale[n] : 1.f;
+            shd[j] = p.ds_shift ? p.ds_shift[n] : 0.f;
+        }
     }
     constexpr bool PRE_RES = (TM * TN * NACC <= 4) && !SK && RUN;
     float resv[PRE_RES ? TM * TN * NACC : 1];
@@ -220,6 +252,27 @@
                             accv& a = acc[i][j][t % NCH];
                             if constexpr (MF == 32) a = mfma_32x32x2(av, bv, a);
                             else a = mfma_16x16x4(av, bv, a);
+                        }
+                    }
+                }
+                if constexpr (DS) {
+                    if (tap == 4) {
+                        float4 fd[TN];
+#pragma unroll
+                        for (int j = 0; j < TN; ++j)
+                            fd[j] = *reinterpret_cast<const float4*>(&Dsm[(wn0 + j * MF + frow) * LD + kk * KSTEP + kg * 4]);
+#pragma unroll
+                        for (int t = 0; t < 4; ++t) {
+#pragma unroll
+                            for (int i = 0; i < TM; ++i) {
+                                const float av = t == 0 ? fa[i].x : t == 1 ? fa[i].y : t == 2 ? fa[i].z : fa[i].w;
+#pragma unroll
+                                for (int j = 0; j < TN; ++j) {
+                                    const float dv = t == 0 ? fd[j].x : t == 1 ? fd[j].y : t == 2 ? fd[j].z : fd[j].w;
+                                    if constexpr (MF == 32) accd[i][j] = mfma_32x32x2(av, dv, accd[i][j]);
+                                    else accd[i][j] = mfma_16x16x4(av, dv, accd[i][j]);
+                                }
+                            }
                         }
                     }
                 }
@@ -348,10 +401,22 @@
                 const size_t o = element(i, j, r, ok);
                 if (ok) p.out[o] = vals[i][j][r];
             }
+    if constexpr (DS) {
+#pragma unroll
+        for (int i = 0; i < TM; ++i)
+#pragma unroll
+            for (int j = 0; j < TN; ++j)
+#pragma unroll
+                for (int r = 0; r < NACC; ++r) {
+                    bool ok;
+                    const size_t o = element(i, j, r, ok);
+                    if (ok) p.ds_out[o] = accd[i][j][r] * scd[j] + shd[j];
+                }
+    }
     (void)NE;
 }
 
-template <int TH, int TW, int BN, int BK, int MF, int WGM, bool RUN = false, int LDPAD = 4, int S = 1, bool SKOK = false>
+template <int TH, int TW, int BN, int BK, int MF, int WGM, bool RUN = false, int LDPAD = 4, int S = 1, bool SKOK = false, bool DS = false>
 static int launch_patch(PatchK k, hipStream_t stream) {
     if (RUN) {
         const int spanned = (TH * TW - 1 + k.Wo - 1) / k.Wo + 1;
@@ -364,11 +429,15 @@
     const int chunks = (k.Ca + k.Cb) / BK;
     int ksplit = 1;
     if (const char* e = getenv("CLSLAM_SPLITK")) { if (k.ws) ksplit = std::max(1, std::min(atoi(e), chunks)); }
-    if (!SKOK || (size_t)ksplit * tiles * (TH * TW * BN) * sizeof(float) > k.ws_bytes || tiles > kSplitKMaxTiles) ksplit = 1;
+    if (DS || !SKOK || (size_t)ksplit * tiles * (TH * TW * BN) * sizeof(float) > k.ws_bytes || tiles > kSplitKMaxTiles) ksplit = 1;
     k.ksplit = ksplit;
     k.nblk = tiles * ksplit;
     k.n_fastest = ((size_t)k.Cout * 9 * (k.Ca + k.Cb) * 4 <= (size_t)(2 << 20)) ? 1 : 0;
     if (const char* e = getenv("CLSLAM_N_FASTEST")) k.n_fastest = atoi(e);
+    if constexpr (DS) {
+        conv_launch(conv3x3_patch_kernel<TH, TW, BN, BK, MF, WGM, RUN, LDPAD, S, false, true>, k.nblk, stream, k);
+        return check_launch("conv3x3_patch(stage entry)");
+    }
     if constexpr (SKOK) {
         if (ksplit > 1) {
             conv_launch(conv3x3_patch_kernel<TH, TW, BN, BK, MF, WGM, RUN, LDPAD, S, true>, k.nblk, stream, k);
@@ -379,8 +448,9 @@
     return check_launch("conv3x3_patch");
 }
 
-int conv3x3_patch_dispatch(const clslam_conv_desc* d, int cfg, hipStream_t stream) {
+int conv3x3_patch_dispatch(const clslam_conv_desc* d, int cfg, hipStream_t stream, const StageEntryDs* ds) {
     const int st = d->stride;
+    if (ds && cfg != 23) { set_error("conv2d: the fused stage entry runs on patch config 23 (asked for %d)", cfg); return CLSLAM_ERR_INVALID; }
     if (d->ksize != 3 || (st != 1 && st != 2) || (st == 2) != (cfg == 23) || ((cfg == 24 || cfg == 25) && (d->ch_a + d->ch_b) % 32 != 0) ||
         (cfg == 26 && d->ch_out % 32 != 0)) {
         set_error("conv2d: patch configs need a 3x3 conv with stride 1 (configs 10-22) or 2 (config 23)");
@@ -397,6 +467,8 @@
     k.Cout = d->ch_out; k.pad = d->pad; k.pad_mode = d->pad_mode; k.ups = d->upsample_a; k.act = d->act;
     k.tilesX = k.tilesY = k.tilesN = k.nblk = 0; k.n_fastest = 0;
     k.ksplit = 1; k.ws = nullptr; k.counters = nullptr; k.ws_bytes = 0;
+    k.ds_wgt = ds ? ds->weight : nullptr; k.ds_scale = ds ? ds->scale : nullptr; k.ds_shift = ds ? ds->shift : nullptr;
+    k.ds_out = ds ? ds->out : nullptr;
     if (d->workspace && d->workspace_bytes > (size_t)kSplitKMaxTiles * sizeof(unsigned)) {
         k.counters = (unsigned*)d->workspace;
         k.ws = (float*)((char*)d->workspace + (size_t)kSplitKMaxTiles * sizeof(unsigned));
@@ -416,7 +488,8 @@
         case 20: return launch_patch<8, 16, 16, 16, 16, 4, false, 8, 1, true>(k, stream);
         case 21: return launch_patch<4, 16, 16, 16, 16, 4, false, 8, 1, true>(k, stream);
         case 22: return launch_patch<4, 16, 16, 16, 16, 4, true, 8, 1, true>(k, stream);
-        case 23: return launch_patch<4, 16, 16, 16, 16, 4, false, 8, 2, true>(k, stream);
+        case 23: if (ds) return launch_patch<4, 16, 16, 16, 16, 4, false, 8, 2, true, true>(k, stream);
+                 return launch_patch<4, 16, 16, 16, 16, 4, false, 8, 2, true>(k, stream);
         case 24: return launch_patch<4, 16, 16, 32, 16, 4, true, 8>(k, stream);
         case 25: return launch_patch<4, 16, 16, 32, 16, 4, false, 8>(k, stream);
         case 26: return launch_patch<4, 8, 32, 16, 16, 2, false, 8>(k, stream);
diff --git a/cl-slam_amd/csrc/conv_sk.hip b/cl-slam_amd/csrc/conv_sk.hip
--- a/cl-slam_amd/csrc/conv_sk.hip
+++ b/cl-slam_amd/csrc/conv_sk.hip
@@ -31,19 +31,26 @@
     int b_fastest;
     unsigned epoch;
     int dbg;
+    const float* __restrict__ ds_wgt;
+    const float* __restrict__ ds_scale;
+    const float* __restrict__ ds_shift;
+    float* __restrict__ ds_out;
 };
 
 constexpr int sk_run_pp(int bm, int s = 1) { return s == 2 ? 544 : (bm <= 64 ? 336 : 416); }
 
-template <int TH, int TW, bool RUN, int S, int BN, int NWM, int NWN>
+template <int TH, int TW, bool RUN, int S, int BN, int NWM, int NWN, bool DS = false>
 __global__ __launch_bounds__(NWM * NWN * 64) void conv3x3_sk_kernel(SkK p) {
     constexpr int NW = NWM * NWN, NT = NW * 64;
     constexpr int BM = TH * TW;
     constexpr int TM = BM / (16 * NWM), TN = BN / (16 * NWN);
     constexpr int PH = (TH - 1) * S + 3, PW = (TW - 1) * S + 3;
     constexpr int PP = RUN ? sk_run_pp(BM, S) : (PH * PW + 15) / 16 * 16;
-    constexpr int NPP = PP / 16, NWP = 9 * BN / 16;
-    constexpr int STAGE = (PP + 9 * BN) * 16;
+    constexpr int NTAP = DS ? 10 : 9;
+    constexpr int NPP = PP / 16, NWP = NTAP * BN / 16;
+    constexpr int STAGE = (PP + NTAP * BN) * 16;
+    constexpr int SLAB = (DS ? 2 : 1) * BM * BN;
+    static_assert(!DS || S == 2, "fused stage entry: stride 2");
     static_assert(BM % (16 * NWM) == 0 && BN % (16 * NWN) == 0 && TW % 16 == 0, "tile shape");
 
     __shared__ __attribute__((aligned(1024))) float lds[2 * STAGE];
@@ -67,6 +74,7 @@
     const int drow = lane >> 2;
     const int dslot = (lane & 3) ^ (((drow >> 2) & 1) << 1);
     const int wlane_off = drow * 9 * Cin + dslot * 4;
+    const int dlane_off = drow * Cin + dslot * 4;
 
     auto decode_tile = [&](int t, int& tn, int& tx, int& ty, int& b) {
         if (p.b_fastest) {
@@ -135,6 +143,7 @@
                 const int tap = piece / (BN / 16), nb = (piece % (BN / 16)) * 16;
                 const bool ok = dma_n0 + nb + drow < p.Cout;
                 const float* src = ok ? p.wgt + (size_t)((dma_n0 + nb) * 9 + tap) * Cin + c0 + wlane_off : g_zero_page + dslot * 4;
+                if constexpr (DS) { if (ok && tap == 9) src = p.ds_wgt + (size_t)(dma_n0 + nb) * Cin + c0 + dlane_off; }
                 lds_dma16(src, stage + PP * 16 + piece * 256);
             }
         }
@@ -154,7 +163,19 @@
 #pragma unroll
                 for (int r = 0; r < 4; ++r) acc[i][j][r] = 0.f;
     };
+    f32x4 accd[DS ? TM : 1][DS ? TN : 1];
+    auto zero_accd = [&]() {
+        if constexpr (DS) {
+#pragma unroll
+            for (int i = 0; i < TM; ++i)
+#pragma unroll
+                for (int j = 0; j < TN; ++j)
+#pragma unroll
+                    for (int r = 0; r < 4; ++r) accd[i][j][r] = 0.f;
+        }
+    };
     zero_acc();
+    zero_accd();
 
     int prow[TM];
     int c_pw = PW;
@@ -213,6 +234,24 @@
                         acc[i][j] = mfma_16x16x4(wv, xv, acc[i][j]);
                     }
                 }
+            if constexpr (DS) {
+                if (tap == 4) {
+                    float4 fd[TN];
+#pragma unroll
+                    for (int j = 0; j < TN; ++j) fd[j] = *reinterpret_cast<const float4*>(&Ws[9 * BN * 16 + brow[j]]);
+#pragma unroll
+                    for (int t = 0; t < 4; ++t)
+#pragma unroll
+                        for (int i = 0; i < TM; ++i) {
+                            const float xv = t == 0 ? ca[i].x : t == 1 ? ca[i].y : t == 2 ? ca[i].z : ca[i].w;
+#pragma unroll
+                            for (int j = 0; j < TN; ++j) {
+                                const float dv = t == 0 ? fd[j].x : t == 1 ? fd[j].y : t == 2 ? fd[j].z : fd[j].w;
+                                accd[i][j] = mfma_16x16x4(dv, xv, accd[i][j]);
+                            }
+                        }
+                }
+            }
             sched_fence();
         }
     };
@@ -222,12 +261,18 @@
         const bool owner = c_hi == p.NC;
         if ((p.dbg & 2) && (!owner || c_lo > 0)) return;
         if (!owner) {
-            float* slab = p.slabs + (size_t)grp * (BM * BN) + (size_t)wave * (TM * TN * 256) + lane * 4;
+            float* slab = p.slabs + (size_t)grp * SLAB + (size_t)wave * (TM * TN * 256) + lane * 4;
             mfma_results_settle();
 #pragma unroll
             for (int i = 0; i < TM; ++i)
 #pragma unroll
                 for (int j = 0; j < TN; ++j) coherent_store4(slab + (i * TN + j) * 256, acc[i][j]);
+            if constexpr (DS) {
+#pragma unroll
+                for (int i = 0; i < TM; ++i)
+#pragma unroll
+                    for (int j = 0; j < TN; ++j) coherent_store4(slab + BM * BN + (i * TN + j) * 256, accd[i][j]);
+            }
             vmem_drain_visible();
             publish_pending = true;
             return;
@@ -244,31 +289,40 @@
             }
             __syncthreads();
             const float poison = s_flag_ok ? 0.f : __builtin_nanf("");
-            const float* slab0 = p.slabs + (size_t)wave * (TM * TN * 256) + lane * 4;
-            for (int base = 0; base < ncon; base += 4) {
-                const float* sp[4];
-#pragma unroll
-                for (int q = 0; q < 4; ++q) sp[q] = slab0 + (size_t)(grp - 1 - min(base + q, ncon - 1)) * (BM * BN);
-                f32x4 part[4][TM * TN];
-                if constexpr (TM * TN == 4) coherent_load4x4_x4(sp[0], sp[1], sp[2], sp[3], part[0], part[1], part[2], part[3]);
-                else if constexpr (TM * TN == 2) coherent_load4x2_x4(sp[0], sp[1], sp[2], sp[3], part[0], part[1], part[2], part[3]);
-                else {
-#pragma unroll
-                    for (int q = 0; q < 4; ++q)
-#pragma unroll
-                        for (int r = 0; r < TM * TN; r += 2) coherent_load4x2(sp[q] + r * 256, part[q][r], part[q][r + 1]);
+            auto gather = [&](int set_off, f32x4 (&dst)[TM][TN]) {
+                const float* slab0 = p.slabs + set_off + (size_t)wave * (TM * TN * 256) + lane * 4;
+                constexpr int GB = (DS && !RUN && TH == 8) ? 2 : 4;
+                for (int base = 0; base < ncon; base += GB) {
+                    const float* sp[GB];
+#pragma unroll
+                    for (int q = 0; q < GB; ++q) sp[q] = slab0 + (size_t)(grp - 1 - min(base + q, ncon - 1)) * SLAB;
+                    f32x4 part[GB][TM * TN];
+                    if constexpr (GB == 2) {
+                        static_assert(GB != 2 || TM * TN == 4, "two-slab gather: 2x2 MFMA tiles per wave");
+#pragma unroll
+                        for (int q = 0; q < GB; ++q) coherent_load4x4(sp[q], part[q][0], part[q][1], part[q][2], part[q][3]);
+                    } else if constexpr (TM * TN == 4) coherent_load4x4_x4(sp[0], sp[1], sp[2], sp[3], part[0], part[1], part[2], part[3]);
+                    else if constexpr (TM * TN == 2) coherent_load4x2_x4(sp[0], sp[1], sp[2], sp[3], part[0], part[1], part[2], part[3]);
+                    else {
+#pragma unroll
+                        for (int q = 0; q < GB; ++q)
+#pragma unroll
+                            for (int r = 0; r < TM * TN; r += 2) coherent_load4x2(sp[q] + r * 256, part[q][r], part[q][r + 1]);
+                    }
+#pragma unroll
+                    for (int q = 0; q < GB; ++q)
+                        if (base + q < ncon) {
+#pragma unroll
+                            for (int i = 0; i < TM; ++i)
+#pragma unroll
+                                for (int j = 0; j < TN; ++j)
+#pragma unroll
+                                    for (int r = 0; r < 4; ++r) dst[i][j][r] += part[q][i * TN + j][r] + poison;
+                        }
                 }
-#pragma unroll
-                for (int q = 0; q < 4; ++q)
-                    if (base + q < ncon) {
-#pragma unroll
-                        for (int i = 0; i < TM; ++i)
-#pragma unroll
-                            for (int j = 0; j < TN; ++j)
-#pragma unroll
-                                for (int r = 0; r < 4; ++r) acc[i][j][r] += part[q][i * TN + j][r] + poison;
-                    }
-            }
+            };
+            gather(0, acc);
+            if constexpr (DS) gather(BM * BN, accd);
         }
         if (p.dbg & 1) { if (acc[0][0][0] == 12345.678f) uncounted_flag_store((unsigned*)p.out, 1u); return; }
         int tn, tx, ty, b;
@@ -293,6 +347,7 @@
         const float* extra = p.residual ? p.residual : p.actgrad_src;
         const bool has_res = p.residual != nullptr, has_ag = !has_res && p.actgrad_src != nullptr;
         float4 sc[TN], sh[TN], ex[TM][TN];
+        float4 scd[DS ? TN : 1], shd[DS ? TN : 1];
         bool ch_ok[TN];
 #pragma unroll
         for (int j = 0; j < TN; ++j) {
@@ -301,6 +356,10 @@
             const int nc = ch_ok[j] ? n : 0;
             sc[j] = p.scale ? *reinterpret_cast<const float4*>(p.scale + nc) : make_float4(1.f, 1.f, 1.f, 1.f);
             sh[j] = p.shift ? *reinterpret_cast<const float4*>(p.shift + nc) : make_float4(0.f, 0.f, 0.f, 0.f);
+            if constexpr (DS) {
+                scd[j] = p.ds_scale ? *reinterpret_cast<const float4*>(p.ds_scale + nc) : make_float4(1.f, 1.f, 1.f, 1.f);
+                shd[j] = p.ds_shift ? *reinterpret_cast<const float4*>(p.ds_shift + nc) : make_float4(0.f, 0.f, 0.f, 0.f);
+            }
 #pragma unroll
             for (int i = 0; i < TM; ++i)
                 ex[i][j] = (extra && ch_ok[j] && pix_ok[i]) ? *reinterpret_cast<const float4*>(extra + opix[i] + n)
@@ -320,6 +379,15 @@
                 v.z *= has_ag ? act_grad_from_output(e.z, p.actgrad_kind) : 1.f; v.w *= has_ag ? act_grad_from_output(e.w, p.actgrad_kind) : 1.f;
                 res[i][j] = v;
             }
+        float4 resd[DS ? TM : 1][DS ? TN : 1];
+        if constexpr (DS) {
+#pragma unroll
+            for (int j = 0; j < TN; ++j)
+#pragma unroll
+                for (int i = 0; i < TM; ++i)
+                    resd[i][j] = make_float4(accd[i][j][0] * scd[j].x + shd[j].x, accd[i][j][1] * scd[j].y + shd[j].y,
+                                             accd[i][j][2] * scd[j].z + shd[j].z, accd[i][j][3] * scd[j].w + shd[j].w);
+        }
         vmem_drain_visible();
 #pragma unroll
         for (int j = 0; j < TN; ++j) {
@@ -327,6 +395,15 @@
 #pragma unroll
             for (int i = 0; i < TM; ++i)
                 if (ch_ok[j] && pix_ok[i]) uncounted_store4(p.out + opix[i] + n, res[i][j]);
+        }
+        if constexpr (DS) {
+#pragma unroll
+            for (int j = 0; j < TN; ++j) {
+                const int n = n0 + (wn * TN + j) * 16 + 4 * kg;
+#pragma unroll
+                for (int i = 0; i < TM; ++i)
+                    if (ch_ok[j] && pix_ok[i]) uncounted_store4(p.ds_out + opix[i] + n, resd[i][j]);
+            }
         }
     };
 
@@ -359,6 +436,7 @@
                 --ct; c_lo = seg_lo(ct); c_hi = seg_hi(ct); cc = c_lo;
                 cmp_setup_tile(ct);
                 zero_acc();
+                zero_accd();
             }
         }
     }
@@ -394,7 +472,7 @@
     return e;
 }
 
-template <int TH, int TW, bool RUN, int S, int BN, int NWM, int NWN>
+template <int TH, int TW, bool RUN, int S, int BN, int NWM, int NWN, bool DS = false>
 static int launch_sk(SkK k, const clslam_conv_desc* d, hipStream_t stream) {
     constexpr int BM = TH * TW;
     if (RUN) {
@@ -411,13 +489,14 @@
     if (const char* e = getenv("CLSLAM_SK_B_FASTEST")) k.b_fastest = atoi(e);
     constexpr int PHs = (TH - 1) * S + 3, PWs = (TW - 1) * S + 3;
     constexpr int PPs = RUN ? sk_run_pp(BM, S) : (PHs * PWs + 15) / 16 * 16;
-    constexpr size_t lds_bytes = (size_t)2 * (PPs + 9 * BN) * 64 + 16;
+    constexpr size_t lds_bytes = (size_t)2 * (PPs + (DS ? 10 : 9) * BN) * 64 + 16;
+    static_assert(lds_bytes <= 163840, "LDS stages of one workgroup");
     constexpr int per_cu = (int)std::max<size_t>(1, std::min<size_t>((size_t)(163840 / lds_bytes), (size_t)(2048 / (NWM * NWN * 64))));
     int G = (d->cu_limit > 0 ? std::min(d->cu_limit, sk_device_cus()) : sk_device_cus()) * per_cu;
     if (const char* e = getenv("CLSLAM_SK_GROUPS")) G = std::max(1, atoi(e));
     G = (int)std::min<long long>(std::min(G, kSkMaxGroups), k.units);
     k.G = G;
-    const size_t need = (size_t)kSkSlabOffsetBytes + (size_t)G * BM * BN * sizeof(float);
+    const size_t need = (size_t)kSkSlabOffsetBytes + (size_t)G * (DS ? 2 : 1) * BM * BN * sizeof(float);
     if (!d->workspace || d->workspace_bytes < need) {
         set_error("conv2d: the stream-K kernel needs a zero-filled workspace of %zu bytes on the launching stream", need);
         return CLSLAM_ERR_INVALID;
@@ -425,7 +504,7 @@
     k.flags = (unsigned*)d->workspace + kSkFlagOffset;
     k.epoch = sk_next_epoch(d->workspace);
     k.slabs = (float*)((char*)d->workspace + kSkSlabOffsetBytes);
-    auto kern = conv3x3_sk_kernel<TH, TW, RUN, S, BN, NWM, NWN>;
+    auto kern = conv3x3_sk_kernel<TH, TW, RUN, S, BN, NWM, NWN, DS>;
 #if CLSLAM_DEVICE_BUILD
     hipEvent_t e0, e1;
     if (profile_next_events(&e0, &e1)) {
@@ -437,8 +516,9 @@
     return check_launch("conv3x3_sk");
 }
 
-int conv3x3_sk_dispatch(const clslam_conv_desc* d, int cfg, hipStream_t stream) {
+int conv3x3_sk_dispatch(const clslam_conv_desc* d, int cfg, hipStream_t stream, const StageEntryDs* ds) {
     const int st = d->stride;
+    if (ds && (st != 2 || cfg < 30 || cfg > 32)) { set_error("conv2d: the fused stage entry runs on stream-K configs 30-32 with stride 2 (asked for %d, stride %d)", cfg, st); return CLSLAM_ERR_INVALID; }
     if (d->ksize != 3 || (st != 1 && st != 2)) { set_error("conv2d: stream-K configs need a 3x3 conv with stride 1 or 2"); return CLSLAM_ERR_INVALID; }
     SkK k;
     k.src_a = d->src_a; k.src_b = d->src_b; k.wgt = d->weight; k.scale = d->scale; k.shift = d->shift;
@@ -448,8 +528,15 @@
     k.tilesX = k.tilesY = k.tilesN = k.tiles = k.NC = k.G = 0; k.units = 0; k.slabs = nullptr; k.flags = nullptr;
     k.epoch = 1u; k.b_fastest = 0;
     k.dbg = 0;
+    k.ds_wgt = ds ? ds->weight : nullptr; k.ds_scale = ds ? ds->scale : nullptr; k.ds_shift = ds ? ds->shift : nullptr;
+    k.ds_out = ds ? ds->out : nullptr;
     if (const char* e = getenv("CLSLAM_SK_DBG")) k.dbg = atoi(e);
     const bool s2 = st == 2;
+    if (ds) {
+        if (cfg == 30) return launch_sk<8, 16, false, 2, 64, 4, 2, true>(k, d, stream);
+        if (cfg == 31) return launch_sk<4, 16, false, 2, 64, 4, 2, true>(k, d, stream);
+        return launch_sk<8, 16, true, 2, 64, 4, 2, true>(k, d, stream);
+    }
     switch (cfg) {
         case 30: return s2 ? launch_sk<8, 16, false, 2, 64, 4, 2>(k, d, stream) : launch_sk<8, 16, false, 1, 64, 4, 2>(k, d, stream);
         case 31: return s2 ? launch_sk<4, 16, false, 2, 64, 4, 2>(k, d, stream) : launch_sk<4, 16, false, 1, 64, 4, 2>(k, d, stream);
diff --git a/include/clslam_hip.h b/include/clslam_hip.h
--- a/include/clslam_hip.h
+++ b/include/clslam_hip.h
@@ -21,7 +21,7 @@
 #define CLSLAM_PAD_ZERO 0
 #define CLSLAM_PAD_REFLECT 1
 
-#define CLSLAM_ABI_VERSION 106
+#define CLSLAM_ABI_VERSION 107
 int clslam_version(void);
 const char* clslam_last_error(void);
 const char* clslam_last_error_string(void);
@@ -47,6 +47,8 @@
     int32_t cu_limit;
 } clslam_conv_desc;
 int clslam_conv2d(const clslam_conv_desc* desc, void* stream);
+int clslam_conv2d_stage_entry(const clslam_conv_desc* desc, const float* ds_weight, const float* ds_scale, const float* ds_shift,
+                              float* ds_out, void* stream);
 int clslam_conv2d_pick_config(const clslam_conv_desc* desc);
 size_t clslam_wino_weight_size(int ch_out, int ch_in);
 int clslam_wino_weight_transform(const float* w, float* u, int ch_out, int ch_in, void* stream);
```

Result: no change. 354.4 frames/s (median of 6 runs) (+0.7%).
